# mprib/caliscope

Measured on AMD Instinct MI355X. Metric: observations/sec per LM iteration, higher is better.
Workload: dtype f64; 1 GPU; cfg4: 64 cams / 2000000 obs in total (200000 points / 2000000 obs on rank 0), extrinsics-only BA, linear loss; n_obs_total=2000000, params_per_camera=6, tolerances=ftol=xtol=gtol=1e-8 (reference defaults), sums=FP64 atomics (default)

## Files before the change

### caliscope_amd/csrc/cba_kernels.h

```cpp
#pragma once
#include <hip/hip_runtime.h>

#include "ba_math.h"
#include "trf_math.h"
#include "wg_binding.h"
#include "chol_schedule.h"

namespace cba {

constexpr int BLOCK = 256;
constexpr int CHUNK = 256;
constexpr int WAVE = 64;

struct VecLayout {
  int ncp;
  int ncp_pad;
  int P;
  int Ppad;
  __host__ __device__ long total() const { return (long)ncp_pad + 3L * Ppad; }
};

__device__ __forceinline__ double wave_sum(double v) {
#pragma unroll
  for (int o = WAVE / 2; o > 0; o >>= 1) v += __shfl_down(v, o, WAVE);
// ... 422 lines not shown
  double* sh_pt = sh_U + (DET ? DET_ROUND * DET_LD : n_cams * UP::STRIDE);
  double* sh_red = sh_pt + 9 * CHUNK;
  int* sh_perm = reinterpret_cast<int*>(sh_red + 8);
  int* sh_cs = sh_perm + CHUNK;
  constexpr int DROUNDS = (UP::STRIDE + DET_ROUND - 1) / DET_ROUND;
  constexpr int DM = DET ? DETM : 1;
  double dacc[DROUNDS][DM];
#pragma unroll
  for (int r = 0; r < DROUNDS; ++r)
#pragma unroll
    for (int m = 0; m < DM; ++m) dacc[r][m] = 0.0;
  if (!CAMG) stage_camtab(sh_tab, tab, n_cams);
  if (!DET)
    for (int i = threadIdx.x; i < n_cams * UP::STRIDE; i += BLOCK) sh_U[i] = 0.0;
  __syncthreads();
  const double* px = xvec + lay.ncp_pad;
  double* gp = gvec + lay.ncp_pad;
  double cost = 0.0;
  bool bad = false;
  const int last_obs = max(chunk_start[n_chunks] - 1, 0);
  int ch = blockIdx.x;
  int o0 = 0, o1 = 0;
  ObsRec cur = {0.0, 0.0, 0, 0};
  if (ch < n_chunks) {
    o0 = chunk_start[ch]; o1 = chunk_start[ch + 1];
    cur = load_obs(obs_u, obs_v, obs_cam, obs_pt, min(o0 + (int)threadIdx.x, last_obs));
  }
  while (ch < n_chunks) {
    const int nxt = ch + gridDim.x, nc = min(nxt, n_chunks - 1);
    const int no0 = chunk_start[nc], no1 = chunk_start[nc + 1];
    const ObsRec nx = load_obs(obs_u, obs_v, obs_cam, obs_pt, min(no0 + (int)threadIdx.x, last_obs));
    const int cp0 = chunk_pts[2 * ch], npts = chunk_pts[2 * ch + 1];
    const int pp = min(cp0 + (int)threadIdx.x, lay.P - 1);
    const int pa = pt_start[pp] - o0, pb = pt_start[pp + 1] - o0;
    const int i = o0 + threadIdx.x;
    double pv[9];
#pragma unroll
    for (int q = 0; q < 9; ++q) pv[q] = 0.0;
    double e[2] = {0.0, 0.0}, A[2][MAX_NC];
    int np_det = 0;
    if (DET) {
#pragma unroll
      for (int k = 0; k < MAX_NC; ++k) { A[0][k] = 0.0; A[1][k] = 0.0; }
      sh_perm[threadIdx.x] = det.perm[(long)ch * CHUNK + threadIdx.x];
      for (int q = threadIdx.x; q <= n_cams; q += BLOCK) sh_cs[q] = det.cstart[(long)ch * (n_cams + 1) + q];
    }
    if (i < o1) {
      const int cam = cur.cam, pt = cur.pt;
      double B[2][3];
      cost += obs_linearize<NC>(cam_of(cam), px[pt], px[lay.Ppad + pt], px[2 * lay.Ppad + pt], cur.u, cur.v, loss,
                                f_scale, e, A, B);
      if (!isfinite(e[0] + e[1])) bad = true;
      pv[0] = B[0][0] * B[0][0] + B[1][0] * B[1][0];
      pv[1] = B[0][0] * B[0][1] + B[1][0] * B[1][1];
      pv[2] = B[0][0] * B[0][2] + B[1][0] * B[1][2];
      pv[3] = B[0][1] * B[0][1] + B[1][1] * B[1][1];
      pv[4] = B[0][1] * B[0][2] + B[1][1] * B[1][2];
      pv[5] = B[0][2] * B[0][2] + B[1][2] * B[1][2];
      pv[6] = B[0][0] * e[0] + B[1][0] * e[1];
      pv[7] = B[0][1] * e[0] + B[1][1] * e[1];
      pv[8] = B[0][2] * e[0] + B[1][2] * e[1];
      const int np = (int)cam_of(cam).nparams;
      np_det = np;
      if (!DET) {
        double* Uc = sh_U + cam * UP::STRIDE;
#pragma unroll
        for (int r = 0; r < NC; ++r) {
          if (r < np) {
#pragma unroll
            for (int c = r; c < NC; ++c)
              if (c < np) lds_add(&Uc[UP::idx(r, c)], A[0][r] * A[0][c] + A[1][r] * A[1][c]);
            lds_add(&Uc[UP::TRI + r], A[0][r] * e[0] + A[1][r] * e[1]);
          }
        }
      }
    }
#pragma unroll
    for (int q = 0; q < 9; ++q) sh_pt[q * CHUNK + threadIdx.x] = pv[q];
    __syncthreads();
    auto reduce_point = [&](int p, int a, int b) {
      double acc[9];
#pragma unroll
      for (int q = 0; q < 9; ++q) acc[q] = 0.0;
      for (int j = a; j < b; ++j) {
#pragma unroll
        for (int q = 0; q < 9; ++q) acc[q] += sh_pt[q * CHUNK + j];
      }
#pragma unroll
      for (int q = 0; q < 6; ++q) Vblk[(long)q * lay.Ppad + p] = acc[q];
      gp[p] = acc[6];
      gp[lay.Ppad + p] = acc[7];
      gp[2 * lay.Ppad + p] = acc[8];
    };
    if (npts < 0 && threadIdx.x < 9) {
      double acc = 0.0;
      for (int j = 0; j < o1 - o0; ++j) acc += sh_pt[threadIdx.x * CHUNK + j];
      if (threadIdx.x < 6) unsafeAtomicAdd(&Vblk[(long)threadIdx.x * lay.Ppad + cp0], acc);
      else unsafeAtomicAdd(&gp[(long)(threadIdx.x - 6) * lay.Ppad + cp0], acc);
    }
    if ((int)threadIdx.x < npts && pb > pa) reduce_point(pp, pa, pb);
    for (int lp = threadIdx.x + BLOCK; lp < npts; lp += BLOCK) {
      const int p = cp0 + lp;
      const int a = pt_start[p] - o0, b = pt_start[p + 1] - o0;
      if (b > a) reduce_point(p, a, b);
    }
    __syncthreads();
    if (DET) {
#pragma unroll
      for (int rd = 0; rd < DROUNDS; ++rd) {
        double val[DET_ROUND];
#pragma unroll
        for (int q = 0; q < DET_ROUND; ++q) val[q] = cam_block_value<NC>(rd * DET_ROUND + q, A, e, np_det);
        det_round<DM>(val, sh_U, sh_perm, sh_cs, n_cams, dacc[rd]);
      }
    }
    cur = nx; o0 = no0; o1 = no1; ch = nxt;
  }
  double* dst = partialU + (long)blockIdx.x * n_cams * UP::STRIDE;
  if (DET) {
#pragma unroll
    for (int rd = 0; rd < DROUNDS; ++rd)
#pragma unroll
      for (int m = 0; m < DM; ++m) {
        const int task = (int)threadIdx.x + BLOCK * m;
        const int c = task / DET_ROUND, v = rd * DET_ROUND + task % DET_ROUND;
        if (task < n_cams * DET_ROUND && v < UP::STRIDE) dst[c * UP::STRIDE + v] = dacc[rd][m];
      }
  } else {
    for (int i = threadIdx.x; i < n_cams * UP::STRIDE; i += BLOCK) dst[i] = sh_U[i];
  }
  const double tot = block_sum(cost, sh_red);
  if (threadIdx.x == 0) partial_cost[blockIdx.x] = tot;
  if (bad) flags[0] = 1;
}

constexpr int CS_MAX_PTS = 512;
struct CsPlan {
  const double* u;
  const double* v;
  const int* cam;
  const int* ptl;
  const int* obs_start;
  const int* pt_first;
  const int* pt_count;
  int n_sc;
  int pmax;
};
struct TrialSrc {
  const double *x, *g, *sinv, *s;
  const double* ab;
  double* x_new;
  double* step_partial;
};
template <int NC, bool CAMG = false, bool UGLOB = false, bool TRIAL = false>
__global__ void __launch_bounds__(BLOCK)
k_build_cs(CsPlan cs, const double* __restrict__ xvec, VecLayout lay, const double* __restrict__ tab, int n_cams, int loss, double f_scale,
           double* __restrict__ Vblk, double* __restrict__ gvec, double* __restrict__ partialU, double* __restrict__ partial_cost,
           int* __restrict__ flags, const double* __restrict__ skip, TrialSrc trial = TrialSrc{}) {
  CBA_STAMP(ST_BUILD);
  using UP = UPack<NC>;
  static_assert(!UGLOB || CAMG, "a camera count beyond the LDS copy of the blocks is beyond the LDS copy of the table as well");
  if (skip && *skip != 0.0) return;
  extern __shared__ __attribute__((aligned(16))) double sh[];
  double* sh_tab = sh;
  double* sh_U = sh_tab + (CAMG ? 0 : n_cams * CAMTAB_LDS);
  const int PM = cs.pmax;
  double* sh_vg = sh_U + (UGLOB ? 0 : n_cams * UP::STRIDE);
  double* sh_x = sh_vg + 9 * PM;
  double* sh_red = sh_x + 3 * PM;
  if (!CAMG) stage_camtab(sh_tab, tab, n_cams);
  if (!UGLOB)
    for (int i = threadIdx.x; i < n_cams * UP::STRIDE; i += BLOCK) sh_U[i] = 0.0;
  const double* px = xvec + lay.ncp_pad;
  double* gp = gvec + lay.ncp_pad;
  double cost = 0.0, step_sq = 0.0;
  const double t_alpha = TRIAL ? trial.ab[0] : 0.0, t_beta = TRIAL ? trial.ab[1] : 0.0;
  bool bad = false;
  for (int s = blockIdx.x; s < cs.n_sc; s += gridDim.x) {
    const int o0 = cs.obs_start[s], o1 = cs.obs_start[s + 1], p0 = cs.pt_first[s], npts = cs.pt_count[s];
    __syncthreads();
    for (int i = threadIdx.x; i < 9 * PM; i += BLOCK) sh_vg[i] = 0.0;
    if (TRIAL) {
      for (int i = threadIdx.x; i < npts; i += BLOCK) {
#pragma unroll
        for (int k = 0; k < 3; ++k) {
          const long e = (long)lay.ncp_pad + (long)k * lay.Ppad + p0 + i;
          const double si = trial.sinv[e];
          const double st = t_alpha * trial.g[e] / (si * si) + t_beta * trial.s[e];
          const double xn = trial.x[e] + st;
          trial.x_new[e] = xn;
          sh_x[k * PM + i] = xn;
          step_sq = fma(st, st, step_sq);
        }
      }
    } else {
      for (int i = threadIdx.x; i < npts; i += BLOCK) {
        sh_x[i] = px[p0 + i]; sh_x[PM + i] = px[lay.Ppad + p0 + i]; sh_x[2 * PM + i] = px[2 * lay.Ppad + p0 + i];
      }
    }
    __syncthreads();
    const int R = (o1 - o0 + BLOCK - 1) / BLOCK;
    const int j0 = o0 + (int)threadIdx.x * R, j1 = min(j0 + R, o1);
    double acc[UP::STRIDE];
#pragma unroll
    for (int q = 0; q < UP::STRIDE; ++q) acc[q] = 0.0;
    int cur_cam = -1, cur_np = 0;
    auto flush = [&]() {
      if (cur_cam < 0) return;
      double* Uc = (UGLOB ? partialU : sh_U) + (long)cur_cam * UP::STRIDE;
#pragma unroll
      for (int r = 0; r < NC; ++r) {
        if (r < cur_np) {
#pragma unroll
          for (int c = r; c < NC; ++c)
            if (c < cur_np) { if (UGLOB) atomicAdd(&Uc[UP::idx(r, c)], acc[UP::idx(r, c)]); else lds_add(&Uc[UP::idx(r, c)], acc[UP::idx(r, c)]); }
          if (UGLOB) atomicAdd(&Uc[UP::TRI + r], acc[UP::TRI + r]); else lds_add(&Uc[UP::TRI + r], acc[UP::TRI + r]);
        }
      }
#pragma unroll
      for (int q = 0; q < UP::STRIDE; ++q) acc[q] = 0.0;
    };
    const int jl = max(o1 - 1, 0);
    int n_cam = cs.cam[min(j0, jl)], n_pl = cs.ptl[min(j0, jl)];
    double n_u = cs.u[min(j0, jl)], n_v = cs.v[min(j0, jl)];
    for (int j = j0; j < j1; ++j) {
      asm volatile("s_waitcnt vmcnt(0)" ::: "memory");
      asm volatile("" : "+v"(n_cam), "+v"(n_pl), "+v"(n_u), "+v"(n_v));
      const int cam = n_cam, pl = n_pl;
      const double u = n_u, v = n_v;
      n_cam = cs.cam[min(j + 1, jl)]; n_pl = cs.ptl[min(j + 1, jl)]; n_u = cs.u[min(j + 1, jl)]; n_v = cs.v[min(j + 1, jl)];
      __builtin_amdgcn_sched_barrier(0);
      if (cam != cur_cam) { flush(); cur_cam = cam; cur_np = (int)cam_of<CAMG>(sh_tab, tab, cam).nparams; }
      double e[2], A[2][MAX_NC], B[2][3];
      {
        double G[2][3], Yr[3], Aint[2][3];
        const CamTab& ctc = cam_of<CAMG>(sh_tab, tab, cam);
        cost += obs_factors(ctc, sh_x[pl], sh_x[PM + pl], sh_x[2 * PM + pl], u, v, loss, f_scale, e, G, Yr, Aint, B);
#pragma unroll
        for (int r = 0; r < 2; ++r) {
          const double p0 = Yr[1] * G[r][2] - Yr[2] * G[r][1], p1 = Yr[2] * G[r][0] - Yr[0] * G[r][2], p2 = Yr[0] * G[r][1] - Yr[1] * G[r][0];
          if constexpr (UGLOB) {
            A[r][0] = ctc.Jl[0] * p0 + ctc.Jl[3] * p1 + ctc.Jl[6] * p2;
            A[r][1] = ctc.Jl[1] * p0 + ctc.Jl[4] * p1 + ctc.Jl[7] * p2;
            A[r][2] = ctc.Jl[2] * p0 + ctc.Jl[5] * p1 + ctc.Jl[8] * p2;
          } else {
            A[r][0] = p0; A[r][1] = p1; A[r][2] = p2;
          }
          A[r][3] = G[r][0]; A[r][4] = G[r][1]; A[r][5] = G[r][2];
          A[r][6] = Aint[r][0]; A[r][7] = Aint[r][1]; A[r][8] = Aint[r][2];
        }
      }
      if (!isfinite(e[0] + e[1])) bad = true;
#pragma unroll
      for (int r = 0; r < NC; ++r) {
#pragma unroll
        for (int c = r; c < NC; ++c) acc[UP::idx(r, c)] = fma(A[1][r], A[1][c], fma(A[0][r], A[0][c], acc[UP::idx(r, c)]));
        acc[UP::TRI + r] = fma(A[1][r], e[1], fma(A[0][r], e[0], acc[UP::TRI + r]));
      }
      lds_add(&sh_vg[0 * PM + pl], B[0][0] * B[0][0] + B[1][0] * B[1][0]);
      lds_add(&sh_vg[1 * PM + pl], B[0][0] * B[0][1] + B[1][0] * B[1][1]);
      lds_add(&sh_vg[2 * PM + pl], B[0][0] * B[0][2] + B[1][0] * B[1][2]);
      lds_add(&sh_vg[3 * PM + pl], B[0][1] * B[0][1] + B[1][1] * B[1][1]);
      lds_add(&sh_vg[4 * PM + pl], B[0][1] * B[0][2] + B[1][1] * B[1][2]);
      lds_add(&sh_vg[5 * PM + pl], B[0][2] * B[0][2] + B[1][2] * B[1][2]);
      lds_add(&sh_vg[6 * PM + pl], B[0][0] * e[0] + B[1][0] * e[1]);
      lds_add(&sh_vg[7 * PM + pl], B[0][1] * e[0] + B[1][1] * e[1]);
      lds_add(&sh_vg[8 * PM + pl], B[0][2] * e[0] + B[1][2] * e[1]);
    }
    flush();
    __syncthreads();
    for (int i = threadIdx.x; i < npts; i += BLOCK) {
#pragma unroll
      for (int q = 0; q < 6; ++q) Vblk[(long)q * lay.Ppad + p0 + i] = sh_vg[q * PM + i];
      gp[p0 + i] = sh_vg[6 * PM + i];
      gp[lay.Ppad + p0 + i] = sh_vg[7 * PM + i];
      gp[2 * lay.Ppad + p0 + i] = sh_vg[8 * PM + i];
    }
  }
  __syncthreads();
  if (!UGLOB) {
    for (int c = threadIdx.x; c < n_cams; c += BLOCK) {
      const double* Jl = tab + (long)c * CAMTAB_DOUBLES + 12;
      double* Uc = sh_U + (long)c * UP::STRIDE;
      double M[3][3], T[3][3];
#pragma unroll
      for (int r = 0; r < 3; ++r)
#pragma unroll
        for (int q = 0; q < 3; ++q) M[r][q] = Uc[UP::idx(min(r, q), max(r, q))];
#pragma unroll
      for (int r = 0; r < 3; ++r)
#pragma unroll
        for (int q = 0; q < 3; ++q) T[r][q] = Jl[r] * M[0][q] + Jl[3 + r] * M[1][q] + Jl[6 + r] * M[2][q];
#pragma unroll
      for (int r = 0; r < 3; ++r)
#pragma unroll
        for (int q = r; q < 3; ++q) Uc[UP::idx(r, q)] = T[r][0] * Jl[q] + T[r][1] * Jl[3 + q] + T[r][2] * Jl[6 + q];
#pragma unroll
      for (int q = 3; q <= NC; ++q) {
        double* v0 = (q < NC) ? &Uc[UP::idx(0, q)] : &Uc[UP::TRI + 0];
        double* v1 = (q < NC) ? &Uc[UP::idx(1, q)] : &Uc[UP::TRI + 1];
        double* v2 = (q < NC) ? &Uc[UP::idx(2, q)] : &Uc[UP::TRI + 2];
        const double a0 = *v0, a1 = *v1, a2 = *v2;
        *v0 = Jl[0] * a0 + Jl[3] * a1 + Jl[6] * a2;
        *v1 = Jl[1] * a0 + Jl[4] * a1 + Jl[7] * a2;
        *v2 = Jl[2] * a0 + Jl[5] * a1 + Jl[8] * a2;
      }
    }
    __syncthreads();
    double* dst = partialU + (long)blockIdx.x * n_cams * UP::STRIDE;
    for (int i = threadIdx.x; i < n_cams * UP::STRIDE; i += BLOCK) dst[i] = sh_U[i];
  }
  const double tot = block_sum(cost, sh_red);
  if (threadIdx.x == 0) partial_cost[blockIdx.x] = tot;
  if (TRIAL) {
    const double st = block_sum(step_sq, sh_red);
    if (threadIdx.x == 0) trial.step_partial[blockIdx.x] = st;
  }
  if (bad) flags[0] = 1;
}

__global__ void __launch_bounds__(256)
k_gather_uv(const double* __restrict__ uv_raw, const int* __restrict__ order, long n, double* __restrict__ u, double* __restrict__ v) {
  for (long i = (long)blockIdx.x * 256 + threadIdx.x; i < n; i += (long)gridDim.x * 256) {
    const double2 w = reinterpret_cast<const double2*>(uv_raw)[order[i]];
    u[i] = w.x; v[i] = w.y;
  }
}
__global__ void __launch_bounds__(256)
k_cs_fill(const int* __restrict__ perm, const int* __restrict__ sc_obs, const int* __restrict__ sc_p0, const double* __restrict__ u,
          const double* __restrict__ v, const int* __restrict__ cam, const int* __restrict__ pt, double* __restrict__ cu, double* __restrict__ cv,
          int* __restrict__ ccam, int* __restrict__ cptl) {
  const int s = blockIdx.x, o0 = sc_obs[s], o1 = sc_obs[s + 1], p0 = sc_p0[s];
  for (int j = o0 + threadIdx.x; j < o1; j += 256) {
    const int i = perm[j];
    cu[j] = u[i]; cv[j] = v[i]; ccam[j] = cam[i]; cptl[j] = pt[i] - p0;
  }
}

template <int NC>
__global__ void k_unpack_camera_grad(const double* __restrict__ Upacked, const int* __restrict__ cam_off,
                                     const int* __restrict__ cam_np, int n_cams, double* __restrict__ gvec) {
  using UP = UPack<NC>;
  const int t = blockIdx.x * blockDim.x + threadIdx.x;
  const int c = t / NC, r = t % NC;
  if (c >= n_cams || r >= cam_np[c]) return;
  gvec[cam_off[c] + r] = Upacked[c * UP::STRIDE + UP::TRI + r];
}

template <int NC>
__global__ void k_scale_update(const double* __restrict__ Upacked, const double* __restrict__ Vblk,
                               const int* __restrict__ param_cam, const int* __restrict__ param_loc, VecLayout lay,
                               int first, double* __restrict__ sinv, const double* __restrict__ cdiag) {
  using UP = UPack<NC>;
  const long total = lay.total();
  for (long i = (long)blockIdx.x * blockDim.x + threadIdx.x; i < total; i += (long)gridDim.x * blockDim.x) {
    double v;
    if (i < lay.ncp_pad) {
      if (i >= lay.ncp) continue;
      const int r = param_loc[i];
      v = Upacked[param_cam[i] * UP::STRIDE + UP::idx(r, r)];
    } else {
      const long k = (i - lay.ncp_pad) / lay.Ppad, p = (i - lay.ncp_pad) % lay.Ppad;
      if (p >= lay.P) continue;
      const int q = (k == 0) ? 0 : (k == 1 ? 3 : 5);
      v = Vblk[(long)q * lay.Ppad + p];
      if (cdiag) v += cdiag[k * lay.Ppad + p];
    }
    v = sqrt(v);
    if (first) { if (v == 0.0) v = 1.0; }
    else v = fmax(v, sinv[i]);
    sinv[i] = v;
  }
}

__global__ void k_cam_rescale(const double* __restrict__ state, const double* __restrict__ mult, const double* __restrict__ diag_h,
                              int ncp, double* __restrict__ sinv, double* __restrict__ cam_diag) {
  const int i = blockIdx.x * blockDim.x + threadIdx.x;
  if (i >= ncp) return;
  const double si = state[i] * mult[i];
  sinv[i] = si;
  cam_diag[i] = diag_h[i] * si * si;
}

__global__ void __launch_bounds__(BLOCK)
k_lin_scalars(const double* __restrict__ x, const double* __restrict__ g, const double* __restrict__ sinv,
              long total, int cam_end, int count_cams, int max_from, double* __restrict__ v1, double* __restrict__ partial,
              double* __restrict__ partial_max) {
  __shared__ double sh_red[BLOCK / WAVE];
  double s0 = 0, s1 = 0, s2 = 0, m = 0;
  for (long i = (long)blockIdx.x * BLOCK + threadIdx.x; i < total; i += (long)gridDim.x * BLOCK) {
    const double gi = g[i], si = sinv[i], xi = x[i];
    const double gh = gi / si;
    v1[i] = gh / si;
    if (i >= max_from) m = fmax(m, fabs(gi));
    if (i < cam_end && !count_cams) continue;
    s0 += gh * gh;
    s1 += (xi * si) * (xi * si);
    s2 += xi * xi;
  }
  double r;
  r = block_sum(s0, sh_red); if (threadIdx.x == 0) partial[blockIdx.x * 4 + 0] = r;
  r = block_sum(s1, sh_red); if (threadIdx.x == 0) partial[blockIdx.x * 4 + 1] = r;
  r = block_sum(s2, sh_red); if (threadIdx.x == 0) partial[blockIdx.x * 4 + 2] = r;
  if (threadIdx.x == 0) partial[blockIdx.x * 4 + 3] = 0.0;
  r = block_max(m, sh_red); if (threadIdx.x == 0) partial_max[blockIdx.x] = r;
}

__global__ void k_combine(const double* __restrict__ g, const double* __restrict__ sinv, const double* __restrict__ s,
                          double a, double b, long total, const double* __restrict__ over, int n_over, double* __restrict__ out) {
  for (long i = (long)blockIdx.x * blockDim.x + threadIdx.x; i < total; i += (long)gridDim.x * blockDim.x) {
    const double si = sinv[i];
    out[i] = (i < n_over) ? over[i] : a * g[i] / (si * si) + b * s[i];
  }
}

constexpr int MAIL_GNORM = 60, MAIL_GNORM_SEQ = 61;
struct SpecSkip {
  const int* word;
  const double* max_rows;
  int n_rows;
  double* mail; unsigned long long seq;
};
__device__ __forceinline__ void publish_gnorm(const SpecSkip& sk) {
  __shared__ double sh_gn[BLOCK / WAVE];
  double m = 0.0;
  for (int b = threadIdx.x; b < sk.n_rows; b += BLOCK) m = fmax(m, sk.max_rows[b]);
  m = block_max(m, sh_gn);
  if (threadIdx.x == 0) {
    sk.mail[MAIL_GNORM] = m;
    __threadfence_system();
    reinterpret_cast<volatile unsigned long long*>(sk.mail)[MAIL_GNORM_SEQ] = sk.seq;
  }
}
__global__ void __launch_bounds__(BLOCK) k_gnorm_pub(SpecSkip sk) { publish_gnorm(sk); }

// ... 2021 lines not shown
    for (int k = 0; k < NP; ++k) rec[k] = mine[k];
    asm volatile("s_waitcnt lgkmcnt(0)" ::: "memory");
#pragma unroll
    for (int k = 0; k < NP; ++k) asm volatile("" : "+v"(rec[k].x), "+v"(rec[k].y));
    const bool more = ch + stride < n_chunks;
    if (more) issue(nx.o0);
    const int ncam = obs_cam[min(nx.o0 + tid, last_obs)];
    const Ent nn = load_ent(min(ch + 2 * stride, last_chunk));
    const PtIn pcur = load_point(cur.cp0, cur.npts);
    __builtin_amdgcn_sched_barrier(0);
    double t0, t1, t2;
    {
      const double* cs = sh_step + cam * CSS;
      const double w0 = cs[0], w1 = cs[1], w2 = cs[2];
      const double Y0 = rec[0].x, Y1 = rec[0].y, Y2 = rec[1].x;
      const double m0 = fma(w1, Y2, fma(-w2, Y1, cs[3]));
      const double m1 = fma(w2, Y0, fma(-w0, Y2, cs[4]));
      const double m2 = fma(w0, Y1, fma(-w1, Y0, cs[5]));
      t0 = fma(rec[4].y, m2, fma(rec[3].x, m1, rec[1].y * m0));
      t1 = fma(rec[5].x, m2, fma(rec[3].y, m1, rec[2].x * m0));
      t2 = fma(rec[5].y, m2, fma(rec[4].x, m1, rec[2].y * m0));
      if constexpr (NC == 9) {
        const double i0 = cs[6], i1 = cs[7], i2 = cs[8];
        t0 = fma(rec[9].x, i2, fma(rec[7].y, i1, fma(rec[6].x, i0, t0)));
        t1 = fma(rec[9].y, i2, fma(rec[8].x, i1, fma(rec[6].y, i0, t1)));
        t2 = fma(rec[10].x, i2, fma(rec[8].y, i1, fma(rec[7].x, i0, t2)));
      }
      if (cur.o0 + tid >= cur.o1) { t0 = 0.0; t1 = 0.0; t2 = 0.0; }
    }
    double* pt = sh_pt + buf * BSR_PT;
    pt[tid] = t0; pt[CHUNK + tid] = t1; pt[2 * CHUNK + tid] = t2;
    point_phase(pprev, sh_pt + (buf ^ 1) * BSR_PT, eprev.cp0, eprev.npts, eprev.o0);
    __syncthreads();
    pprev = pcur; eprev = cur;
    buf ^= 1;
    if (!more) break;
    cam = ncam; cur = nx; nx = nn; ch += stride;
  }
  asm volatile("s_waitcnt vmcnt(0)" ::: "memory");
  point_phase(pprev, sh_pt + (buf ^ 1) * BSR_PT, eprev.cp0, eprev.npts, eprev.o0);
  if (SCAL) {
    __syncthreads();
    double r;
    r = block_sum(sc0, sh_pt); if (tid == 0) step_partial[blockIdx.x * 4 + 0] = r;
    r = block_sum(sc1, sh_pt); if (tid == 0) { step_partial[blockIdx.x * 4 + 1] = r; step_partial[blockIdx.x * 4 + 2] = 0.0; step_partial[blockIdx.x * 4 + 3] = 0.0; }
  }
}
template <int NC, bool SCAL = false>
__global__ void __launch_bounds__(BLOCK)
k_backsub_rec(const double* __restrict__ Trec, const int* __restrict__ obs_cam, const int* __restrict__ pt_start, const int* __restrict__ chunk_start,
              const int* __restrict__ chunk_pts, int n_chunks, VecLayout lay, const double* __restrict__ tab, const int* __restrict__ cam_off,
              const int* __restrict__ cam_np, int n_cams, double lam, const double* __restrict__ lam_dev, const double* __restrict__ Vblk,
              const double* __restrict__ gvec, const double* __restrict__ sinv, double* __restrict__ svec, double* __restrict__ step_partial) {
  CBA_STAMP(ST_BACKSUB);
  extern __shared__ __attribute__((aligned(16))) double sh[];
  if (lam_dev) lam = *lam_dev;
  backsub_rec_body<NC, SCAL>(Trec, obs_cam, pt_start, chunk_start, chunk_pts, n_chunks, lay, tab, cam_off, cam_np, n_cams, lam, Vblk,
                             gvec + lay.ncp_pad, sinv + lay.ncp_pad, svec, svec + lay.ncp_pad, step_partial, sh);
}

__global__ void __launch_bounds__(BLOCK)
k_step_scalars(const double* __restrict__ g, const double* __restrict__ sinv, const double* __restrict__ s, long total,
               long first, double* __restrict__ partial) {
  __shared__ double sh_red[BLOCK / WAVE];
  double s0 = 0, s1 = 0;
  for (long i = first + (long)blockIdx.x * BLOCK + threadIdx.x; i < total; i += (long)gridDim.x * BLOCK) {
    const double p = s[i] * sinv[i];
    s0 += p * p;
    s1 += g[i] * s[i];
  }
  double r;
  r = block_sum(s0, sh_red); if (threadIdx.x == 0) partial[blockIdx.x * 4 + 0] = r;
  r = block_sum(s1, sh_red); if (threadIdx.x == 0) partial[blockIdx.x * 4 + 1] = r;
  if (threadIdx.x == 0) { partial[blockIdx.x * 4 + 2] = 0.0; partial[blockIdx.x * 4 + 3] = 0.0; }
}
__global__ void __launch_bounds__(BLOCK)
k_w_scalar(const double* __restrict__ g, const double* __restrict__ sinv, const double* __restrict__ s, long total,
           long first, const double* __restrict__ scal_gdot, double gh_sq, const double* __restrict__ gh_sq_dev,
           double* __restrict__ partial) {
  __shared__ double sh_red[BLOCK / WAVE];
  if (gh_sq_dev) gh_sq = *gh_sq_dev;
  const double c = scal_gdot[0] / gh_sq;
  double s0 = 0;
  for (long i = first + (long)blockIdx.x * BLOCK + threadIdx.x; i < total; i += (long)gridDim.x * BLOCK) {
    const double w = s[i] * sinv[i] - c * g[i] / sinv[i];
    s0 += w * w;
  }
  const double r = block_sum(s0, sh_red);
  if (threadIdx.x == 0) partial[blockIdx.x] = r;
}

__global__ void __launch_bounds__(BLOCK)
k_trial_update(const double* __restrict__ x, const double* __restrict__ g, const double* __restrict__ sinv,
               const double* __restrict__ s, double alpha, double beta, long total, int cam_end, int count_cams,
               const double* __restrict__ cam_x_new, int n_over, const double* __restrict__ ab_dev, double* __restrict__ x_new,
               double* __restrict__ partial, double* __restrict__ tab_out = nullptr, const double* __restrict__ cam_const = nullptr,
               const int* __restrict__ cam_model = nullptr, const int* __restrict__ cam_np = nullptr, const int* __restrict__ cam_off = nullptr,
               int n_cams = 0) {
  __shared__ double sh_red[BLOCK / WAVE];
  if (ab_dev) { alpha = ab_dev[0]; beta = ab_dev[1]; }
  double s0 = 0;
  auto entry = [&](long i) {
    const double si = sinv[i];
    double st = alpha * g[i] / (si * si) + beta * s[i];
    double xn = x[i] + st;
    if (i < n_over) { xn = cam_x_new[i]; st = xn - x[i]; }
    x_new[i] = xn;
    if (i >= cam_end || count_cams) s0 += st * st;
  };
  if (tab_out) {
    if (blockIdx.x == 0)
      for (long i = threadIdx.x; i < cam_end; i += BLOCK) entry(i);
    for (long i = cam_end + (long)blockIdx.x * BLOCK + threadIdx.x; i < total; i += (long)gridDim.x * BLOCK) entry(i);
  } else {
    for (long i = (long)blockIdx.x * BLOCK + threadIdx.x; i < total; i += (long)gridDim.x * BLOCK) entry(i);
  }
  const double r = block_sum(s0, sh_red);
  if (threadIdx.x == 0) partial[blockIdx.x] = r;
  if (tab_out && blockIdx.x == 0) {
    __threadfence();
    __syncthreads();
    for (int c = threadIdx.x; c < n_cams; c += BLOCK) {
      double xc[MAX_NC];
      const int np = cam_np[c];
      for (int i = 0; i < MAX_NC; ++i) xc[i] = (i < np) ? __builtin_nontemporal_load(&x_new[cam_off[c] + i]) : 0.0;
      CamTab t;
      cam_prepare(xc, cam_const + c * CAM_CONST_STRIDE, cam_model[c], np, &t, cam_off[c]);
      const double* src = reinterpret_cast<const double*>(&t);
      for (int i = 0; i < CAMTAB_DOUBLES; ++i) tab_out[c * CAMTAB_DOUBLES + i] = src[i];
    }
  }
}

__device__ __forceinline__ void fused_lam(double* __restrict__ scal, double radius_in, double* __restrict__ fz);
struct SubspaceIn;
__device__ __forceinline__ void fused_subspace(double* __restrict__ scal, const int* __restrict__ flags, double* __restrict__ fz, const SubspaceIn* pre = nullptr);
__global__ void k_fused_lam(double* __restrict__ scal, double radius_in, double* __restrict__ fz) { fused_lam(scal, radius_in, fz); }
__global__ void k_fused_subspace(double* __restrict__ scal, const int* __restrict__ flags, double* __restrict__ fz) {
  fused_subspace(scal, flags, fz);
}

__device__ __forceinline__ void fused_lam(double* __restrict__ scal, double radius_in, double* __restrict__ fz) {
  const double gh_sq = scal[0], jg_sq = scal[12] + scal[3], xs = sqrt(scal[1]);
  const double radius = radius_in > 0.0 ? radius_in : (xs > 0.0 ? xs : 1.0);
  const double lam = trf::damping(jg_sq, gh_sq, radius);
  fz[0] = lam; fz[1] = radius;
  scal[40] = lam; scal[41] = radius;
}

struct SubspaceIn { double gh_sq, c_gg, jg, lam, radius; int f1, f2; };
__device__ __forceinline__ SubspaceIn subspace_inputs(const double* __restrict__ scal, const int* __restrict__ flags, const double* __restrict__ fz) {
  return SubspaceIn{scal[0], scal[3], scal[12], fz[0], fz[1], flags[1], flags[2]};
}
__device__ __forceinline__ void fused_subspace(double* __restrict__ scal, const int* __restrict__ flags, double* __restrict__ fz, const SubspaceIn* pre) {
  const SubspaceIn in = pre ? *pre : subspace_inputs(scal, flags, fz);
  const double gh_sq = in.gh_sq, jg_sq = in.jg + in.c_gg, p_sq = scal[16], ghp = scal[17];
  const double lam = in.lam, radius = in.radius, gh_norm = sqrt(gh_sq);
  const double c = ghp / gh_sq;
  const double w_sq = p_sq - ghp * ghp / gh_sq;
  scal[20] = w_sq;
  const bool two_d = true;
  double need_host = 0.0, pS[2] = {0.0, 0.0}, alpha = 0.0, beta = 0.0, predicted = 0.0;
  const bool ok = in.f1 == 0 && in.f2 == 0 && isfinite(p_sq) && isfinite(ghp) && gh_sq > 0.0;
  if (!ok || !(w_sq > 1e-3 * p_sq)) {
    need_host = 1.0;
  } else {
    double b00, b01 = 0.0, b11;
    const double w_norm = two_d ? sqrt(w_sq) : 1.0;
    if (two_d) trf::subspace_model(jg_sq, gh_sq, lam, ghp, p_sq, w_sq, &b00, &b01, &b11);
    else { b00 = jg_sq / gh_sq; b11 = 1.0; }
    trf::solve_subspace_2d(b00, b01, b11, gh_norm, 0.0, radius, pS);
    if (!two_d) pS[1] = 0.0;
    predicted = -(0.5 * (pS[0] * (b00 * pS[0] + b01 * pS[1]) + pS[1] * (b01 * pS[0] + b11 * pS[1])) + gh_norm * pS[0]);
    beta = two_d ? pS[1] / w_norm : 0.0;
    alpha = pS[0] / gh_norm - beta * c;
  }
  fz[2] = alpha; fz[3] = beta;
  scal[42] = need_host; scal[43] = pS[0]; scal[44] = pS[1]; scal[45] = predicted; scal[46] = alpha; scal[47] = beta;
}


struct BoundArgs {
  const double* lb;
  const double* ub;
  const double* state_in;
  double* state_out;
  double* cam_diag_out;
};
struct ScaleSums { double s0 = 0.0, s1 = 0.0, s2 = 0.0, m = 0.0; };
__device__ __forceinline__ bool scale_point_diag(long i, const VecLayout& lay, const double* __restrict__ Vblk, const double* __restrict__ cdiag, double* v) {
  const long k = (i - lay.ncp_pad) / lay.Ppad, p = (i - lay.ncp_pad) % lay.Ppad;
  if (p >= lay.P) return false;
  const int q = (k == 0) ? 0 : (k == 1 ? 3 : 5);
  *v = Vblk[(long)q * lay.Ppad + p];
  if (cdiag) *v += cdiag[k * lay.Ppad + p];
  return true;
}
__device__ __forceinline__ void scale_lin_entry(long i, bool live, double v, double si, int first, bool carry, double gi, double xi,
                                                double* __restrict__ sinv, double* __restrict__ v1, ScaleSums& a) {
  if (live) {
    v = sqrt(v);
    if (first) { if (v == 0.0) v = 1.0; } else v = fmax(v, si);
    si = v;
    sinv[i] = si;
  } else if (carry) {
    sinv[i] = si;
  }
  const double gh = gi / si;
  v1[i] = gh / si;
  a.m = fmax(a.m, fabs(gi));
  a.s0 += gh * gh;
  a.s1 += (xi * si) * (xi * si);
  a.s2 += xi * xi;
}
template <int NC, bool BND = false>
__global__ void __launch_bounds__(BLOCK)
k_scale_lin(const double* __restrict__ Upacked, const double* __restrict__ Vblk, const int* __restrict__ param_cam,
            const int* __restrict__ param_loc, VecLayout lay, int first, double* __restrict__ sinv, const double* __restrict__ cdiag,
            const double* __restrict__ x, const double* __restrict__ g, double* __restrict__ v1, double* __restrict__ partial,
            double* __restrict__ partial_max, const double* __restrict__ sinv_in = nullptr, BoundArgs bnd = BoundArgs{}) {
  CBA_STAMP(ST_SCALE_LIN);
  using UP = UPack<NC>;
  __shared__ double sh_red[BLOCK / WAVE];
  const long total = lay.total();
  const double* sin = sinv_in ? sinv_in : sinv;
  ScaleSums a;
  double s3 = 0.0;
  for (long i = (long)blockIdx.x * BLOCK + threadIdx.x; i < total; i += (long)gridDim.x * BLOCK) {
    double si = sin[i];
    bool live = true;
    double v = 0.0;
    if (BND && i < lay.ncp) {
      const int r = param_loc[i];
      double sj = sqrt(Upacked[param_cam[i] * UP::STRIDE + UP::idx(r, r)]);
      if (first) { if (sj == 0.0) sj = 1.0; } else sj = fmax(sj, bnd.state_in[i]);
      bnd.state_out[i] = sj;
      const double gi = g[i], xi = x[i], lo = bnd.lb[i], hi = bnd.ub[i];
      double vv = 1.0, dv = 0.0;
      if (gi < 0.0 && isfinite(hi)) { vv = hi - xi; dv = -1.0; }
      else if (gi > 0.0 && isfinite(lo)) { vv = xi - lo; dv = 1.0; }
      a.m = fmax(a.m, fabs(gi * vv));
      if (dv != 0.0) vv *= sj;
      const double se = sj / sqrt(vv);
      const double dh = gi * dv / sj;
      sinv[i] = se;
      bnd.cam_diag_out[i] = dh * se * se;
      const double gh = gi / se;
      v1[i] = gh / se;
      a.s0 += gh * gh;
      a.s1 += (xi * se) * (xi * se);
      a.s2 += xi * xi;
      s3 += dh * gh * gh;
      continue;
    }
    if (i < lay.ncp_pad) {
      if (i >= lay.ncp) live = false;
      else { const int r = param_loc[i]; v = Upacked[param_cam[i] * UP::STRIDE + UP::idx(r, r)]; }
    } else {
      live = scale_point_diag(i, lay, Vblk, cdiag, &v);
    }
    scale_lin_entry(i, live, v, si, first, sinv_in != nullptr, g[i], x[i], sinv, v1, a);
  }
  double r;
  r = block_sum(a.s0, sh_red); if (threadIdx.x == 0) partial[blockIdx.x * 4 + 0] = r;
  r = block_sum(a.s1, sh_red); if (threadIdx.x == 0) partial[blockIdx.x * 4 + 1] = r;
  r = block_sum(a.s2, sh_red); if (threadIdx.x == 0) partial[blockIdx.x * 4 + 2] = r;
  r = block_sum(s3, sh_red); if (threadIdx.x == 0) partial[blockIdx.x * 4 + 3] = r;
  r = block_max(a.m, sh_red); if (threadIdx.x == 0) partial_max[blockIdx.x] = r;
  if (BND && blockIdx.x == 0)
    for (int i = lay.ncp + threadIdx.x; i < lay.ncp_pad; i += BLOCK) { bnd.state_out[i] = 1.0; bnd.cam_diag_out[i] = 0.0; }
}

template <int NC> struct ScaleFuse {
  static constexpr int CPW = 1;
  static constexpr int PT_UNROLL = 4;
  static constexpr int PT_ENTRIES = PT_UNROLL * 64 * REDUCE_RY;
  __host__ __device__ static int cam_wgs(int n_cams) { return (n_cams + CPW - 1) / CPW; }
  __host__ __device__ static long pt_wgs(const VecLayout& lay) { return (lay.total() - lay.ncp + PT_ENTRIES - 1) / PT_ENTRIES; }
};
struct ScaleArgs {
  const double* Vblk; VecLayout lay; int first;
  double* sinv; const double* sinv_in;
  const double* x; const double* g;
  double* v1; double* partial; double* partial_max;
};
template <int NC>
__global__ void __launch_bounds__(64 * REDUCE_RY)
k_reduce_scale_pub(const double* __restrict__ partial, int nrow, int n_cams, double* __restrict__ out, double* __restrict__ grad_out,
                   const int* __restrict__ cam_off, const int* __restrict__ cam_np, ScaleArgs sc, int with_pub, PubArgs pub) {
  CBA_STAMP(ST_REDUCE_PUB);
  using UP = UPack<NC>;
  using SF = ScaleFuse<NC>;
  int wg = (int)blockIdx.x;
  if (with_pub) {
    if (wg == 0) { publish_packet(pub); return; }
    --wg;
  }
  __shared__ double sh[REDUCE_RY][64];
  __shared__ double sh_col[64];
  __shared__ double sh_s[4][REDUCE_RY];
  const int tx = threadIdx.x, ty = threadIdx.y;
  const int n_cam_wgs = SF::cam_wgs(n_cams);
  const double* __restrict__ xv = sc.x;
  double* __restrict__ sout = sc.sinv;
  const double* sin = sc.sinv_in ? sc.sinv_in : sout;
  double* __restrict__ v1 = sc.v1;
  ScaleSums a;
  if (wg < n_cam_wgs) {
    const int c0 = wg * SF::CPW, ncol = min(SF::CPW, n_cams - c0) * UP::STRIDE;
    const int width = n_cams * UP::STRIDE, j = c0 * UP::STRIDE + tx;
    double acc[8] = {0.0, 0.0, 0.0, 0.0, 0.0, 0.0, 0.0, 0.0};
    if (tx < ncol) {
      int b = ty;
      for (; b + 31 * REDUCE_RY < nrow; b += 32 * REDUCE_RY) {
        double v[32];
#pragma unroll
        for (int q = 0; q < 32; ++q) v[q] = partial[(long)(b + q * REDUCE_RY) * width + j];
#pragma unroll
        for (int q = 0; q < 32; ++q) acc[q & 7] += v[q];
      }
      for (; b + 7 * REDUCE_RY < nrow; b += 8 * REDUCE_RY) {
#pragma unroll
        for (int q = 0; q < 8; ++q) acc[q] += partial[(long)(b + q * REDUCE_RY) * width + j];
      }
      for (; b < nrow; b += REDUCE_RY) acc[0] += partial[(long)b * width + j];
    }
    sh[ty][tx] = ((acc[0] + acc[1]) + (acc[2] + acc[3])) + ((acc[4] + acc[5]) + (acc[6] + acc[7]));
    __syncthreads();
    if (ty == 0) {
      double tot = 0.0;
#pragma unroll
      for (int y = 0; y < REDUCE_RY; ++y) tot += sh[y][tx];
      sh_col[tx] = tot;
      if (tx < ncol) {
        out[j] = tot;
        const int c = j / UP::STRIDE, r = j % UP::STRIDE - UP::TRI;
        if (r >= 0 && r < cam_np[c]) grad_out[cam_off[c] + r] = tot;
      }
    }
    __syncthreads();
    if (ty == 0 && tx < SF::CPW * NC) {
      const int cl = tx / NC, r = tx % NC, c = c0 + cl;
      if (c < n_cams && r < cam_np[c]) {
        const long i = cam_off[c] + r;
        scale_lin_entry(i, true, sh_col[cl * UP::STRIDE + UP::idx(r, r)], sin[i], sc.first, false, sh_col[cl * UP::STRIDE + UP::TRI + r], xv[i], sout, v1, a);
      }
    }
  } else {
    const double* __restrict__ gv = sc.g;
    const double* __restrict__ Vblk = sc.Vblk;
    const long total = sc.lay.total(), stride = ((long)gridDim.x - (with_pub ? 1 : 0) - n_cam_wgs) * (64 * REDUCE_RY);
    constexpr int UNR = SF::PT_UNROLL;
    const long i0 = sc.lay.ncp + (long)(wg - n_cam_wgs) * (64 * REDUCE_RY) + ty * 64 + tx;
    if (i0 < total) {
      double v[UNR], si[UNR], gi[UNR], xi[UNR];
      bool live[UNR];
#pragma unroll
      for (int u = 0; u < UNR; ++u) {
        const long i = (i0 + u * stride < total) ? i0 + u * stride : i0;
        v[u] = 0.0;
        live[u] = i >= sc.lay.ncp_pad && scale_point_diag(i, sc.lay, Vblk, nullptr, &v[u]);
        si[u] = sin[i]; gi[u] = gv[i]; xi[u] = xv[i];
      }
#pragma unroll
      for (int u = 0; u < UNR; ++u)
        if (i0 + u * stride < total) scale_lin_entry(i0 + u * stride, live[u], v[u], si[u], sc.first, sc.sinv_in != nullptr, gi[u], xi[u], sout, v1, a);
    }
  }
  const double r0 = wave_sum(a.s0), r1 = wave_sum(a.s1), r2 = wave_sum(a.s2), rm = wave_max(a.m);
  if (tx == 0) { sh_s[0][ty] = r0; sh_s[1][ty] = r1; sh_s[2][ty] = r2; sh_s[3][ty] = rm; }
  __syncthreads();
  if (ty == 0 && tx < 4) {
    double r = 0.0;
    for (int y = 0; y < REDUCE_RY; ++y) r = (tx == 3) ? fmax(r, sh_s[3][y]) : r + sh_s[tx][y];
    if (tx == 3) { sc.partial_max[wg] = r; sc.partial[wg * 4 + 3] = 0.0; } else sc.partial[wg * 4 + tx] = r;
  }
}

__device__ __forceinline__ double column_sum(const double* __restrict__ partial, int nrow, int width, int col, double* sh) {
  double s = 0.0;
  for (int b = threadIdx.x; b < nrow; b += BLOCK) s += partial[(long)b * width + col];
  return block_sum(s, sh);
}

__global__ void __launch_bounds__(BLOCK)
k_lin_finish(const double* __restrict__ partial_lin, const double* __restrict__ partial_max, int rows_lin,
             const double* __restrict__ partial_jv, int rows_jv, double radius, double* __restrict__ scal, double* __restrict__ fz) {
  __shared__ double sh_red[10][BLOCK / WAVE];
  double v[10];
#pragma unroll
  for (int q = 0; q < 10; ++q) v[q] = 0.0;
  for (int b = threadIdx.x; b < rows_lin; b += BLOCK) {
#pragma unroll
    for (int j = 0; j < 4; ++j) v[j] += partial_lin[(long)b * 4 + j];
    v[4] = fmax(v[4], partial_max[b]);
  }
  for (int b = threadIdx.x; b < rows_jv; b += BLOCK) {
#pragma unroll
    for (int j = 0; j < 4; ++j) v[5 + j] += partial_jv[(long)b * 4 + j];
  }
  const int lane = threadIdx.x & (WAVE - 1), w = threadIdx.x / WAVE;
#pragma unroll
  for (int q = 0; q < 9; ++q) {
    const double r = (q == 4) ? wave_max(v[q]) : wave_sum(v[q]);
    if (lane == 0) sh_red[q][w] = r;
  }
  __syncthreads();
  if (threadIdx.x == 0) {
#pragma unroll
    for (int q = 0; q < 9; ++q) {
      double r = 0.0;
      for (int i = 0; i < BLOCK / WAVE; ++i) r = (q == 4) ? fmax(r, sh_red[q][i]) : r + sh_red[q][i];
      scal[q < 5 ? q : 12 + (q - 5)] = r;
    }
    fused_lam(scal, radius, fz);
  }
}

__global__ void __launch_bounds__(BLOCK)
k_step_finish(const double* __restrict__ partial, int rows, double* __restrict__ scal, const int* __restrict__ flags, double* __restrict__ fz) {
  __shared__ double sh_red[4][BLOCK / WAVE];
  double v[4] = {0.0, 0.0, 0.0, 0.0};
  for (int b = threadIdx.x; b < rows; b += BLOCK) {
#pragma unroll
    for (int j = 0; j < 4; ++j) v[j] += partial[(long)b * 4 + j];
  }
  const int lane = threadIdx.x & (WAVE - 1), w = threadIdx.x / WAVE;
#pragma unroll
  for (int j = 0; j < 4; ++j) {
    const double r = wave_sum(v[j]);
    if (lane == 0) sh_red[j][w] = r;
  }
  __syncthreads();
  if (threadIdx.x == 0) {
#pragma unroll
    for (int j = 0; j < 4; ++j) {
      double r = 0.0;
      for (int i = 0; i < BLOCK / WAVE; ++i) r += sh_red[j][i];
      scal[16 + j] = r;
    }
    fused_subspace(scal, flags, fz);
  }
}

constexpr int STEP_SMALL_THREADS = 1024;
constexpr long STEP_SMALL_MAX = 32768;
__global__ void __launch_bounds__(STEP_SMALL_THREADS)
k_step_small(const double* __restrict__ g, const double* __restrict__ sinv, const double* __restrict__ s, long total, double* __restrict__ scal,
             const int* __restrict__ flags, double* __restrict__ fz) {
  __shared__ double sh_red[2][STEP_SMALL_THREADS / WAVE];
  double s0 = 0.0, s1 = 0.0;
  for (long i = threadIdx.x; i < total; i += STEP_SMALL_THREADS) {
    const double p = s[i] * sinv[i];
    s0 += p * p;
    s1 += g[i] * s[i];
  }
  const int lane = threadIdx.x & (WAVE - 1), w = threadIdx.x / WAVE;
  const double r0 = wave_sum(s0), r1 = wave_sum(s1);
  if (lane == 0) { sh_red[0][w] = r0; sh_red[1][w] = r1; }
  __syncthreads();
  if (threadIdx.x == 0) {
    double a = 0.0, b = 0.0;
    for (int i = 0; i < STEP_SMALL_THREADS / WAVE; ++i) { a += sh_red[0][i]; b += sh_red[1][i]; }
    scal[16] = a; scal[17] = b; scal[18] = 0.0; scal[19] = 0.0;
    fused_subspace(scal, flags, fz);
  }
}

__global__ void __launch_bounds__(BLOCK)
k_step_cam(const double* __restrict__ partial, int rows, const double* __restrict__ x, const double* __restrict__ g, const double* __restrict__ sinv,
           const double* __restrict__ s, int ncp_pad, double* __restrict__ scal, const int* __restrict__ flags, double* __restrict__ fz,
           double* __restrict__ x_new, double* __restrict__ step_cam, double* __restrict__ tab_out, const double* __restrict__ cam_const,
           const int* __restrict__ cam_model, const int* __restrict__ cam_np, const int* __restrict__ cam_off, int n_cams,
           const double* __restrict__ lb = nullptr, const double* __restrict__ ub = nullptr, int ncp = 0) {
  CBA_STAMP(ST_STEP_CAM);
  extern __shared__ __attribute__((aligned(16))) double sh_xc[];
  __shared__ double sh_red[4][BLOCK / WAVE];
  __shared__ double sh_ab[3];
  __shared__ int sh_outside;
  if (threadIdx.x == 0) sh_outside = 0;
  SubspaceIn pre{};
  if (threadIdx.x == 0) pre = subspace_inputs(scal, flags, fz);
  constexpr int KEEP = 2;
  double kx[KEEP], kg[KEEP], ksi[KEEP], ks[KEEP];
#pragma unroll
  for (int q = 0; q < KEEP; ++q) {
    const int i = threadIdx.x + q * BLOCK;
    const bool in = i < ncp_pad;
    kx[q] = in ? x[i] : 0.0; kg[q] = in ? g[i] : 0.0; ksi[q] = in ? sinv[i] : 1.0; ks[q] = in ? s[i] : 0.0;
  }
  const int my_cam = threadIdx.x < n_cams ? threadIdx.x : -1;
  int my_np = 0, my_off = 0, my_model = 0;
  double my_const[CAM_CONST_STRIDE];
  if (my_cam >= 0) {
    my_np = cam_np[my_cam]; my_off = cam_off[my_cam]; my_model = cam_model[my_cam];
#pragma unroll
    for (int i = 0; i < CAM_CONST_STRIDE; ++i) my_const[i] = cam_const[my_cam * CAM_CONST_STRIDE + i];
  }
  double v[2] = {0.0, 0.0};
  for (int b = threadIdx.x; b < rows; b += BLOCK) { v[0] += partial[(long)b * 4 + 0]; v[1] += partial[(long)b * 4 + 1]; }
#pragma unroll
  for (int q = 0; q < KEEP; ++q) {
    const double ps = ks[q] * ksi[q];
    v[0] = fma(ps, ps, v[0]);
    v[1] = fma(kg[q], ks[q], v[1]);
  }
  for (int i = threadIdx.x + KEEP * BLOCK; i < ncp_pad; i += BLOCK) {
    const double si = s[i], ps = si * sinv[i];
    v[0] = fma(ps, ps, v[0]);
    v[1] = fma(g[i], si, v[1]);
  }
  const int lane = threadIdx.x & (WAVE - 1), w = threadIdx.x / WAVE;
#pragma unroll
  for (int j = 0; j < 2; ++j) {
    const double r = wave_sum(v[j]);
    if (lane == 0) sh_red[j][w] = r;
  }
  __syncthreads();
  if (threadIdx.x == 0) {
#pragma unroll
    for (int j = 0; j < 2; ++j) {
      double r = 0.0;
      for (int i = 0; i < BLOCK / WAVE; ++i) r += sh_red[j][i];
      scal[16 + j] = r;
    }
    scal[18] = 0.0; scal[19] = 0.0;
    fused_subspace(scal, flags, fz, &pre);
    sh_ab[0] = fz[2]; sh_ab[1] = fz[3]; sh_ab[2] = scal[42];
  }
  __syncthreads();
  if (sh_ab[2] != 0.0) return;
  const double alpha = sh_ab[0], beta = sh_ab[1];
  double s0 = 0.0;
  auto entry = [&](int i, double xi, double gi, double si, double stp) {
    const double st = alpha * gi / (si * si) + beta * stp;
    const double xn = xi + st;
    x_new[i] = xn;
    sh_xc[i] = xn;
    s0 = fma(st, st, s0);
    if (lb && i < ncp && !(xn > lb[i] && xn < ub[i])) sh_outside = 1;
  };
#pragma unroll
  for (int q = 0; q < KEEP; ++q)
    if (threadIdx.x + q * BLOCK < ncp_pad) entry(threadIdx.x + q * BLOCK, kx[q], kg[q], ksi[q], ks[q]);
  for (int i = threadIdx.x + KEEP * BLOCK; i < ncp_pad; i += BLOCK) entry(i, x[i], g[i], sinv[i], s[i]);
  {
    const double r = wave_sum(s0);
    if (lane == 0) sh_red[2][w] = r;
  }
  __syncthreads();
  if (sh_outside) {
    if (threadIdx.x == 0) { scal[42] = 2.0; step_cam[0] = 0.0; }
    return;
  }
  if (threadIdx.x == 0) {
    double r = 0.0;
    for (int i = 0; i < BLOCK / WAVE; ++i) r += sh_red[2][i];
    step_cam[0] = r;
  }
  for (int c = threadIdx.x; c < n_cams; c += BLOCK) {
    double xc[MAX_NC];
    const bool mine = c == my_cam;
    const int np = mine ? my_np : cam_np[c], off = mine ? my_off : cam_off[c];
    for (int i = 0; i < MAX_NC; ++i) xc[i] = (i < np) ? sh_xc[off + i] : 0.0;
    CamTab t;
    if (mine) cam_prepare(xc, my_const, my_model, np, &t, off);
    else cam_prepare(xc, cam_const + c * CAM_CONST_STRIDE, cam_model[c], np, &t, off);
    const double* src = reinterpret_cast<const double*>(&t);
    for (int i = 0; i < CAMTAB_DOUBLES; ++i) tab_out[c * CAMTAB_DOUBLES + i] = src[i];
  }
}

__global__ void __launch_bounds__(BLOCK)
k_publish(double* __restrict__ scal, int n_scal, int* __restrict__ flags, double* __restrict__ host_scal,
          int* __restrict__ host_flags, unsigned long long seq, const double* __restrict__ part_a, int rows_a, int slot_a,
          const double* __restrict__ part_b, int rows_b, int slot_b) {
  __shared__ double sh_red[BLOCK / WAVE];
  const int t = threadIdx.x;
  if (part_a) { const double r = column_sum(part_a, rows_a, 1, 0, sh_red); if (t == 0) scal[slot_a] = r; }
  if (part_b) { const double r = column_sum(part_b, rows_b, 1, 0, sh_red); if (t == 0) scal[slot_b] = r; }
  __syncthreads();
  if (t < n_scal) host_scal[t] = scal[t];
  if (t < 4) { host_flags[t] = flags[t]; flags[t] = 0; }
  __threadfence_system();
  __syncthreads();
  if (t == 0) reinterpret_cast<volatile unsigned long long*>(host_scal)[63] = seq;
}

__global__ void k_publish_cam(const double* __restrict__ a, const double* __restrict__ b, const double* __restrict__ c, int ncp,
                              double* __restrict__ host, unsigned long long* __restrict__ host_seq, unsigned long long seq) {
  for (int i = threadIdx.x; i < ncp; i += blockDim.x) {
    host[i] = a[i];
    if (b) host[ncp + i] = b[i];
    if (c) host[2 * ncp + i] = c[i];
  }
  __threadfence_system();
  __syncthreads();
  if (threadIdx.x == 0) *reinterpret_cast<volatile unsigned long long*>(host_seq) = seq;
}

__global__ void k_fill(double* __restrict__ p, double v, long n) {
  for (long i = (long)blockIdx.x * blockDim.x + threadIdx.x; i < n; i += (long)gridDim.x * blockDim.x) p[i] = v;
}


__global__ void __launch_bounds__(BLOCK)
k_triangulate(long n_points, const long* __restrict__ pt_start, const int* __restrict__ obs_cam, const double* __restrict__ obs_xy,
              const int* __restrict__ cam_model, const double* __restrict__ cam_intr, const double* __restrict__ cam_P, int f32,
              double* __restrict__ xyz, double* __restrict__ undist) {
  const long q = (long)blockIdx.x * BLOCK + threadIdx.x;
  if (q >= n_points) return;
  const long a = pt_start[q], b = pt_start[q + 1];
  const double nan = __longlong_as_double(0x7ff8000000000000LL);
  double M[4][4];
#pragma unroll
  for (int r = 0; r < 4; ++r)
#pragma unroll
    for (int c = 0; c < 4; ++c) M[r][c] = 0.0;
  for (long i = a; i < b; ++i) {
    const int cam = obs_cam[i];
    double x = obs_xy[2 * i], y = obs_xy[2 * i + 1];
    if (cam_intr) undistort_one(cam_model[cam], cam_intr + 9 * cam, x, y, f32, &x, &y);
    if (undist) { undist[2 * i] = x; undist[2 * i + 1] = y; }
    const double* P = cam_P + 12 * cam;
    double r0[4], r1[4];
#pragma unroll
    for (int c = 0; c < 4; ++c) { r0[c] = x * P[8 + c] - P[c]; r1[c] = y * P[8 + c] - P[4 + c]; }
#pragma unroll
    for (int r = 0; r < 4; ++r)
#pragma unroll
      for (int c = r; c < 4; ++c) M[r][c] += r0[r] * r0[c] + r1[r] * r1[c];
  }
  if (b - a < 2) { xyz[3 * q] = xyz[3 * q + 1] = xyz[3 * q + 2] = nan; return; }
#pragma unroll
  for (int r = 1; r < 4; ++r)
#pragma unroll
    for (int c = 0; c < r; ++c) M[r][c] = M[c][r];
  double w[4];
  sym4_null_vector(M, w);
  xyz[3 * q] = w[0] / w[3];
  xyz[3 * q + 1] = w[1] / w[3];
  xyz[3 * q + 2] = w[2] / w[3];
}


constexpr int HEAVY_OBS = 40;

__global__ void k_zero_heavy(const int* __restrict__ heavy_pts, int n_heavy, VecLayout lay, double* __restrict__ a, int rows_a,
                             double* __restrict__ b, int rows_b) {
  const int t = blockIdx.x * blockDim.x + threadIdx.x;
  if (t >= n_heavy) return;
  const int p = heavy_pts[t];
  for (int k = 0; k < rows_a; ++k) a[(long)k * lay.Ppad + p] = 0.0;
  for (int k = 0; k < rows_b; ++k) b[(long)k * lay.Ppad + p] = 0.0;
}

__global__ void k_heavy_finish(const int* __restrict__ heavy_pts, const int* __restrict__ heavy_frag, int n_heavy, VecLayout lay, double lam,
                               const double* __restrict__ Vblk, const double* __restrict__ gvec, const double* __restrict__ sinv,
                               double* __restrict__ svec) {
  const int t = blockIdx.x * blockDim.x + threadIdx.x;
  if (t >= n_heavy || !heavy_frag[t]) return;
  const int p = heavy_pts[t];
  const double* gp = gvec + lay.ncp_pad;
  const double* dp = sinv + lay.ncp_pad;
  double* sp = svec + lay.ncp_pad;
  double Vd[6], L[6], q[3], y[3], x[3] = {0.0, 0.0, 0.0};
#pragma unroll
  for (int k = 0; k < 6; ++k) Vd[k] = Vblk[(long)k * lay.Ppad + p];
  const double d0 = dp[p], d1 = dp[lay.Ppad + p], d2 = dp[2 * lay.Ppad + p];
  Vd[0] += lam * d0 * d0; Vd[3] += lam * d1 * d1; Vd[5] += lam * d2 * d2;
#pragma unroll
  for (int k = 0; k < 3; ++k) q[k] = gp[(long)k * lay.Ppad + p] + sp[(long)k * lay.Ppad + p];
  if (chol3(Vd, L)) { chol3_fwd(L, q, y); chol3_bwd(L, y, x); }
#pragma unroll
  for (int k = 0; k < 3; ++k) sp[(long)k * lay.Ppad + p] = -x[k];
}

template <int NC>
__global__ void __launch_bounds__(BLOCK)
k_heavy_schur(const int* __restrict__ heavy_pts, const int* __restrict__ pt_start, const int* __restrict__ obs_cam,
              const int* __restrict__ cam_off, const int* __restrict__ cam_np, int ncp,
              const double* __restrict__ Trec, const double* __restrict__ tab, double* __restrict__ heavy_W, double* __restrict__ Sacc) {
  constexpr int REC = SchurRec<NC>::HREC;
  extern __shared__ __attribute__((aligned(16))) double sh[];
  double* W = sh;
  int* seen = reinterpret_cast<int*>(W + (size_t)ncp * 3);
  const int h = blockIdx.x, p = heavy_pts[h];
  for (int e = threadIdx.x; e < ncp * 3; e += BLOCK) W[e] = 0.0;
  for (int e = threadIdx.x; e < ncp; e += BLOCK) seen[e] = 0;
  __syncthreads();
  const int o0 = pt_start[p], o1 = pt_start[p + 1];
  for (int i = o0 + threadIdx.x; i < o1; i += BLOCK) {
    const int cam = obs_cam[i], off = cam_off[cam], np = cam_np[cam];
    double T[3 * NC];
    expand_record<NC>(Trec + (long)i * REC, tab + (long)cam * CAMTAB_DOUBLES + 12, T);
#pragma unroll
    for (int r = 0; r < NC; ++r) {
      if (r < np) {
        lds_add(&W[(off + r) * 3 + 0], T[3 * r]); lds_add(&W[(off + r) * 3 + 1], T[3 * r + 1]); lds_add(&W[(off + r) * 3 + 2], T[3 * r + 2]);
        seen[off + r] = 1;
      }
    }
  }
  __syncthreads();
  double* Wg = heavy_W + (long)h * ncp * 3;
  for (int e = threadIdx.x; e < ncp * 3; e += BLOCK) Wg[e] = W[e];
  for (long e = threadIdx.x; e < (long)ncp * ncp; e += BLOCK) {
    const int r = (int)(e / ncp), c = (int)(e % ncp);
    if (c < r || !seen[r] || !seen[c]) continue;
    const double acc = W[r * 3] * W[c * 3] + W[r * 3 + 1] * W[c * 3 + 1] + W[r * 3 + 2] * W[c * 3 + 2];
    unsafeAtomicAdd(&Sacc[(long)r * ncp + c], acc);
  }
}

struct ConPlan {
  int n_con, n_comp;
  const int* pt;
  const int* lp;
  const double* dist;
  const double* weight;
  const int* order;
  const int* comp_con;
  const int* comp_pt;
// ... 561 lines not shown
```

### caliscope_amd/csrc/cba_lib.hip

```cpp
#include <hip/hip_runtime.h>

#include <algorithm>
#include <atomic>
#include <chrono>
#include <cmath>
#include <condition_variable>
#include <cstdarg>
#include <cstdio>
#include <cstdlib>
#include <cstring>
#include <map>
#include <mutex>
#include <shared_mutex>
#include <memory>
#include <string>
#include <type_traits>
#include <thread>
#include <utility>
#include <vector>

#include <rccl/rccl.h>
#include <rocprofiler-sdk-roctx/roctx.h>

#include "../../include/caliscope_ba.h"
#include "cba_kernels.h"
#include "chol_factor.h"
#include "schur_plan.h"
#include "host_plan.h"
#include "wg_binding.h"

using namespace cba;

#ifndef CBA_SOURCE_DIGEST
#define CBA_SOURCE_DIGEST "unknown"
#endif
extern "C" __attribute__((used, visibility("hidden"))) const char cba_source_digest_marker[] = "CBA_SOURCE_DIGEST=" CBA_SOURCE_DIGEST;

static thread_local std::string g_last_error;

static int fail(int code, const char* fmt, ...) {
  char buf[1024];
  va_list ap;
  va_start(ap, fmt);
  vsnprintf(buf, sizeof(buf), fmt, ap);
  va_end(ap);
  g_last_error = buf;
  return code;
}

#define HIPCHK(expr)                                                                                   \
  do {                                                                                                 \
    hipError_t _e = (expr);                                                                            \
    if (_e != hipSuccess)                                                                              \
      return fail(CBA_ERR_HIP, "%s failed: %s (%s:%d)", #expr, hipGetErrorString(_e), __FILE__, __LINE__); \
  } while (0)

enum TimerId {
  T_CAM_PREP = 0, T_COST, T_BUILD, T_BUILD_REDUCE, T_SCALE_SCALARS, T_JV, T_SCHUR, T_SCHUR_REDUCE, T_CHOLESKY,
  T_BACKSUB, T_VECTOR, T_SCHUR_PAIRS, T_EXCHANGE, T_COUNT
};
static const char* kTimerNames[T_COUNT] = {
    "cam_prep", "cost", "build", "build_reduce", "scale_scalars", "jv", "schur", "schur_reduce_finalize",
    "cholesky_solve", "backsub", "vector_ops", "schur_pairs", "exchange"};

struct EventPair { hipEvent_t a, b; };
struct cba_group;

constexpr int JV_ROWS = 2048, CON_ROWS = 1024, PARTIAL4_ROWS = JV_ROWS + CON_ROWS;

struct cba_problem {
  int device = 0;
  hipStream_t stream = nullptr;
  int C = 0, P = 0, ncp = 0, nct = 6;
  long N = 0;
  VecLayout lay{};
  int n_chunks = 0, grid = 0, max_obs_per_point = 0;
  int G = 1, gsz = 1, n_tiles = 1, n_tile_chunks = 0, tile_grid = 0;
  int cus = 256;
  double plan_lane_util = 0.0;
  long tile_stream_len = 0, n_pairs = 0;
  TilePlan tp{};
  int* tile_wg_begin = nullptr;
  int loss = 0;
  double f_scale = 1.0;
  long device_bytes = 0;
  double *obs_u = nullptr, *obs_v = nullptr;
  int *obs_cam = nullptr, *obs_pt = nullptr, *pt_start = nullptr, *chunk_start = nullptr, *order = nullptr;
  int* chunk_pts = nullptr;
  double* cam_const = nullptr;
  int *cam_model = nullptr, *cam_np = nullptr, *cam_off = nullptr, *param_cam = nullptr, *param_loc = nullptr;
  double *tab = nullptr, *tab_new = nullptr;
  double *x0 = nullptr, *x = nullptr, *x_new = nullptr, *g = nullptr, *s = nullptr, *sinv = nullptr, *v1 = nullptr, *v2 = nullptr;
  double *V = nullptr, *Upacked = nullptr;
  double *partial = nullptr, *partial4 = nullptr, *partial1 = nullptr;
  double* partial_gmax = nullptr;
  int scale_rows = 0;
  bool scale_fused = true;
  long partial_width = 0;
  bool want_chol_trace = false;
  long long* chol_trace = nullptr;
  int ldw = 0;
  double *Sacc = nullptr, *S = nullptr, *Lbuf = nullptr, *rhs = nullptr, *red = nullptr, *Trec = nullptr, *partial_b = nullptr;
  CsPlan cs{};
  bool tab_global = false;
  int det_m = 0;
  DetPlan det{nullptr, nullptr};
  double* tri = nullptr;
  double* Xinv = nullptr;
  double* Tinv = nullptr;
  bool chol_ends = true;
  bool linear_pass = true;
  bool chol_pair = true;
  bool chol_early = true;
  bool fuse_reg_finalize = true;
  double* scal = nullptr;
  double* xbuf = nullptr;
  double *sinv_state_c = nullptr, *cam_diag = nullptr, *cam_over1 = nullptr, *cam_over2 = nullptr;
  bool cam_scaled = false, cam_state_saved = false;
  double *fz = nullptr, *V2 = nullptr, *g2 = nullptr, *U2 = nullptr, *partial4b = nullptr;
  bool eval_only = false;
  bool peer_needs_primitives = false;
  bool have_build = false;
  bool trial_built = false;
  bool cost_pending = false;
  double cost_x = 0.0;
  double trial_cost = 0.0;
  int grid_backsub = 1;
  int jv_grid = 0;
  bool has_fragments = false;
  bool backsub_rec = false;
  int n_heavy = 0; int* heavy_pts = nullptr; int* heavy_frag = nullptr; double* heavy_W = nullptr;
  std::vector<int> h_heavy_pts;
  ConPlan con{};
  int con_grid = 0;
  int n_con_orphan = 0; int* con_orphan = nullptr;
  int* flags = nullptr;
  double* h_scal = nullptr;
  int* h_flags = nullptr;
  double* d_hscal = nullptr;
  double *h_cam = nullptr, *d_hcam = nullptr;
  double *h_bcam = nullptr, *d_hbcam = nullptr;
  double *lb_dev = nullptr, *ub_dev = nullptr, *sinv_state_c2 = nullptr, *cam_diag2 = nullptr;
  bool bounds_on = false;
  unsigned long long publish_seq = 0;
  bool spin_wait = true;
  int* d_hflags = nullptr;
  bool first_scale = true;
  double* sinv2 = nullptr;
  bool spec_enqueued = false, spec_valid = false;
  int spec_rows_jv = 0;
  bool spec_skip = true, tol_set = false, last_trial_hint = false;
  double ftol = 0.0, xtol = 0.0;
  int* spec_word = nullptr;
  bool spec_jv_enqueued = false;
  bool spec_jv_dropped = false;
  bool spec_scale_ready = false;
  long spec_jv_skipped = 0;
  unsigned long long gnorm_seq = 0;
  bool gnorm_mailed = false;
  bool lf_pending = false;
  LinFin lf{};
  bool have_x0 = false;
  std::vector<int> h_tile_wg_begin;
  struct PlanTask* plan_task = nullptr;
  int reg_reduce_y = 4;
  int plan_max_blocks = 0;
  size_t partial_capacity = 0;
  bool plan_is_cheap = false;
  int plan_error = 0;
  bool schur_clock = false;
  long long* stamps = nullptr;
  bool begun = false, linearized = false, stepped = false, have_trial = false;
  double gh_sq = 0.0;
  std::vector<int> h_cam_off, h_cam_np;
  double* h_vec = nullptr;
  size_t h_vec_doubles = 0;
  hipEvent_t h_vec_sent = nullptr;
  bool h_vec_in_flight = false;
  bool timers_on = false;
  std::vector<EventPair> pending[T_COUNT];
  std::vector<EventPair> free_events;
  double t_ms[T_COUNT] = {0};
  long t_calls[T_COUNT] = {0};
  std::vector<void*> allocs;
  std::vector<size_t> alloc_bytes;
  size_t mail_doubles = 0;
  char* arena_cur = nullptr; size_t arena_left = 0, arena_next = (size_t)4 << 20;
  char* up_stage = nullptr; size_t up_cap = 0, up_used = 0;
  std::atomic<ncclComm_t> comm{nullptr};
  std::atomic<bool> comm_aborted{false};
  cba_group* group = nullptr;
  int rank = 0, world = 1;
  unsigned long long group_generation = 0;
  bool sharded() const { return comm.load() != nullptr || group != nullptr || comm_aborted.load(); }
  bool small_solve_on = true;
  bool one_workgroup_solve() const { return ncp <= SMALL_N && small_solve_on && !sharded() && !chol_trace; }
};

constexpr size_t kPoolChunk = (size_t)4 << 20;
constexpr size_t kPoolKeep = 4;
constexpr size_t kPoolStagingMax = (size_t)8 << 20;
struct DevicePool {
  std::vector<void*> chunks;
  std::vector<hipStream_t> streams;
  std::vector<std::pair<double*, size_t>> mail;
  std::vector<std::pair<double*, size_t>> staging;
  std::vector<char*> upstage;
};
constexpr size_t kUpStage = (size_t)256 << 10, kUpStageMax = (size_t)64 << 10;
static std::mutex g_pool_mu;
static std::map<int, DevicePool> g_pool;

template <typename T>
static int dev_alloc(cba_problem* p, T** out, size_t count) {
  const size_t bytes = (std::max<size_t>(count, 1) * sizeof(T) + 255) & ~(size_t)255;
  if (bytes > p->arena_left) {
    const size_t chunk = std::max(bytes, p->arena_next);
    void* ptr = nullptr;
    if (chunk == kPoolChunk) {
      std::lock_guard<std::mutex> lock(g_pool_mu);
      DevicePool& pool = g_pool[p->device];
      if (!pool.chunks.empty()) { ptr = pool.chunks.back(); pool.chunks.pop_back(); }
    }
    if (!ptr) HIPCHK(hipMalloc(&ptr, chunk));
    p->allocs.push_back(ptr);
    p->alloc_bytes.push_back(chunk);
    if (bytes >= p->arena_next) {
      p->device_bytes += (long)bytes;
      *out = static_cast<T*>(ptr);
      return CBA_OK;
    }
    p->arena_cur = static_cast<char*>(ptr);
    p->arena_left = chunk;
    p->arena_next = std::min<size_t>(p->arena_next * 2, (size_t)256 << 20);
  }
  *out = reinterpret_cast<T*>(p->arena_cur);
  p->arena_cur += bytes;
  p->arena_left -= bytes;
  p->device_bytes += (long)bytes;
  return CBA_OK;
}
template <typename T>
static int dev_upload(cba_problem* p, T** out, const T* h, size_t count) {
  int rc = dev_alloc(p, out, count);
  if (rc) return rc;
  const size_t bytes = count * sizeof(T);
  if (bytes && p->up_stage && p->stream && bytes <= kUpStageMax && p->up_used + bytes <= p->up_cap) {
    std::memcpy(p->up_stage + p->up_used, h, bytes);
    HIPCHK(hipMemcpyAsync(*out, p->up_stage + p->up_used, bytes, hipMemcpyHostToDevice, p->stream));
    p->up_used += (bytes + 63) & ~(size_t)63;
  } else if (bytes) {
    HIPCHK(hipMemcpy(*out, h, bytes, hipMemcpyHostToDevice));
  }
  return CBA_OK;
}
template <typename T, typename V>
static int dev_upload(cba_problem* p, T** out, const V& h) {
  static_assert(std::is_same<typename std::remove_cv<typename std::remove_pointer<decltype(h.data())>::type>::type, T>::value, "element type");
  return dev_upload(p, out, h.data(), h.size());
}
template <typename T>
static int dev_zeros(cba_problem* p, T** out, size_t count) {
  int rc = dev_alloc(p, out, count);
  if (rc) return rc;
  HIPCHK(hipMemsetAsync(*out, 0, count * sizeof(T), p->stream));
  return CBA_OK;
// ... 541 lines not shown
  }
  {
    int t = 0;
    for (int a = 0; a < G; ++a)
      for (int b = a; b < G; ++b, ++t) { ta[t] = a; tb[t] = b; }
  }
  int rc;
  int *dob = nullptr, *dcs = nullptr, *dcode = nullptr, *dwf = nullptr, *dwt = nullptr, *dwe = nullptr, *dws = nullptr, *dta = nullptr, *dtb = nullptr,
      *dgc = nullptr, *dgp = nullptr;
  unsigned *dcodes = nullptr, *dnit = nullptr;
#define TRYP(e) do { rc = (e); if (rc) return rc; } while (0)
  TRYP(upload(&dob, plan.obs)); TRYP(upload(&dcs, plan.chunk_start)); TRYP(upload(&dcode, plan.code_start));
  TRYP(upload(&dcodes, plan.codes)); TRYP(upload(&dnit, plan.nit));
  TRYP(upload(&dwf, bind.wfirst)); TRYP(upload(&dwt, bind.wt)); TRYP(upload(&dwe, bind.wend)); TRYP(upload(&dws, bind.wstride));
  TRYP(upload(&dta, ta)); TRYP(upload(&dtb, tb)); TRYP(upload(&dgc, gcam)); TRYP(upload(&dgp, gpar));
  TRYP(upload(&out.tile_wg_begin, bind.wgb));
#undef TRYP
  out.h_wgb = bind.wgb;
  {
    int rows = 0;
    for (int t = 0; t < nT; ++t) rows = std::max(rows, (bind.wgb[t + 1] - bind.wgb[t]) * std::max(prm.rep, 1));
    out.reg_reduce_y = rows > 96 ? REG_REDUCE_Y_MAX : 4;
  }
  lap("upload");
  TilePlan tp{};
  tp.chunk_start = dcs; tp.wg_first = dwf; tp.wg_end = dwe; tp.wg_tile = dwt; tp.wg_stride = dws; tp.tile_a = dta; tp.tile_b = dtb;
  tp.group_cam_begin = dgc; tp.group_par_begin = dgp; tp.g = g;
  tp.tile_elems = CT * p->nct * p->nct; tp.obs = dob; tp.rep = prm.rep;
  tp.codes = dcodes; tp.code_start = dcode; tp.nit = dnit;
  tp.prio_shift = (NC == 6) ? 0 : -1;
  if (const char* e = std::getenv("CBA_PAIR_PRIO")) tp.prio_shift = std::atoi(e);
  out.tp = tp;
  return CBA_OK;
}

static void apply_install(cba_problem* p, PlanInstall& in) {
  p->tp = in.tp;
  p->tile_grid = in.tile_grid; p->n_tile_chunks = in.n_tile_chunks; p->reg_reduce_y = in.reg_reduce_y;
  p->tile_stream_len = in.tile_stream_len; p->n_pairs = in.n_pairs; p->plan_lane_util = in.lane_util;
  p->tile_wg_begin = in.tile_wg_begin;
  p->h_tile_wg_begin = std::move(in.h_wgb);
  for (auto& o : in.owned) { p->allocs.push_back(o.first); p->alloc_bytes.push_back(o.second); p->device_bytes += (long)o.second; }
  in.owned.clear();
}

static int prepare_install_background(const cba_problem* p, Reg2Plan& plan, const Reg2Params& prm, PlanInstall& in) {
  if (hipSetDevice(p->device) != hipSuccess) return CBA_ERR_HIP;
  auto upload = [&](auto** out, const auto& h) -> int {
    using T = typename std::remove_pointer<typename std::remove_pointer<decltype(out)>::type>::type;
    const size_t bytes = std::max<size_t>(h.size(), 1) * sizeof(T);
    void* ptr = nullptr;
    if (hipMalloc(&ptr, bytes) != hipSuccess) return CBA_ERR_HIP;
    in.owned.emplace_back(ptr, bytes);
    if (!h.empty() && hipMemcpy(ptr, h.data(), h.size() * sizeof(T), hipMemcpyHostToDevice) != hipSuccess) return CBA_ERR_HIP;
    *out = static_cast<T*>(ptr);
    return CBA_OK;
  };
  return (p->nct == 9) ? prepare_install<9, Reg3Cfg<9>>(p, plan, prm, p->plan_max_blocks, upload, in)
                       : prepare_install<6, Reg3Cfg<6>>(p, plan, prm, p->plan_max_blocks, upload, in);
}

struct PlanTask {
  Reg2Params prm;
  Reg2Plan cheap, plan;
  PlanInstall install;
  const cba_problem* handle = nullptr;
  int rc_cheap = 0, rc = 0;
  double seconds_cheap = 0.0, seconds = 0.0;
  bool two_stage = false;
  std::atomic<int> stage{0};
  std::atomic<bool> cancel{false};
  std::mutex mu;
  std::condition_variable cv;
  std::thread th;
  HostVec<int> hcam_keep;
  std::vector<int> hps_keep;
  void start(const Reg2Params& params, const int* hcam, const int* hps, bool two, const cba_problem* h) {
    prm = params;
    handle = h;
    prm.cancel = &cancel;
    two_stage = two;
    th = std::thread([this, hcam, hps] {
      auto publish = [this](int s) { { std::lock_guard<std::mutex> lock(mu); stage.store(s, std::memory_order_release); } cv.notify_all(); };
      if (two_stage) {
        const auto t0 = std::chrono::steady_clock::now();
        Reg2Params c = prm;
        c.cheap = true;
        rc_cheap = build_reg2_plan(c, hcam, hps, cheap);
        seconds_cheap = std::chrono::duration<double>(std::chrono::steady_clock::now() - t0).count();
        publish(1);
      }
      const auto t0 = std::chrono::steady_clock::now();
      if (two_stage && prm.threads == 0) prm.threads = (int)std::max(1u, std::min(32u, usable_cpus() / 2));
      rc = (two_stage && rc_cheap) ? rc_cheap : build_reg2_plan(prm, hcam, hps, plan);
      if (two_stage && !rc && !cancel.load()) {
        rc = prepare_install_background(handle, plan, prm, install);
        if (rc) for (auto& o : install.owned) (void)hipFree(o.first);
        if (rc) install.owned.clear();
      }
      seconds = std::chrono::duration<double>(std::chrono::steady_clock::now() - t0).count();
      publish(2);
    });
  }
  void wait_stage(int s) {
    std::unique_lock<std::mutex> lock(mu);
    cv.wait(lock, [&] { return stage.load(std::memory_order_acquire) >= s; });
  }
  ~PlanTask() {
    cancel.store(true);
    if (th.joinable()) th.join();
    for (auto& o : install.owned) (void)hipFree(o.first);
  }
};

static void drop_plan_task(cba_problem* p) {
  delete p->plan_task;
  p->plan_task = nullptr;
}

static int install_reg2_plan(cba_problem* p, Reg2Plan& plan, const Reg2Params& prm) {
  PlanInstall in;
  auto upload = [&](auto** out, const auto& h) { return dev_upload(p, out, h); };
  const int rc = (p->nct == 9) ? prepare_install<9, Reg3Cfg<9>>(p, plan, prm, p->plan_max_blocks, upload, in)
                               : prepare_install<6, Reg3Cfg<6>>(p, plan, prm, p->plan_max_blocks, upload, in);
  if (rc) return rc;
  apply_install(p, in);
  return CBA_OK;
}

static void choose_schur_groups(cba_problem* p) {
  const int gmax = std::min(p->C, kSchurRegMaxGroup);
  p->G = (p->C + gmax - 1) / gmax;
  p->gsz = (p->C + p->G - 1) / p->G;
  p->n_tiles = p->G * (p->G + 1) / 2;
}

template <int NC>
static int configure_kernels(cba_problem* p) {
  int rc;
  {
    p->tab_global = false;
    const size_t worst = std::max(std::max(lds_jv(p, 2), lds_backsub(p)), lds_tprep<NC>(p));
    p->tab_global = !p->det_m && worst > 150 * 1024;
    if (const char* e = std::getenv("CBA_CAMTAB_GLOBAL")) p->tab_global = std::atoi(e) != 0 && !p->det_m;
  }
  if ((rc = allow_lds(k_cost<false>, lds_cost(p)))) return rc;
  if ((rc = allow_lds(k_cost<true>, lds_cost(p)))) return rc;
  if ((rc = allow_lds(k_cost<false, true>, lds_cost(p)))) return rc;
  if ((rc = allow_lds(k_cost<true, true>, lds_cost(p)))) return rc;
  const bool use_cs = p->cs.n_sc && !p->det_m && !p->n_heavy;
  if (use_cs) {
    if (build_cs_uglob<NC>(p)) { rc = allow_lds(k_build_cs<NC, true, true>, lds_build_cs<NC>(p, true, true)); if (!rc) rc = allow_lds(k_build_cs<NC, true, true, true>, lds_build_cs<NC>(p, true, true)); }
    else if (build_cs_camg<NC>(p)) { rc = allow_lds(k_build_cs<NC, true>, lds_build_cs<NC>(p, true)); if (!rc) rc = allow_lds(k_build_cs<NC, true, false, true>, lds_build_cs<NC>(p, true)); }
    else { rc = allow_lds(k_build_cs<NC, false>, lds_build_cs<NC>(p, false)); if (!rc) rc = allow_lds(k_build_cs<NC, false, false, true>, lds_build_cs<NC>(p, false)); }
    if (rc) return rc;
  }
  if (!use_cs || !build_cs_uglob<NC>(p)) {
    if ((rc = allow_lds(k_build<NC>, lds_build<NC>(p)))) return rc;
    if ((rc = allow_lds(k_build<NC, 0, true>, lds_build<NC>(p)))) return rc;
  } else if (p->eval_only) {
  }
  if (p->det_m) {
    if ((rc = allow_lds(k_build<NC, 3>, lds_build<NC>(p)))) return rc;
    if ((rc = allow_lds(k_build<NC, 5>, lds_build<NC>(p)))) return rc;
    if ((rc = allow_lds(k_build<NC, 8>, lds_build<NC>(p)))) return rc;
    if ((rc = allow_lds(k_tprep<NC, 3>, lds_tprep<NC>(p)))) return rc;
    if ((rc = allow_lds(k_tprep<NC, 5>, lds_tprep<NC>(p)))) return rc;
    if ((rc = allow_lds(k_tprep<NC, 8>, lds_tprep<NC>(p)))) return rc;
    if ((rc = allow_lds(k_tprep<NC, 3, false, false, LIN_FORM<NC>>, lds_tprep<NC>(p)))) return rc;
    if ((rc = allow_lds(k_tprep<NC, 5, false, false, LIN_FORM<NC>>, lds_tprep<NC>(p)))) return rc;
    if ((rc = allow_lds(k_tprep<NC, 8, false, false, LIN_FORM<NC>>, lds_tprep<NC>(p)))) return rc;
    if constexpr (NC == 6) {
      if ((rc = allow_lds(k_build<NC, 16>, lds_build<NC>(p)))) return rc;
      if ((rc = allow_lds(k_tprep<NC, 16>, lds_tprep<NC>(p)))) return rc;
      if ((rc = allow_lds(k_tprep<NC, 16, false, false, LIN_FORM<NC>>, lds_tprep<NC>(p)))) return rc;
    }
  }
  if ((rc = allow_lds(k_jv<NC, 1>, lds_jv(p, 1)))) return rc;
  if ((rc = allow_lds(k_jv<NC, 2>, lds_jv(p, 2)))) return rc;
  if ((rc = allow_lds(k_jv<NC, 1, true>, lds_jv(p, 1)))) return rc;
  if ((rc = allow_lds(k_jv<NC, 2, true>, lds_jv(p, 2)))) return rc;
  if ((rc = allow_lds(k_jv<NC, 1, false, LIN_FORM<NC>>, lds_jv(p, 1)))) return rc;
  if ((rc = allow_lds(k_jv<NC, 2, false, LIN_FORM<NC>>, lds_jv(p, 2)))) return rc;
  if ((rc = allow_lds(k_jv<NC, 1, true, LIN_FORM<NC>>, lds_jv(p, 1)))) return rc;
  if ((rc = allow_lds(k_jv<NC, 2, true, LIN_FORM<NC>>, lds_jv(p, 2)))) return rc;
  if ((rc = allow_lds(k_schur_reg3<NC, RegCfg<NC>::SPLIT, RegCfg<NC>::MINW>, Reg3Cfg<NC>::LDS_BYTES))) return rc;
  if ((rc = allow_lds(k_tprep<NC>, lds_tprep<NC>(p)))) return rc;
  if ((rc = allow_lds(k_tprep<NC, 0, true>, lds_tprep<NC>(p)))) return rc;
  if ((rc = allow_lds(k_tprep<NC, 0, false, true>, lds_tprep<NC>(p)))) return rc;
  if ((rc = allow_lds(k_tprep<NC, 0, true, true>, lds_tprep<NC>(p)))) return rc;
  if ((rc = allow_lds(k_tprep<NC, 0, false, false, LIN_FORM<NC>>, lds_tprep<NC>(p)))) return rc;
  if ((rc = allow_lds(k_tprep<NC, 0, true, false, LIN_FORM<NC>>, lds_tprep<NC>(p)))) return rc;
  if ((rc = allow_lds(k_tprep<NC, 0, false, true, LIN_FORM<NC>>, lds_tprep<NC>(p)))) return rc;
  if ((rc = allow_lds(k_tprep<NC, 0, true, true, LIN_FORM<NC>>, lds_tprep<NC>(p)))) return rc;
  if ((rc = allow_lds(k_backsub<NC>, lds_backsub(p)))) return rc;
  if ((rc = allow_lds(k_backsub<NC, true>, lds_backsub(p)))) return rc;
  if ((rc = allow_lds(k_backsub<NC, false, true>, lds_backsub(p)))) return rc;
  if ((rc = allow_lds(k_backsub<NC, true, true>, lds_backsub(p)))) return rc;
  {
    const char* e = std::getenv("CBA_BACKSUB_REC");
    p->backsub_rec = (NC == 6 || (e && e[0] == '1')) && !p->eval_only && !p->has_fragments && lds_backsub_rec<NC>(p) <= 150 * 1024 && !(e && e[0] == '0');
    if (p->backsub_rec) {
      if ((rc = allow_lds(k_backsub_rec<NC, false>, lds_backsub_rec<NC>(p)))) return rc;
      if ((rc = allow_lds(k_backsub_rec<NC, true>, lds_backsub_rec<NC>(p)))) return rc;
      if (!std::getenv("CBA_BACKSUB_WGS"))
        p->grid_backsub = std::max(1, std::min(p->n_chunks, p->cus * resident_per_cu(k_backsub_rec<NC, true>, lds_backsub_rec<NC>(p), 2)));
    }
  }
  {
    int per_cu = p->tab_global ? resident_per_cu(k_jv<NC, 1, true>, lds_jv(p, 1), 2) : resident_per_cu(k_jv<NC, 1>, lds_jv(p, 1), 2);
    if (const char* e = std::getenv("CBA_JV_WGS")) per_cu = std::max(1, std::min(std::atoi(e), 8));
    p->jv_grid = (int)std::max<long>(1, std::min<long>((p->N + BLOCK - 1) / BLOCK, (long)p->cus * per_cu));
    p->jv_grid = std::min(p->jv_grid, JV_ROWS);
  }
  if (p->n_heavy && (rc = allow_lds(k_heavy_schur<NC>, (size_t)p->ncp * 3 * sizeof(double) + (size_t)p->ncp * sizeof(int)))) return rc;
  if ((rc = allow_lds(k_chol_apply, (size_t)p->ncp * 8))) return rc;
  if ((rc = allow_lds(k_step_cam, (size_t)p->lay.ncp_pad * 8))) return rc;
  if (p->one_workgroup_solve() && (rc = allow_lds(k_small_solve<NC>, kSmallSolveLds))) return rc;
  return CBA_OK;
}


static void start_plan_task(cba_problem* p, const cba_options* opt, int n_cus, const int* hcam, const int* hps) {
  constexpr long kTwoStageObs = 500000;
  const char* plan_env = std::getenv("CBA_PLAN");
  bool plan_two_stage = p->N >= kTwoStageObs;
  if (plan_env && std::strcmp(plan_env, "swap") == 0) plan_two_stage = true;
  if (plan_env && (std::strcmp(plan_env, "full") == 0 || std::strcmp(plan_env, "cheap") == 0)) plan_two_stage = false;
  if ((opt && opt->deterministic) || p->schur_clock) plan_two_stage = false;
  Reg2Params prm = (p->nct == 9) ? reg2_params<9, Reg3Cfg<9>>(p) : reg2_params<6, Reg3Cfg<6>>(p);
  if (plan_env) prm.cheap = std::strcmp(plan_env, "cheap") == 0;
  p->plan_task = new PlanTask();
  {
    const int cus0 = n_cus > 0 ? n_cus : 256;
    const size_t tile_lds = (p->nct == 9) ? Reg3Cfg<9>::LDS_BYTES : Reg3Cfg<6>::LDS_BYTES;
    const int per_cu = std::min(std::max<int>(1, (int)((160 * 1024) / tile_lds)), (p->nct == 9) ? RegCfg<9>::PER_CU : RegCfg<6>::PER_CU);
    const int mb0 = (opt && opt->max_blocks > 0) ? opt->max_blocks : 2 * cus0;
    p->plan_max_blocks = std::min(cus0 * per_cu, std::max(mb0, cus0));
  }
  p->plan_task->start(prm, hcam, hps, plan_two_stage, p);
}

static int open_stream_and_mailbox(cba_problem* p, const MailLayout& mail) {
  {
    std::lock_guard<std::mutex> lock(g_pool_mu);
    DevicePool& pool = g_pool[p->device];
    if (!pool.streams.empty()) { p->stream = pool.streams.back(); pool.streams.pop_back(); }
    for (size_t i = 0; i < pool.mail.size(); ++i)
      if (pool.mail[i].second >= mail.total) {
        p->h_scal = pool.mail[i].first; p->mail_doubles = pool.mail[i].second;
        pool.mail.erase(pool.mail.begin() + (long)i);
        break;
      }
  }
  if (!p->stream) HIPCHK(hipStreamCreateWithFlags(&p->stream, hipStreamNonBlocking));
  if (!p->h_scal) {
    p->mail_doubles = std::max<size_t>(mail.total, MailLayout(96).total);
    HIPCHK(hipHostMalloc((void**)&p->h_scal, p->mail_doubles * sizeof(double), hipHostMallocMapped));
  }
  HIPCHK(hipHostGetDevicePointer((void**)&p->d_hscal, p->h_scal, 0));
  p->h_cam = p->h_scal + mail.cam; p->d_hcam = p->d_hscal + mail.cam;
  p->h_flags = reinterpret_cast<int*>(p->h_scal + mail.flags); p->d_hflags = reinterpret_cast<int*>(p->d_hscal + mail.flags);
  p->h_bcam = p->h_scal + mail.bcam; p->d_hbcam = p->d_hscal + mail.bcam;
  std::memset(p->h_scal, 0, mail.total * sizeof(double));
  return CBA_OK;
}

#define TRYS(e) do { const int rc_ = (e); if (rc_) return rc_; } while (0)

static int upload_observations(cba_problem* p, const double* obs_uv, const SortedObs& obs, const PointTables& tabs) {
  TRYS(dev_upload(p, &p->obs_cam, obs.cam)); TRYS(dev_upload(p, &p->obs_pt, obs.pt));
  TRYS(dev_upload(p, &p->order, obs.order)); TRYS(dev_upload(p, &p->pt_start, tabs.pt_start)); TRYS(dev_upload(p, &p->chunk_start, tabs.chunk_start));
  double* uv_raw = nullptr;
  TRYS(dev_upload(p, &uv_raw, obs_uv, (size_t)2 * p->N)); TRYS(dev_alloc(p, &p->obs_u, (size_t)p->N)); TRYS(dev_alloc(p, &p->obs_v, (size_t)p->N));
  hipLaunchKernelGGL(k_gather_uv, dim3((int)std::min<long>((p->N + 255) / 256, 2048)), dim3(256), 0, p->stream, (const double*)uv_raw, (const int*)p->order, p->N, p->obs_u, p->obs_v);
  return CBA_OK;
}

static int upload_det_plan(cba_problem* p, const HostDetPlan& plan) {
  unsigned char* dperm = nullptr; unsigned short* dcst = nullptr;
  TRYS(dev_upload(p, &dperm, plan.perm)); TRYS(dev_upload(p, &dcst, plan.cst));
  p->det_m = plan.det_m;
  p->det = DetPlan{dperm, dcst};
  return CBA_OK;
}

static int upload_cs_plan(cba_problem* p, const HostCsPlan& plan) {
  double *dcu = nullptr, *dcv = nullptr;
  int *dcc = nullptr, *dcp = nullptr, *dso = nullptr, *dp0 = nullptr, *dnp = nullptr, *dperm = nullptr;
  TRYS(dev_upload(p, &dperm, plan.cperm));
  TRYS(dev_alloc(p, &dcu, (size_t)p->N)); TRYS(dev_alloc(p, &dcv, (size_t)p->N)); TRYS(dev_alloc(p, &dcc, (size_t)p->N)); TRYS(dev_alloc(p, &dcp, (size_t)p->N));
  TRYS(dev_upload(p, &dso, plan.sc_obs)); TRYS(dev_upload(p, &dp0, plan.sc_p0)); TRYS(dev_upload(p, &dnp, plan.sc_np));
  hipLaunchKernelGGL(k_cs_fill, dim3(plan.n_sc), dim3(256), 0, p->stream, (const int*)dperm, (const int*)dso, (const int*)dp0, (const double*)p->obs_u, (const double*)p->obs_v,
                     (const int*)p->obs_cam, (const int*)p->obs_pt, dcu, dcv, dcc, dcp);
  p->cs = CsPlan{dcu, dcv, dcc, dcp, dso, dp0, dnp, plan.n_sc, plan.pmax};
  return CBA_OK;
}

static int upload_cameras(cba_problem* p, const double* cam_const, const CameraLayout& cams, const PointTables& tabs) {
  if (p->n_heavy) {
    TRYS(dev_upload(p, &p->heavy_pts, tabs.heavy)); TRYS(dev_upload(p, &p->heavy_frag, tabs.heavy_frag));
    TRYS(dev_alloc(p, &p->heavy_W, (size_t)p->n_heavy * p->ncp * 3));
  }
  TRYS(dev_upload(p, &p->cam_const, cam_const, (size_t)p->C * 12));
  TRYS(dev_upload(p, &p->cam_model, cams.model)); TRYS(dev_upload(p, &p->cam_np, cams.np)); TRYS(dev_upload(p, &p->cam_off, cams.off));
  TRYS(dev_upload(p, &p->param_cam, cams.param_cam)); TRYS(dev_upload(p, &p->param_loc, cams.param_loc));
  return CBA_OK;
}

static int alloc_vectors(cba_problem* p) {
  TRYS(dev_alloc(p, &p->tab, (size_t)p->C * CAMTAB_DOUBLES)); TRYS(dev_alloc(p, &p->tab_new, (size_t)p->C * CAMTAB_DOUBLES));
  for (double** v : {&p->x0, &p->x, &p->x_new, &p->g, &p->s, &p->sinv, &p->v1, &p->v2, &p->sinv2}) TRYS(dev_zeros(p, v, (size_t)p->lay.total()));
  for (double** v : {&p->sinv_state_c, &p->cam_diag, &p->cam_over1, &p->cam_over2, &p->lb_dev, &p->ub_dev, &p->sinv_state_c2, &p->cam_diag2})
    TRYS(dev_zeros(p, v, (size_t)p->lay.ncp_pad));
  TRYS(dev_zeros(p, &p->V, (size_t)6 * p->lay.Ppad));
  const int ustride = (p->nct == 9) ? UPack<9>::STRIDE : UPack<6>::STRIDE;
  TRYS(dev_alloc(p, &p->Upacked, (size_t)p->C * ustride + 128));
  return CBA_OK;
}

static int install_first_plan(cba_problem* p, bool plan_timing) {
  PlanTask& task = *p->plan_task;
  const auto t_wait = std::chrono::steady_clock::now();
  task.wait_stage(task.two_stage ? 1 : 2);
  if (plan_timing) {
    fprintf(stderr, "  plan: %s took %.3f s on its own threads, started before the uploads; waited %.3f s for it\n", task.two_stage ? "the cheap plan" : "dealt streams and codes",
            task.two_stage ? task.seconds_cheap : task.seconds, std::chrono::duration<double>(std::chrono::steady_clock::now() - t_wait).count());
    const Reg2Plan& made = task.two_stage ? task.cheap : task.plan;
    fprintf(stderr, "  plan: its phases: point runs %.4f s, jobs %.4f s, concatenation %.4f s (%.0f MB)\n", made.seconds_runs, made.seconds_jobs, made.seconds_concat,
            (made.obs.size() + made.codes.size()) * 4e-6);
  }
  if (task.two_stage ? task.rc_cheap : task.rc)
    return fail(CBA_ERR_UNSUPPORTED, "a world point has more observations inside one camera-group tile than a chunk of the pair plan holds (%d records)",
                (p->nct == 9) ? Reg3Cfg<9>::SCHUNK : Reg3Cfg<6>::SCHUNK);
  const int rc = install_reg2_plan(p, task.two_stage ? task.cheap : task.plan, task.prm);
  p->plan_is_cheap = task.two_stage || task.prm.cheap;
  return rc;
}

static int alloc_solver_buffers(cba_problem* p) {
  const int ncp = p->ncp, nct = p->nct;
  const long tot = p->lay.total();
  const int ustride = (nct == 9) ? UPack<9>::STRIDE : UPack<6>::STRIDE;
  const long w_build = (long)p->C * ustride;
  p->partial_width = w_build;
  p->partial_capacity = (size_t)std::max<long>((long)p->grid * w_build, (long)(p->tile_grid + p->tile_grid / 8 + 1) * std::max(p->tp.rep, 1) * p->tp.tile_elems);
  TRYS(dev_alloc(p, &p->partial, p->partial_capacity));
  TRYS(dev_alloc(p, &p->partial4, (size_t)PARTIAL4_ROWS * 4)); TRYS(dev_alloc(p, &p->partial1, (size_t)2048)); TRYS(dev_alloc(p, &p->partial_gmax, (size_t)2048)); TRYS(dev_alloc(p, &p->partial4b, (size_t)2048 * 4));
  TRYS(dev_zeros(p, &p->Sacc, (size_t)ncp * ncp + (size_t)B_SLICES * p->lay.ncp_pad));
  TRYS(dev_alloc(p, &p->tri, (size_t)ncp * (ncp + 1) / 2 + p->lay.ncp_pad));
  if (!p->eval_only) {
    TRYS(dev_alloc(p, &p->red, (size_t)p->G * p->tp.tile_elems));
    TRYS(dev_alloc(p, &p->Trec, (size_t)std::max<long>(p->N, 1) * ((nct == 9) ? SchurRec<9>::HREC : SchurRec<6>::HREC)));
    TRYS(dev_alloc(p, &p->partial_b, (size_t)p->grid * p->lay.ncp_pad));
  }
  TRYS(dev_alloc(p, &p->S, (size_t)ncp * ncp)); p->ldw = (ncp + 3) & ~3;
  if (p->want_chol_trace) TRYS(dev_alloc(p, &p->chol_trace, (size_t)((ncp + NB - 1) / NB + 2) * 8));
  TRYS(dev_alloc(p, &p->Lbuf, (size_t)(ncp + 1) * p->ldw));
  TRYS(dev_alloc(p, &p->Xinv, (size_t)chol_xinv_blocks((ncp + NB - 1) / NB) * NB * NB));
  TRYS(dev_zeros(p, &p->Tinv, (size_t)ncp * p->ldw));
  TRYS(dev_alloc(p, &p->rhs, (size_t)p->lay.ncp_pad));
  TRYS(dev_zeros(p, &p->scal, 64)); TRYS(dev_zeros(p, &p->flags, 8)); TRYS(dev_alloc(p, &p->xbuf, 128));
  p->spec_word = p->flags + 4;
  TRYS(dev_alloc(p, &p->fz, 8)); TRYS(dev_zeros(p, &p->V2, (size_t)6 * p->lay.Ppad)); TRYS(dev_zeros(p, &p->g2, (size_t)tot));
  TRYS(dev_alloc(p, &p->U2, (size_t)p->C * ustride + 128));
  return CBA_OK;
}

static int open_staging(cba_problem* p) {
  const size_t tot = (size_t)p->lay.total();
  {
    std::lock_guard<std::mutex> lock(g_pool_mu);
    DevicePool& pool = g_pool[p->device];
    for (size_t i = 0; i < pool.staging.size(); ++i)
      if (pool.staging[i].second >= tot && pool.staging[i].second <= 4 * tot + 4096) {
        p->h_vec = pool.staging[i].first; p->h_vec_doubles = pool.staging[i].second;
        pool.staging.erase(pool.staging.begin() + (long)i);
        break;
      }
  }
  HIPCHK(hipEventCreateWithFlags(&p->h_vec_sent, hipEventDisableTiming));
  if (!p->h_vec) {
    p->h_vec_doubles = tot;
    HIPCHK(hipHostMalloc((void**)&p->h_vec, p->h_vec_doubles * sizeof(double), hipHostMallocDefault));
  }
  return CBA_OK;
}
static int device_synchronize() { HIPCHK(hipDeviceSynchronize()); return CBA_OK; }
#undef TRYS

extern "C" {

int cba_create(const cba_problem_desc* d, const cba_options* opt, cba_problem** out) {
  if (!d || !out) return fail(CBA_ERR_INVALID, "cba_create: null argument");
  *out = nullptr;
  if (const int rc = validate_problem_desc(fail, d)) return rc;
  const double t_enter = std::chrono::duration<double>(std::chrono::steady_clock::now().time_since_epoch()).count();
  int ndev = 0;
  if (hipGetDeviceCount(&ndev) != hipSuccess || ndev <= 0)
    return fail(CBA_ERR_NO_DEVICE, "no HIP device available: the MI355X engine has no CPU fallback");
  int dev = (opt && opt->device_id >= 0) ? opt->device_id : 0;
  if (!(opt && opt->device_id >= 0)) (void)hipGetDevice(&dev);
  if (dev >= ndev) return fail(CBA_ERR_INVALID, "device %d requested, %d available", dev, ndev);
  HIPCHK(hipSetDevice(dev));
  int n_cus = 0;
  if (hipDeviceGetAttribute(&n_cus, hipDeviceAttributeMultiprocessorCount, dev) != hipSuccess) n_cus = 0;

  cba_problem* p = new cba_problem();
  p->device = dev;
  p->C = d->n_cams; p->P = d->n_points; p->N = d->n_obs;
  p->loss = d->loss; p->f_scale = d->f_scale;
  if (const char* e = std::getenv("CBA_REG_FINALIZE")) p->fuse_reg_finalize = e[0] != '0';
  if (const char* e = std::getenv("CBA_CHOL_EARLY")) p->chol_early = e[0] != '0';
  if (const char* e = std::getenv("CBA_CHOL_ENDS")) p->chol_ends = e[0] != '0';
  if (const char* e = std::getenv("CBA_CHOL_PAIR")) p->chol_pair = e[0] != '0';
  if (const char* e = std::getenv("CBA_LINEAR_PASS")) p->linear_pass = e[0] != '0';
  if (const char* e = std::getenv("CBA_SPEC_SKIP")) p->spec_skip = e[0] != '0';
  if (const char* e = std::getenv("CBA_SCALE_FUSED")) p->scale_fused = e[0] != '0';
  if (const char* e = std::getenv("CBA_SMALL_SOLVE")) p->small_solve_on = e[0] != '0';
#ifdef CBA_PROFILING
  p->schur_clock = std::getenv("CBA_SCHUR_CLOCK") != nullptr;
  p->want_chol_trace = std::getenv("CBA_CHOL_TRACE") != nullptr;
  if (std::getenv("CBA_STAMPS")) {
    const size_t n = (size_t)STAMP_SLOTS * STAMP_BLOCKS * STAMP_ROW;
    if (hipMalloc((void**)&p->stamps, n * sizeof(long long)) == hipSuccess) {
      (void)hipMemset(p->stamps, 0, n * sizeof(long long));
      (void)hipMemcpyToSymbol(HIP_SYMBOL(g_cba_stamps), &p->stamps, sizeof(p->stamps));
    }
  }
#endif
  int rc = CBA_OK;
#define TRY(e) do { rc = (e); if (rc) { cba_destroy(p); return rc; } } while (0)
  const bool deterministic = opt && opt->deterministic;

  CameraLayout cams;
  TRY(camera_layout(fail, d, cams));
  const int ncp = cams.ncp, nct = cams.nct;
  p->ncp = ncp; p->nct = nct;
  p->h_cam_off = cams.off; p->h_cam_np = cams.np;
  p->lay.ncp = ncp; p->lay.ncp_pad = cams.ncp_pad;
  p->lay.P = p->P; p->lay.Ppad = (p->P + 31) / 32 * 32;

  const bool plan_timing = plan_timing_on();
  auto t_now = []() { return std::chrono::duration<double>(std::chrono::steady_clock::now().time_since_epoch()).count(); };
  double t_mark = t_now();
  auto lap = [&](const char* what) { if (plan_timing) { const double t = t_now(); fprintf(stderr, "cba_create: %-28s %.6f s\n", what, t - t_mark); t_mark = t; } };
  SortedObs obs;
  PointTables tabs;
  {
    HostVec<int64_t> order(p->N), pstart((size_t)p->P + 1), cstart((size_t)p->N + 2);
    const int64_t nch = cba_host_plan(p->P, p->N, d->obs_pt, d->obs_cam, p->C, CHUNK, order.data(), pstart.data(), cstart.data());
    if (nch < 0) TRY((int)nch);
    p->n_chunks = (int)nch;
    lap("sort by point, chunk table");
    gather_sorted(p->N, d->obs_cam, d->obs_pt, order.data(), obs);
    TRY(point_tables(fail, p->P, pstart.data(), nch, cstart.data(), obs.pt.data(), CHUNK, HEAVY_OBS, tabs));
  }
  p->max_obs_per_point = tabs.max_obs_per_point;
  p->n_heavy = (int)tabs.heavy.size();
  p->h_heavy_pts = tabs.heavy;
  p->has_fragments = tabs.has_fragments;
  p->eval_only = opt && opt->evaluation_only != 0;
  choose_schur_groups(p);
  if (!p->eval_only) start_plan_task(p, opt, n_cus, obs.cam.data(), tabs.pt_start.data());

  TRY(open_stream_and_mailbox(p, MailLayout(ncp)));
  const int cus = n_cus > 0 ? n_cus : 256;
  p->cus = cus;
  const int max_blocks = (opt && opt->max_blocks > 0) ? opt->max_blocks : 2 * cus;
  p->grid = std::max(1, std::min(p->n_chunks, max_blocks));
  p->grid_backsub = std::max(1, std::min(p->n_chunks, 2 * cus));
  if (const char* e = std::getenv("CBA_BACKSUB_WGS")) p->grid_backsub = std::max(1, std::min(p->n_chunks, std::min(std::max(std::atoi(e), 1), 8) * cus));

  lap("reorder on host");
  upload_stage_acquire(p);
  TRY(upload_observations(p, d->obs_uv, obs, tabs));
  if (deterministic) {
    HostDetPlan det;
    TRY(det_plan(fail, p->C, nct, p->n_chunks, tabs.chunk_start.data(), obs.cam.data(), CHUNK, DET_ROUND, BLOCK, det));
    TRY(upload_det_plan(p, det));
  }
  TRY(dev_upload(p, &p->chunk_pts, tabs.chunk_pts));
  {
    const char* cs_env = std::getenv("CBA_BUILD_CS");
    HostCsPlan cs;
    cs_plan(!(cs_env && cs_env[0] == '0'), deterministic, p->C, p->N, p->n_chunks, tabs.chunk_start.data(), tabs.chunk_pts.data(), obs.cam.data(), p->grid,
            (nct == 9) ? 4096 : 2048, CHUNK, CS_MAX_PTS, cs);
    if (cs.n_sc) TRY(upload_cs_plan(p, cs));
  }
  TRY(upload_cameras(p, d->cam_const, cams, tabs));
  lap("upload observations");
  TRY(alloc_vectors(p));
  lap("allocate vectors");
  if (nct == 9) TRY(configure_kernels<9>(p)); else TRY(configure_kernels<6>(p));
  lap("reorder, upload, allocate");
  if (!p->eval_only) TRY(install_first_plan(p, plan_timing));
  lap("Schur plan (streams, pairs, upload)");
  TRY(alloc_solver_buffers(p));
  TRY(open_staging(p));
  lap("solver buffers");
  TRY(device_synchronize());
#undef TRY
  upload_stage_release(p);
  lap("device synchronize");
  if (p->plan_task) {
    if (p->plan_task->two_stage) {
      p->plan_task->hcam_keep = std::move(obs.cam);
      p->plan_task->hps_keep = std::move(tabs.pt_start);
    } else {
      drop_plan_task(p);
    }
  }
  if (plan_timing) fprintf(stderr, "cba_create: %.3f s in total\n", t_now() - t_enter);
  *out = p;
  return CBA_OK;
}

static int maybe_swap_plan(cba_problem* p, bool wait);

int cba_plan_wait(cba_problem* p) {
  if (!p) return fail(CBA_ERR_INVALID, "cba_plan_wait: null problem");
  HIPCHK(hipSetDevice(p->device));
  return maybe_swap_plan(p, true);
}

int cba_set_loss(cba_problem* p, int32_t loss, double f_scale) {
  if (!p) return fail(CBA_ERR_INVALID, "cba_set_loss: null problem");
  if (loss < CBA_LOSS_LINEAR || loss > CBA_LOSS_ARCTAN) return fail(CBA_ERR_INVALID, "cba_set_loss: unknown loss %d", loss);
  if (loss != CBA_LOSS_LINEAR && !(f_scale > 0.0)) return fail(CBA_ERR_INVALID, "cba_set_loss: f_scale must be positive");
  p->loss = loss; p->f_scale = f_scale;
  p->have_build = false;
  p->spec_valid = false; p->spec_enqueued = false; p->spec_scale_ready = false;
  return CBA_OK;
}

int cba_get_info(cba_problem* p, cba_info* o) {
  if (!p || !o) return fail(CBA_ERR_INVALID, "null argument");
  o->n_cams = p->C; o->n_points = p->P; o->n_cam_params = p->ncp; o->n_params = p->ncp + 3 * p->P; o->n_obs = p->N;
  o->n_chunks = p->n_chunks; o->grid_blocks = p->grid;
  o->plan_state = !p->plan_is_cheap ? 0 : (p->plan_task ? 1 : 2); o->plan_error = p->plan_error;
  o->schur_groups = p->G; o->schur_tiles = p->n_tiles; o->schur_grid = p->tile_grid; o->schur_stream_len = p->tile_stream_len; o->schur_pairs = p->n_pairs;
  o->max_obs_per_point = p->max_obs_per_point; o->device_bytes = p->device_bytes; o->n_heavy_points = p->n_heavy;
  {
    const bool cs = p->cs.n_sc && !p->det_m && !p->n_heavy;
    const bool camg = cs ? (p->nct == 6 ? build_cs_camg<6>(p) : build_cs_camg<9>(p)) : (p->nct == 6 ? build_camg<6>(p) : build_camg<9>(p));
    const bool uglob = cs && (p->nct == 6 ? build_cs_uglob<6>(p) : build_cs_uglob<9>(p));
    o->build_camg = (camg ? 1 : 0) | (p->tab_global ? 2 : 0) | (cs ? 4 : 0) | (uglob ? 8 : 0) | (p->backsub_rec ? 16 : 0) |
                    (p->con.n_con && p->con.small ? 32 : 0) | (p->one_workgroup_solve() ? 64 : 0);
  }
  o->spec_jv_skipped = p->spec_jv_skipped;
  return CBA_OK;
}

int cba_enable_timers(cba_problem* p, int32_t on) { if (!p) return fail(CBA_ERR_INVALID, "null"); p->timers_on = on != 0; return CBA_OK; }
int cba_reset_timers(cba_problem* p) {
  if (!p) return fail(CBA_ERR_INVALID, "null");
  (void)hipSetDevice(p->device);
  drain_timers(p);
  for (int t = 0; t < T_COUNT; ++t) { p->t_ms[t] = 0; p->t_calls[t] = 0; }
  return CBA_OK;
}
int cba_get_timers(cba_problem* p, double* ms, int64_t* calls) {
  if (!p) return fail(CBA_ERR_INVALID, "null");
  (void)hipSetDevice(p->device);
  drain_timers(p);
  for (int t = 0; t < T_COUNT; ++t) { if (ms) ms[t] = p->t_ms[t]; if (calls) calls[t] = p->t_calls[t]; }
  return CBA_OK;
}

}

static void pack_host(const cba_problem* p, const double* x_ref, double* v, double pad_value) {
  const VecLayout& L = p->lay;
  std::fill(v, v + L.total(), pad_value);
  for (int i = 0; i < L.ncp; ++i) v[i] = x_ref[i];
  const double* pts = x_ref + L.ncp;
  double* vx = v + L.ncp_pad;
  for (int q = 0; q < L.P; ++q) {
    vx[q] = pts[3 * q]; vx[L.Ppad + q] = pts[3 * q + 1]; vx[2 * L.Ppad + q] = pts[3 * q + 2];
  }
}
static void unpack_host(const cba_problem* p, const double* v, double* x_ref) {
  const VecLayout& L = p->lay;
  for (int i = 0; i < L.ncp; ++i) x_ref[i] = v[i];
  double* pts = x_ref + L.ncp;
  const double* vx = v + L.ncp_pad;
  for (int q = 0; q < L.P; ++q) {
    pts[3 * q] = vx[q]; pts[3 * q + 1] = vx[L.Ppad + q]; pts[3 * q + 2] = vx[2 * L.Ppad + q];
  }
}

static int launch_cam_prep(cba_problem* p, const double* xvec, double* tab) {
  ScopedTimer t(p, T_CAM_PREP);
  hipLaunchKernelGGL(k_cam_prep, dim3((p->C + 63) / 64), dim3(64), 0, p->stream, xvec, p->cam_const, p->cam_model,
                     p->cam_np, p->cam_off, p->C, tab);
  return CBA_OK;
}

static int launch_cost(cba_problem* p, const double* xvec, const double* tab, int slot, double* r_out, int* rows_out = nullptr) {
  const int grid = (int)std::min<long>((p->N + BLOCK - 1) / BLOCK, 1024);
  {
    ScopedTimer t(p, T_COST);
    auto launch = [&](auto kernel, double* r, const int* ord) {
      hipLaunchKernelGGL(kernel, dim3(grid), dim3(BLOCK), lds_cost(p), p->stream, p->obs_u, p->obs_v, p->obs_cam,
                         p->obs_pt, p->N, xvec, p->lay, tab, p->C, p->loss, p->f_scale, p->partial1, p->flags, r, ord);
    };
    if (r_out) { if (p->tab_global) launch(k_cost<true, true>, r_out, (const int*)p->order); else launch(k_cost<true>, r_out, (const int*)p->order); }
    else { if (p->tab_global) launch(k_cost<false, true>, (double*)nullptr, (const int*)nullptr); else launch(k_cost<false>, (double*)nullptr, (const int*)nullptr); }
  }
  ScopedTimer t(p, T_VECTOR);
  int rows = grid;
  if (p->con.n_con) {
    hipLaunchKernelGGL(k_con_eval<false>, dim3(p->con_grid), dim3(BLOCK), 0, p->stream, p->con, xvec, p->lay, p->loss, p->f_scale,
                       (double*)nullptr, p->partial1 + grid, p->flags, r_out ? r_out + 2 * p->N : (double*)nullptr);
    rows += p->con_grid;
  }
  if (rows_out) { *rows_out = rows; return CBA_OK; }
  hipLaunchKernelGGL(k_reduce_narrow<false>, dim3(1), dim3(BLOCK), 0, p->stream, p->partial1, rows, 1, p->scal + slot);
  return CBA_OK;
}

static bool fused_trial(const cba_problem* p, bool compact) { return compact && p->cs.n_sc && !p->det_m && !p->n_heavy && !p->con.n_con; }
template <int NC>
static bool scale_fusable(const cba_problem* p, bool compact) {
  return p->scale_fused && fused_trial(p, compact) && !p->bounds_on && !p->cam_scaled && ScaleFuse<NC>::cam_wgs(p->C) + ScaleFuse<NC>::pt_wgs(p->lay) <= 2048;
}

template <int NC>
static int run_build_into(cba_problem* p, const double* xvec, const double* tab, double* V, double* g, double* Upacked, int cost_slot,
                          const double* skip = nullptr, bool defer_exchange = false, bool compact = false, int flag_slot = 0,
                          const TrialSrc* trial = nullptr, const PubArgs* pub = nullptr, const ScaleArgs* scale = nullptr) {
  RoctxRange range("cba:build");
  {
    ScopedTimer t(p, T_BUILD);
    if (p->n_heavy)
      hipLaunchKernelGGL(k_zero_heavy, dim3((p->n_heavy + 63) / 64), dim3(64), 0, p->stream, p->heavy_pts, p->n_heavy, p->lay, V, 6,
                         g + p->lay.ncp_pad, 3);
    auto launch_build = [&](auto kernel) {
      hipLaunchKernelGGL(kernel, dim3(p->grid), dim3(BLOCK), lds_build<NC>(p), p->stream, p->obs_u, p->obs_v, p->obs_cam,
                         p->obs_pt, p->pt_start, p->chunk_start, p->chunk_pts, p->n_chunks, xvec, p->lay, tab, p->C, p->loss, p->f_scale,
                         V, g, p->partial, p->partial1, p->flags + flag_slot, skip, p->det);
    };
    if (p->cs.n_sc && !p->det_m && !p->n_heavy) {
      const TrialSrc tsrc = trial ? *trial : TrialSrc{};
      auto launch_cs = [&](auto kernel, size_t lds) {
        hipLaunchKernelGGL(kernel, dim3(p->grid), dim3(BLOCK), lds, p->stream, p->cs, xvec, p->lay, tab, p->C, p->loss, p->f_scale,
                           V, g, p->partial, p->partial1, p->flags + flag_slot, skip, tsrc);
      };
      if (build_cs_uglob<NC>(p)) {
        (void)hipMemsetAsync(p->partial, 0, (size_t)p->C * UPack<NC>::STRIDE * sizeof(double), p->stream);
        if (trial) launch_cs(k_build_cs<NC, true, true, true>, lds_build_cs<NC>(p, true, true));
        else launch_cs(k_build_cs<NC, true, true>, lds_build_cs<NC>(p, true, true));
      } else if (build_cs_camg<NC>(p)) {
        if (trial) launch_cs(k_build_cs<NC, true, false, true>, lds_build_cs<NC>(p, true));
        else launch_cs(k_build_cs<NC, true>, lds_build_cs<NC>(p, true));
      } else {
        if (trial) launch_cs(k_build_cs<NC, false, false, true>, lds_build_cs<NC>(p, false));
        else launch_cs(k_build_cs<NC, false>, lds_build_cs<NC>(p, false));
      }
    } else
    switch (p->det_m) {
      case 3: launch_build(k_build<NC, 3>); break;
      case 5: launch_build(k_build<NC, 5>); break;
      case 8: launch_build(k_build<NC, 8>); break;
      case 16: { if constexpr (NC == 6) launch_build(k_build<NC, 16>); } break;
      default:
        if (build_camg<NC>(p)) launch_build(k_build<NC, 0, true>); else launch_build(k_build<NC, 0>);
        break;
    }
  }
  {
    ScopedTimer t(p, T_BUILD_REDUCE);
    const int w = p->C * UPack<NC>::STRIDE;
    const int u_rows = (p->cs.n_sc && !p->det_m && !p->n_heavy && build_cs_uglob<NC>(p)) ? 1 : p->grid;
    if (scale) {
      using SF = ScaleFuse<NC>;
      const int rows = SF::cam_wgs(p->C) + (int)SF::pt_wgs(p->lay);
      hipLaunchKernelGGL((k_reduce_scale_pub<NC>), dim3(rows + (pub ? 1 : 0)), dim3(64, REDUCE_RY), 0, p->stream, (const double*)p->partial, u_rows, p->C, Upacked, g,
                         (const int*)p->cam_off, (const int*)p->cam_np, *scale, pub ? 1 : 0, pub ? *pub : PubArgs{});
      p->scale_rows = rows;
      if (!compact)
        hipLaunchKernelGGL(k_reduce_narrow<false>, dim3(1), dim3(BLOCK), 0, p->stream, p->partial1, p->grid, 1, p->scal + cost_slot);
      return CBA_OK;
    }
    if (compact) {
      if (pub)
        hipLaunchKernelGGL(k_reduce_rows_pub, dim3((w + 63) / 64 + 1), dim3(64, REDUCE_RY), 0, p->stream, (const double*)p->partial, u_rows, w, Upacked, g,
                           (const int*)p->cam_off, (const int*)p->cam_np, (int)UPack<NC>::STRIDE, (int)UPack<NC>::TRI, *pub);
      else
        hipLaunchKernelGGL(k_reduce_rows, dim3((w + 63) / 64), dim3(64, REDUCE_RY), 0, p->stream, p->partial, u_rows, w, Upacked, g,
                           (const int*)p->cam_off, (const int*)p->cam_np, (int)UPack<NC>::STRIDE, (int)UPack<NC>::TRI);
      return CBA_OK;
    }
    hipLaunchKernelGGL(k_reduce_rows, dim3((w + 63) / 64), dim3(64, REDUCE_RY), 0, p->stream, p->partial, u_rows, w, Upacked,
                       (double*)nullptr, (const int*)nullptr, (const int*)nullptr, 1, 0);
    int rho_rows = p->grid;
    if (p->con.n_con) {
      HIPCHK(hipMemsetAsync(p->con.cdiag, 0, (size_t)3 * p->lay.Ppad * sizeof(double), p->stream));
      if (p->n_con_orphan)
        hipLaunchKernelGGL(k_zero_heavy, dim3((p->n_con_orphan + 63) / 64), dim3(64), 0, p->stream, (const int*)p->con_orphan, p->n_con_orphan, p->lay,
                           g + p->lay.ncp_pad, 3, (double*)nullptr, 0);
      hipLaunchKernelGGL(k_con_eval<true>, dim3(p->con_grid), dim3(BLOCK), 0, p->stream, p->con, xvec, p->lay, p->loss, p->f_scale, g,
                         p->partial1 + p->grid, p->flags, (double*)nullptr);
      rho_rows += p->con_grid;
    }
    hipLaunchKernelGGL(k_reduce_narrow<false>, dim3(1), dim3(BLOCK), 0, p->stream, p->partial1, rho_rows, 1, p->scal + cost_slot);
    if (defer_exchange) return CBA_OK;
    int rc = allreduce_sum(p, Upacked, (size_t)w);
    if (rc) return rc;
    hipLaunchKernelGGL((k_unpack_camera_grad<NC>), dim3((p->C * NC + 255) / 256), dim3(256), 0, p->stream, Upacked,
                       p->cam_off, p->cam_np, p->C, g);
  }
  return CBA_OK;
}

template <int NC>
static int run_build(cba_problem* p, const ScaleArgs* scale = nullptr) {
  return run_build_into<NC>(p, p->x, p->tab, p->V, p->g, p->Upacked, 8, nullptr, false, false, 3, nullptr, nullptr, scale);
}

template <int NC>
static int run_jv(cba_problem* p, int nv, int* rows_out = nullptr, const double* xvec = nullptr, const double* tab = nullptr, const SpecSkip& skip = SpecSkip{}) {
  ScopedTimer t(p, T_JV);
  if (!xvec) { xvec = p->x; tab = p->tab; }
  const int grid = nv == 1 ? p->jv_grid : (int)std::min<long>((p->N + BLOCK - 1) / BLOCK, 1024);
  const int con_rows = p->con.n_con ? p->con_grid : 0;
  if (grid + con_rows > PARTIAL4_ROWS)
    return fail(CBA_ERR_UNSUPPORTED, "run_jv: %d rows of k_jv and %d of k_con_jv exceed the %d rows of partial4", grid, con_rows, PARTIAL4_ROWS);
  auto launch_jv = [&](auto kernel) {
    hipLaunchKernelGGL(kernel, dim3(grid), dim3(BLOCK), lds_jv(p, nv), p->stream, p->obs_u, p->obs_v, p->obs_cam, p->obs_pt,
                       p->N, xvec, p->lay, tab, p->cam_off, p->C, p->loss, p->f_scale, p->v1, p->v2, p->partial4, skip);
  };
  if (linear_pass_now<NC>(p)) {
    if (nv == 1) { if (p->tab_global) launch_jv(k_jv<NC, 1, true, LIN_FORM<NC>>); else launch_jv(k_jv<NC, 1, false, LIN_FORM<NC>>); }
    else { if (p->tab_global) launch_jv(k_jv<NC, 2, true, LIN_FORM<NC>>); else launch_jv(k_jv<NC, 2, false, LIN_FORM<NC>>); }
  } else if (nv == 1) { if (p->tab_global) launch_jv(k_jv<NC, 1, true>); else launch_jv(k_jv<NC, 1>); }
  else { if (p->tab_global) launch_jv(k_jv<NC, 2, true>); else launch_jv(k_jv<NC, 2>); }
  int rows = grid;
  if (con_rows) {
    if (nv == 1) hipLaunchKernelGGL(k_con_jv<1>, dim3(p->con_grid), dim3(BLOCK), 0, p->stream, p->con, p->lay, p->v1, p->v2, p->partial4 + 4 * grid);
    else hipLaunchKernelGGL(k_con_jv<2>, dim3(p->con_grid), dim3(BLOCK), 0, p->stream, p->con, p->lay, p->v1, p->v2, p->partial4 + 4 * grid);
    rows += con_rows;
  }
  if (rows_out) { *rows_out = rows; return CBA_OK; }
  hipLaunchKernelGGL(k_reduce_narrow<false>, dim3(1), dim3(BLOCK), 0, p->stream, p->partial4, rows, 4, p->scal + 12);
  return CBA_OK;
}

template <int NC>
static int run_lin_chain(cba_problem* p, bool scalars = true, bool compact = false, double radius = 0.0, bool defer_finish = false) {
  RoctxRange range("cba:linearize");
  p->spec_scale_ready = false; p->gnorm_mailed = false;
  bool scaled = false;
  if (!p->have_build) {
    const ScaleArgs sa{p->V, p->lay, p->first_scale ? 1 : 0, p->sinv, nullptr, p->x, p->g, p->v1, p->partial4b, p->partial_gmax};
    scaled = scale_fusable<NC>(p, compact);
    int rcb = run_build<NC>(p, scaled ? &sa : nullptr);
    if (rcb) return rcb;
    p->cost_pending = true;
    p->have_build = true;
    p->spec_valid = false;
  }
  if (compact && p->spec_valid) {
    p->spec_valid = false;
    if (defer_finish) {
      p->lf = LinFin{p->partial4b, p->partial_gmax, p->partial4, p->scale_rows, p->spec_rows_jv, radius, p->scal, p->fz};
      p->lf_pending = true;
      return CBA_OK;
    }
    ScopedTimer t(p, T_SCALE_SCALARS);
    hipLaunchKernelGGL(k_lin_finish, dim3(1), dim3(BLOCK), 0, p->stream, p->partial4b, p->partial_gmax, p->scale_rows, p->partial4, p->spec_rows_jv, radius,
                       p->scal, p->fz);
    return CBA_OK;
  }
  p->spec_valid = false;
  const long tot = p->lay.total();
  const int vg = vec_grid(tot);
  const bool bnd = defer_finish && p->bounds_on;
  if (bnd && !p->first_scale && !p->cam_scaled)
    HIPCHK(hipMemcpyAsync(p->sinv_state_c, p->sinv, (size_t)p->lay.ncp_pad * sizeof(double), hipMemcpyDeviceToDevice, p->stream));
  if (p->cam_scaled && !bnd)
    HIPCHK(hipMemcpyAsync(p->sinv, p->sinv_state_c, (size_t)p->lay.ncp_pad * sizeof(double), hipMemcpyDeviceToDevice, p->stream));
  p->cam_state_saved = false;
  {
    ScopedTimer t(p, T_SCALE_SCALARS);
    if (compact) {
      const BoundArgs ba = bnd ? BoundArgs{p->lb_dev, p->ub_dev, p->sinv_state_c, p->sinv_state_c, p->cam_diag} : BoundArgs{};
      if (bnd) p->cam_scaled = true;
      auto launch_sl = [&](auto kernel) {
        hipLaunchKernelGGL(kernel, dim3(vg), dim3(BLOCK), 0, p->stream, p->Upacked, p->V, p->param_cam, p->param_loc, p->lay,
                           p->first_scale ? 1 : 0, p->sinv, p->con.n_con ? (const double*)p->con.cdiag : (const double*)nullptr, p->x, p->g, p->v1,
                           p->partial4b, p->partial_gmax, (const double*)nullptr, ba);
      };
      if (!scaled) {
        if (bnd) launch_sl(k_scale_lin<NC, true>); else launch_sl(k_scale_lin<NC, false>);
        p->scale_rows = vg;
      }
      p->first_scale = false;
      int rows_jv = 0;
      int rcj = run_jv<NC>(p, 1, &rows_jv);
      if (rcj) return rcj;
      if (defer_finish) {
        p->lf = LinFin{p->partial4b, p->partial_gmax, p->partial4, p->scale_rows, rows_jv, radius, p->scal, p->fz};
        p->lf_pending = true;
        return CBA_OK;
      }
      hipLaunchKernelGGL(k_lin_finish, dim3(1), dim3(BLOCK), 0, p->stream, p->partial4b, p->partial_gmax, p->scale_rows, p->partial4, rows_jv, radius,
                         p->scal, p->fz);
      return CBA_OK;
    }
    hipLaunchKernelGGL((k_scale_update<NC>), dim3(vg), dim3(BLOCK), 0, p->stream, p->Upacked, p->V, p->param_cam, p->param_loc,
// ... 176 lines not shown
      fprintf(stderr, "%s phases, mean clocks per wave (%zu waves, %.1f trips, %.1f pair iterations each):", who, waves, sum[4] / wv, sum[5] / wv);
      for (int k = 0; k < 4; ++k) fprintf(stderr, "  %s %.0f", names[k], sum[k] / wv);
      fprintf(stderr, "  | in-loop total %.0f, wave lifetime mean %.0f max %.0f\n", (sum[0] + sum[1] + sum[2] + sum[3]) / wv, sum[6] / wv, tmax);
    };
    report("k_schur_reg3", [](size_t) { return true; });
    return CBA_OK;
  }
}
#endif

template <int NC>
static int run_newton_chain(cba_problem* p, double lam, const double* lam_dev, bool compact = false) {
  const int ncp = p->ncp;
  if (p->plan_task) {
    const int rcs = maybe_swap_plan(p, false);
    if (rcs) return rcs;
  }
  RoctxRange range("cba:damped_step");
  {
    RoctxRange r2("cba:schur");
    ScopedTimer t(p, T_SCHUR);
    {
      const bool linf = p->lf_pending;
      p->lf_pending = false;
      auto launch_tprep = [&](auto kernel) {
        hipLaunchKernelGGL(kernel, dim3(p->grid), dim3(BLOCK), lds_tprep<NC>(p), p->stream, p->obs_u, p->obs_v, p->obs_cam, p->obs_pt,
                           p->chunk_start, p->n_chunks, p->x, p->lay, p->tab, p->cam_off, p->C, p->loss, p->f_scale, lam, lam_dev, p->V, p->g,
                           p->sinv, p->Trec, p->partial_b, p->flags, p->det, linf ? p->lf : LinFin{});
      };
      if (linear_pass_now<NC>(p)) switch (p->det_m) {
        case 3: launch_tprep(k_tprep<NC, 3, false, false, LIN_FORM<NC>>); break;
        case 5: launch_tprep(k_tprep<NC, 5, false, false, LIN_FORM<NC>>); break;
        case 8: launch_tprep(k_tprep<NC, 8, false, false, LIN_FORM<NC>>); break;
        case 16: { if constexpr (NC == 6) launch_tprep(k_tprep<NC, 16, false, false, LIN_FORM<NC>>); } break;
        default:
          if (linf) { if (p->tab_global) launch_tprep(k_tprep<NC, 0, true, true, LIN_FORM<NC>>); else launch_tprep(k_tprep<NC, 0, false, true, LIN_FORM<NC>>); }
          else if (p->tab_global) launch_tprep(k_tprep<NC, 0, true, false, LIN_FORM<NC>>); else launch_tprep(k_tprep<NC, 0, false, false, LIN_FORM<NC>>);
          break;
      } else switch (p->det_m) {
        case 3: launch_tprep(k_tprep<NC, 3>); break;
        case 5: launch_tprep(k_tprep<NC, 5>); break;
        case 8: launch_tprep(k_tprep<NC, 8>); break;
        case 16: { if constexpr (NC == 6) launch_tprep(k_tprep<NC, 16>); } break;
        default:
          if (linf) { if (p->tab_global) launch_tprep(k_tprep<NC, 0, true, true>); else launch_tprep(k_tprep<NC, 0, false, true>); }
          else if (p->tab_global) launch_tprep(k_tprep<NC, 0, true>); else launch_tprep(k_tprep<NC, 0>);
          break;
      }
      ScopedTimer tpairs(p, T_SCHUR_PAIRS);
      constexpr int SP = RegCfg<NC>::SPLIT, MW = RegCfg<NC>::MINW;
#ifdef CBA_PROFILING
      if (p->schur_clock) {
        int rcc = run_pairs_clocked<NC>(p);
        if (rcc) return rcc;
      } else
#endif
      hipLaunchKernelGGL((k_schur_reg3<NC, SP, MW>), dim3(p->tile_grid), dim3(Reg3Cfg<NC>::LAUNCH_THREADS), Reg3Cfg<NC>::LDS_BYTES, p->stream, p->tp, p->Trec, p->partial, (const double*)p->tab);
    }
  }
  bool small_solve = false;
  const bool fold_in_finalize = !p->n_heavy && !p->con.n_con && !p->sharded();
  {
    ScopedTimer t(p, T_SCHUR_REDUCE);
    const bool fused_finalize = fold_in_finalize && !p->one_workgroup_solve() && p->fuse_reg_finalize;
    if (fused_finalize) {
      const int per = REG_REDUCE_Y_MAX / p->reg_reduce_y;
      const int tile_x = (p->gsz * p->gsz * NC * NC + 64 * per - 1) / (64 * per), fold_x = (p->gsz * NC * NC + 63) / 64, rhs_x = (p->lay.ncp_pad + 63) / 64;
      hipLaunchKernelGGL((k_reg_finalize<NC>), dim3(p->G * fold_x + rhs_x + p->n_tiles * tile_x), dim3(64, REG_REDUCE_Y_MAX), 0, p->stream, p->tp, p->tile_wg_begin, p->partial,
                         p->cam_off, p->cam_np, ncp, p->n_tiles, p->G, p->reg_reduce_y, fold_x, rhs_x, tile_x, (const double*)p->partial_b, p->grid, p->lay.ncp_pad, p->Upacked, p->g,
                         p->sinv, lam, lam_dev, p->cam_diag, p->S, p->rhs, p->Lbuf, p->ldw, chol_side_block(p, chol_side_d0((ncp + NB - 1) / NB)), chol_side_block(p, 0));
    } else {
      hipLaunchKernelGGL(k_reg_reduce, dim3(std::max((p->tp.tile_elems + 63) / 64, (p->lay.ncp_pad + 63) / 64), p->n_tiles + B_SLICES), dim3(64, p->reg_reduce_y), 0,
                         p->stream, p->tp, p->tile_wg_begin, p->partial, p->cam_off, p->cam_np, NC, ncp, p->Sacc, p->red, p->n_tiles,
                         (const double*)p->partial_b, p->grid, p->lay.ncp_pad, p->Sacc + (size_t)ncp * ncp);
      if (!fold_in_finalize)
        hipLaunchKernelGGL(k_reg_fold, dim3((p->gsz * NC * NC + 63) / 64, p->G), dim3(64), 0, p->stream, p->tp, p->red,
                           p->cam_off, p->cam_np, NC, ncp, p->Sacc);
      if (p->n_heavy)
        hipLaunchKernelGGL((k_heavy_schur<NC>), dim3(p->n_heavy), dim3(BLOCK), (size_t)ncp * 3 * sizeof(double) + (size_t)ncp * sizeof(int), p->stream,
                           p->heavy_pts, p->pt_start, p->obs_cam, p->cam_off, p->cam_np, ncp, p->Trec, p->tab, p->heavy_W, p->Sacc);
      if (p->con.n_con) {
        if (p->con.small)
          hipLaunchKernelGGL((k_con_schur_small<NC>), dim3(p->con.n_comp), dim3(BLOCK), (size_t)p->con.small_lds, p->stream, p->con, p->lay, lam, p->V, p->g,
                             p->sinv, p->Trec, p->tab, p->pt_start, p->obs_cam, p->cam_off, p->cam_np, ncp, p->Sacc, p->Sacc + (size_t)ncp * ncp, p->flags);
        else
          hipLaunchKernelGGL((k_con_schur<NC>), dim3(p->con.n_comp), dim3(BLOCK), 0, p->stream, p->con, p->lay, lam, p->V, p->g, p->sinv,
                             p->Trec, p->tab, p->pt_start, p->obs_cam, p->cam_off, p->cam_np, ncp, p->Sacc, p->Sacc + (size_t)ncp * ncp, p->flags);
      }
    }
    if (p->sharded()) {
      const size_t ntri = (size_t)ncp * (ncp + 1) / 2 + ncp;
      const int tg = (int)std::min<size_t>(((size_t)ncp * ncp + ncp + 255) / 256, 1024);
      hipLaunchKernelGGL(k_tri_pack, dim3(tg), dim3(256), 0, p->stream, p->Sacc, p->tri, ncp, 0, p->lay.ncp_pad);
      int rcs = allreduce_sum(p, p->tri, ntri);
      if (rcs) return rcs;
      hipLaunchKernelGGL(k_tri_pack, dim3(tg), dim3(256), 0, p->stream, p->Sacc, p->tri, ncp, 1, p->lay.ncp_pad);
    }
    const long nn = (long)ncp * ncp;
    small_solve = p->one_workgroup_solve();
    if (!small_solve && !fused_finalize) {
      hipLaunchKernelGGL((k_schur_finalize<NC>), dim3((int)((nn + 255) / 256)), dim3(256), 0, p->stream, p->Sacc,
                         p->Sacc + (size_t)ncp * ncp, p->Upacked, p->g, p->sinv, p->param_cam, p->param_loc, ncp, lam, lam_dev, p->cam_diag, p->S, p->rhs, p->Lbuf, p->ldw,
                         fold_in_finalize ? (const double*)p->red : (const double*)nullptr, p->tp.g, (long)p->tp.tile_elems, (const int*)p->tp.group_cam_begin,
                         p->lay.ncp_pad, chol_side_block(p, chol_side_d0((ncp + NB - 1) / NB)), chol_side_block(p, 0));
    }
  }
  int rc = CBA_OK;
  if (small_solve) {
    RoctxRange r2("cba:cholesky");
    ScopedTimer t(p, T_CHOLESKY);
    hipLaunchKernelGGL((k_small_solve<NC>), dim3(1), dim3(SMALL_THREADS), kSmallSolveLds, p->stream, p->Sacc, p->Sacc + (size_t)ncp * ncp, p->Upacked, p->g, p->sinv,
                       p->param_cam, p->param_loc, ncp, lam, lam_dev, p->cam_diag, p->S, p->rhs, fold_in_finalize ? (const double*)p->red : (const double*)nullptr,
                       p->tp.g, (long)p->tp.tile_elems, (const int*)p->tp.group_cam_begin, p->flags, p->s, p->lay.ncp_pad);
  } else {
    RoctxRange r2("cba:cholesky");
    rc = run_cholesky(p);
  }
  if (rc) return rc;
  {
    RoctxRange r2("cba:backsub");
    ScopedTimer t(p, T_BACKSUB);
    if (p->n_heavy)
      hipLaunchKernelGGL(k_zero_heavy, dim3((p->n_heavy + 63) / 64), dim3(64), 0, p->stream, p->heavy_pts, p->n_heavy, p->lay,
                         p->s + p->lay.ncp_pad, 3, p->s + p->lay.ncp_pad, 0);
    auto launch_backsub = [&](auto kernel) {
      hipLaunchKernelGGL(kernel, dim3(p->grid_backsub), dim3(BLOCK), lds_backsub(p), p->stream, p->obs_u, p->obs_v, p->obs_cam,
                         p->obs_pt, p->pt_start, p->chunk_start, p->chunk_pts, p->n_chunks, p->x, p->lay, p->tab, p->cam_off, p->C, p->loss,
                         p->f_scale, lam, lam_dev, p->V, p->g, p->sinv, p->s, p->partial4);
    };
    auto launch_backsub_rec = [&](auto kernel) {
      hipLaunchKernelGGL(kernel, dim3(p->grid_backsub), dim3(BLOCK), lds_backsub_rec<NC>(p), p->stream, (const double*)p->Trec, (const int*)p->obs_cam,
                         (const int*)p->pt_start, (const int*)p->chunk_start, (const int*)p->chunk_pts, p->n_chunks, p->lay, (const double*)p->tab,
                         (const int*)p->cam_off, (const int*)p->cam_np, p->C, lam, lam_dev, (const double*)p->V, (const double*)p->g,
                         (const double*)p->sinv, p->s, p->partial4);
    };
    if (p->backsub_rec) { if (fused_trial(p, compact)) launch_backsub_rec(k_backsub_rec<NC, true>); else launch_backsub_rec(k_backsub_rec<NC, false>); }
    else if (fused_trial(p, compact)) { if (p->tab_global) launch_backsub(k_backsub<NC, true, true>); else launch_backsub(k_backsub<NC, false, true>); }
    else if (p->tab_global) launch_backsub(k_backsub<NC, true>); else launch_backsub(k_backsub<NC>);
    if (p->n_heavy)
      hipLaunchKernelGGL(k_heavy_finish, dim3((p->n_heavy + 63) / 64), dim3(64), 0, p->stream, p->heavy_pts, p->heavy_frag, p->n_heavy, p->lay, lam,
                         p->V, p->g, p->sinv, p->s);
    if (p->con.n_con) {
      if (p->n_con_orphan)
        hipLaunchKernelGGL(k_con_orphan_start, dim3((p->n_con_orphan + 63) / 64), dim3(64), 0, p->stream, (const int*)p->con_orphan, p->n_con_orphan, p->lay,
                           lam, (const double*)p->V, (const double*)p->g, (const double*)p->sinv, p->s);
      if (p->con.small)
        hipLaunchKernelGGL(k_con_backsub_small, dim3(p->con.n_comp), dim3(BLOCK), (size_t)(9 * p->con.max_np + 2 * p->con.max_m) * sizeof(double), p->stream,
                           p->con, p->lay, lam, p->V, p->sinv, p->s);
      else
        hipLaunchKernelGGL(k_con_backsub, dim3(p->con.n_comp), dim3(BLOCK), 0, p->stream, p->con, p->lay, lam, p->V, p->sinv, p->s);
    }
  }
  if (fused_trial(p, compact)) {
    ScopedTimer t(p, T_VECTOR);
    hipLaunchKernelGGL(k_step_cam, dim3(1), dim3(BLOCK), (size_t)p->lay.ncp_pad * sizeof(double), p->stream, (const double*)p->partial4, p->grid_backsub,
                       (const double*)p->x, (const double*)p->g, (const double*)p->sinv, (const double*)p->s, p->lay.ncp_pad, p->scal, (const int*)p->flags, p->fz,
                       p->x_new, p->partial4 + p->grid, p->tab_new, (const double*)p->cam_const, (const int*)p->cam_model, (const int*)p->cam_np,
                       (const int*)p->cam_off, p->C, p->bounds_on ? (const double*)p->lb_dev : (const double*)nullptr,
                       p->bounds_on ? (const double*)p->ub_dev : (const double*)nullptr, p->ncp);
    return CBA_OK;
  }
  return run_step_scalars(p, lam_dev != nullptr, compact);
}

static void read_newton(cba_problem* p, cba_newton_info* out) {
  out->ok = (p->h_flags[1] == 0 && p->h_flags[2] == 0) ? 1 : 0;
  out->p_sq = p->h_scal[16];
  out->gh_dot_p = p->h_scal[17];
  out->w_sq = p->h_scal[20];
  if (out->ok && !(std::isfinite(out->p_sq) && std::isfinite(out->gh_dot_p) && std::isfinite(out->w_sq))) out->ok = 0;
}

template <int NC>
static int run_newton(cba_problem* p, double lam, cba_newton_info* out) {
  int rc = run_newton_chain<NC>(p, lam, nullptr);
  if (rc) return rc;
  rc = sync_scalars(p, 24);
  if (rc) return rc;
  read_newton(p, out);
  return CBA_OK;
}

template <int NC>
static int step_enqueue(cba_problem* p, double radius, bool compact, unsigned long long* seq_out) {
  int rc = run_lin_chain<NC>(p, true, compact, radius, compact && !p->det_m);
  if (rc) return rc;
  if (!compact) hipLaunchKernelGGL(k_fused_lam, dim3(1), dim3(1), 0, p->stream, p->scal, radius, p->fz);
  rc = run_newton_chain<NC>(p, 0.0, p->fz, compact);
  if (rc) return rc;
  if (!compact) hipLaunchKernelGGL(k_fused_subspace, dim3(1), dim3(1), 0, p->stream, p->scal, p->flags, p->fz);
  const long tot = p->lay.total();
  const int vg = vec_grid(tot);
  const bool ft = fused_trial(p, compact);
  if (!ft) {
    ScopedTimer t(p, T_VECTOR);
    hipLaunchKernelGGL(k_trial_update, dim3(vg), dim3(BLOCK), 0, p->stream, p->x, p->g, p->sinv, p->s, 0.0, 0.0, tot, p->lay.ncp_pad,
                       p->rank == 0 ? 1 : 0, (const double*)nullptr, 0, (const double*)(p->fz + 2), p->x_new, p->partial4, p->tab_new,
                       (const double*)p->cam_const, (const int*)p->cam_model, (const int*)p->cam_np, (const int*)p->cam_off, p->C);
    if (!compact) hipLaunchKernelGGL(k_reduce_narrow<false>, dim3(1), dim3(BLOCK), 0, p->stream, p->partial4, vg, 1, p->scal + 28);
  }
  const TrialSrc tsrc{p->x, p->g, p->sinv, p->s, p->fz + 2, p->x_new, p->partial4};
  const unsigned long long seq = compact ? ++p->publish_seq : 0;
  const bool bnd = compact && p->bounds_on;
  const bool last_trial = p->last_trial_hint;
  p->last_trial_hint = false;
  const bool spec_test = compact && p->spec_skip && p->tol_set && !p->bounds_on && !last_trial;
  const PubArgs pub{p->scal, 49, p->flags, p->d_hscal, p->d_hflags, seq, p->partial1, p->grid, 24, p->partial4, ft ? p->grid + 1 : vg, 28,
                    {p->x, p->g, p->sinv_state_c, p->s}, bnd ? p->d_hbcam : (double*)nullptr, p->ncp,
                    spec_test ? p->spec_word : (int*)nullptr, p->ftol, p->xtol, p->cost_pending ? NAN : p->cost_x};
  const bool sf = scale_fusable<NC>(p, compact);
  const ScaleArgs sa{p->V2, p->lay, 0, p->sinv2, p->sinv, p->x_new, p->g2, p->v1, p->partial4b, p->partial_gmax};
  rc = run_build_into<NC>(p, p->x_new, p->tab_new, p->V2, p->g2, p->U2, 24, p->scal + 42, true, compact, 0, ft ? &tsrc : nullptr,
                          compact ? &pub : nullptr, sf ? &sa : nullptr);
  if (rc) return rc;
  if (!compact) return CBA_OK;
  *seq_out = seq;
  p->spec_enqueued = false; p->spec_jv_enqueued = false;
  {
    if (!sf) {
      ScopedTimer t(p, T_SCALE_SCALARS);
      const BoundArgs ba2 = bnd ? BoundArgs{p->lb_dev, p->ub_dev, p->sinv_state_c, p->sinv_state_c2, p->cam_diag2} : BoundArgs{};
      auto launch_sl2 = [&](auto kernel) {
        hipLaunchKernelGGL(kernel, dim3(vg), dim3(BLOCK), 0, p->stream, p->U2, p->V2, p->param_cam, p->param_loc, p->lay, 0, p->sinv2,
                           (const double*)nullptr, p->x_new, p->g2, p->v1, p->partial4b, p->partial_gmax, (const double*)p->sinv, ba2);
      };
      if (bnd) launch_sl2(k_scale_lin<NC, true>); else launch_sl2(k_scale_lin<NC, false>);
      p->scale_rows = vg;
    }
    const SpecSkip skip{spec_test ? p->spec_word : (const int*)nullptr, p->partial_gmax, p->scale_rows, p->d_hscal, seq};
    p->gnorm_seq = seq;
    if (!(p->spec_skip && last_trial)) {
      int rows_jv = 0;
      rc = run_jv<NC>(p, 1, &rows_jv, p->x_new, p->tab_new, skip);
      p->spec_rows_jv = rows_jv;
      p->spec_jv_enqueued = true;
    } else {
      ScopedTimer t(p, T_SCALE_SCALARS);
      hipLaunchKernelGGL(k_gnorm_pub, dim3(1), dim3(BLOCK), 0, p->stream, skip);
    }
    if (rc) return rc;
    p->spec_enqueued = true;
  }
  return CBA_OK;
}

template <int NC>
static int run_step(cba_problem* p, double radius, cba_step_info* out) {
  RoctxRange range("cba:step");
  const bool compact = !p->sharded();
  int rc;
  if (compact) {
    unsigned long long seq = 0;
    rc = step_enqueue<NC>(p, radius, true, &seq);
    if (rc) return rc;
    rc = publish_wait(p, seq, !p->spec_enqueued);
  } else {
    unsigned long long seq = 0;
    rc = step_enqueue<NC>(p, radius, false, &seq);
    if (rc) return rc;
    rc = exchange_at(p, SLOT(24) | SLOT(28), false, p->U2, (size_t)p->C * UPack<NC>::STRIDE);
    if (rc) return rc;
    hipLaunchKernelGGL((k_unpack_camera_grad<NC>), dim3((p->C * NC + 255) / 256), dim3(256), 0, p->stream, p->U2, p->cam_off, p->cam_np, p->C, p->g2);
    rc = sync_scalars(p, 48);
  }
  if (rc) return rc;
  p->spec_jv_dropped = compact && p->h_scal[48] != 0.0;
  if (p->spec_jv_dropped) ++p->spec_jv_skipped;
  const int bad_residual = p->h_flags[0];
  read_linearization(p, &out->lin);
  read_newton(p, &out->newton);
  out->lam = p->h_scal[40]; out->radius = p->h_scal[41];
  out->need_host = (int)p->h_scal[42];
  out->p_s[0] = p->h_scal[43]; out->p_s[1] = p->h_scal[44]; out->predicted = p->h_scal[45];
  out->alpha = p->h_scal[46]; out->beta = p->h_scal[47];
  if (const char* e = std::getenv("CBA_TEST_FAIL_FUSED_STEP")) {
    static std::atomic<long> n_fused{0};
    if (++n_fused == std::atol(e)) {
      out->newton.ok = 0; out->need_host = 1;
      if (p->bounds_on) for (int i = 0; i < p->ncp; ++i) p->h_bcam[(size_t)3 * p->ncp + i] = NAN;
    }
  }
  const double c = 0.5 * p->h_scal[24];
  out->trial.finite = (bad_residual == 0 && std::isfinite(c)) ? 1 : 0;
  out->trial.cost = out->trial.finite ? c : NAN;
  out->trial.step_norm = std::sqrt(p->h_scal[28]);
  out->trial.reserved = 0;
  p->trial_cost = c;
  return CBA_OK;
}

template <int NC>
static int run_gradient_norm(cba_problem* p, double* out) {
  if (!p->spec_skip || p->sharded() || p->bounds_on || p->cam_scaled || p->eval_only) {
    cba_linearization lin;
    const int rc = run_linearize<NC>(p, &lin);
    if (rc) return rc;
    p->linearized = true; p->stepped = false;
    *out = lin.g_norm_inf;
    return CBA_OK;
  }
  if (p->spec_scale_ready && p->gnorm_mailed) {
    volatile unsigned long long* word = reinterpret_cast<volatile unsigned long long*>(p->h_scal) + MAIL_GNORM_SEQ;
    const auto t0 = std::chrono::steady_clock::now();
    for (unsigned spins = 0; *word != p->gnorm_seq; ++spins) {
      if ((spins & 0xfff) == 0xfff && std::chrono::steady_clock::now() - t0 > std::chrono::seconds(2)) {
        HIPCHK(hipStreamSynchronize(p->stream));
        if (*word != p->gnorm_seq) return fail(CBA_ERR_HIP, "the gradient norm of the accepted trial did not arrive");
        break;
      }
    }
    std::atomic_thread_fence(std::memory_order_acquire);
    *out = p->h_scal[MAIL_GNORM];
    return CBA_OK;
  }
  const int vg = vec_grid(p->lay.total());
  if (!p->spec_scale_ready) {
    if (!p->have_build) {
      const int rcb = run_build<NC>(p);
      if (rcb) return rcb;
      p->cost_pending = true; p->have_build = true;
    }
    p->spec_valid = false;
    ScopedTimer t(p, T_SCALE_SCALARS);
    hipLaunchKernelGGL((k_scale_lin<NC, false>), dim3(vg), dim3(BLOCK), 0, p->stream, p->Upacked, p->V, p->param_cam, p->param_loc, p->lay, p->first_scale ? 1 : 0,
                       p->sinv, p->con.n_con ? (const double*)p->con.cdiag : (const double*)nullptr, p->x, p->g, p->v1, p->partial4b, p->partial_gmax,
                       (const double*)nullptr, BoundArgs{});
    p->scale_rows = vg;
    p->first_scale = false;
    p->spec_scale_ready = true;
  }
  {
    ScopedTimer t(p, T_SCALE_SCALARS);
    hipLaunchKernelGGL(k_reduce_narrow<true>, dim3(1), dim3(BLOCK), 0, p->stream, p->partial_gmax, p->scale_rows, 1, p->scal + 4);
  }
  const int rc = sync_scalars(p, 16);
  if (rc) return rc;
  *out = p->h_scal[4];
  return CBA_OK;
}

#define DISPATCH_NC(p, call6, call9) ((p)->nct == 9 ? (call9) : (call6))

extern "C" {

static int begin_common(cba_problem* p, double* cost_out, bool evaluate = true);

int cba_set_constraints(cba_problem* p, int32_t n_con, const int32_t* groups_a, const int32_t* groups_b, const double* distances,
                        const double* weights) {
  if (!p) return fail(CBA_ERR_INVALID, "cba_set_constraints: null problem");
  if (p->begun) return fail(CBA_ERR_INVALID, "cba_set_constraints: call it before cba_begin");
  if (p->con.n_con) return fail(CBA_ERR_INVALID, "cba_set_constraints: constraints are already set");
  if (n_con <= 0) return CBA_OK;
  if (!groups_a || !groups_b || !distances || !weights) return fail(CBA_ERR_INVALID, "cba_set_constraints: null array");
  HIPCHK(hipSetDevice(p->device));
  const auto t_enter = std::chrono::steady_clock::now();
  auto lap_ms = [&](std::chrono::steady_clock::time_point since) { return std::chrono::duration<double, std::milli>(std::chrono::steady_clock::now() - since).count(); };
  HostConPlan plan;
  int rc = constraint_plan(fail, p->P, p->ncp, n_con, groups_a, groups_b, distances, weights, CON_LDS_POINTS, plan);
  if (rc) return rc;
  const int K = plan.n_comp, max_pts = plan.max_pts;
  const long max_m = plan.max_m;
  std::vector<int> orphan;
  {
    std::vector<int> hps((size_t)p->P + 1);
    HIPCHK(hipStreamSynchronize(p->stream));
    HIPCHK(hipMemcpy(hps.data(), p->pt_start, hps.size() * sizeof(int), hipMemcpyDeviceToHost));
// ... 39 lines not shown
  HIPCHK(hipStreamSynchronize(p->stream));
  upload_stage_release(p);
  if (plan_timing_on())
    fprintf(stderr, "  cba_set_constraints: %d rows, %d components: graph %.3f ms, uploads + allocations %.3f, kernel attributes %.3f, memset + sync %.3f\n", n_con, K,
            ms_graph, ms_upload, ms_attr, lap_ms(t_sync));
  p->con = cp;
  p->con_orphan = dorphan; p->n_con_orphan = (int)orphan.size();
  p->con_grid = std::max(1, std::min((n_con + BLOCK - 1) / BLOCK, CON_ROWS));
  return CBA_OK;
}

int cba_begin(cba_problem* p, const double* x0, double* cost_out) {
  if (!p || !x0 || !cost_out) return fail(CBA_ERR_INVALID, "cba_begin: null argument");
  HIPCHK(hipSetDevice(p->device));
  { const int rcw = stage_wait(p); if (rcw) return rcw; }
  pack_host(p, x0, p->h_vec, 0.0);
  HIPCHK(hipMemcpyAsync(p->x0, p->h_vec, p->lay.total() * sizeof(double), hipMemcpyHostToDevice, p->stream));
  { const int rcs = stage_sent(p); if (rcs) return rcs; }
  p->have_x0 = true;
  return begin_common(p, cost_out);
}

int cba_restart(cba_problem* p, double* cost_out) {
  if (!p || !cost_out) return fail(CBA_ERR_INVALID, "cba_restart: null argument");
  if (!p->have_x0) return fail(CBA_ERR_INVALID, "cba_restart: call cba_begin first");
  HIPCHK(hipSetDevice(p->device));
  return begin_common(p, cost_out);
}

int cba_begin_deferred(cba_problem* p, const double* x0) {
  if (!p) return fail(CBA_ERR_INVALID, "cba_begin_deferred: null argument");
  if (!x0 && !p->have_x0) return fail(CBA_ERR_INVALID, "cba_begin_deferred: no x0 on the device yet");
  HIPCHK(hipSetDevice(p->device));
  if (x0) {
    { const int rcw = stage_wait(p); if (rcw) return rcw; }
    pack_host(p, x0, p->h_vec, 0.0);
    HIPCHK(hipMemcpyAsync(p->x0, p->h_vec, p->lay.total() * sizeof(double), hipMemcpyHostToDevice, p->stream));
    { const int rcs = stage_sent(p); if (rcs) return rcs; }
    p->have_x0 = true;
  }
  return begin_common(p, nullptr, false);
}

static int begin_common(cba_problem* p, double* cost_out, bool evaluate) {
  p->cam_scaled = false; p->cam_state_saved = false;
  p->have_build = false; p->trial_built = false; p->cost_pending = false; p->lf_pending = false;
  p->spec_scale_ready = false; p->gnorm_mailed = false; p->tol_set = false; p->last_trial_hint = false;
  {
    ScopedTimer t(p, T_CAM_PREP);
    double* trial_buf = (!p->eval_only && fused_trial(p, true)) ? p->x_new : nullptr;
    hipLaunchKernelGGL(k_begin, dim3(std::max(vec_grid(p->lay.total()), (p->C + BLOCK - 1) / BLOCK)), dim3(BLOCK), 0, p->stream, (const double*)p->x0, p->x, trial_buf,
                       p->sinv, p->cam_diag, p->flags, p->lay.total(), p->lay.ncp_pad, (const double*)p->cam_const, (const int*)p->cam_model, (const int*)p->cam_np,
                       (const int*)p->cam_off, p->C, p->tab);
  }
  p->first_scale = true;
  p->begun = true; p->linearized = false; p->stepped = false; p->have_trial = false;
  if (!evaluate) {
    p->cost_x = NAN;
    return CBA_OK;
  }
  int rc = launch_cost(p, p->x, p->tab, 24, nullptr);
  if (rc) return rc;
  rc = exchange(p, SLOT(24), false);
  if (rc) return rc;
  rc = sync_scalars(p, 32);
  if (rc) return rc;
  HIPCHK(hipGetLastError());
  *cost_out = p->h_flags[0] ? NAN : 0.5 * p->h_scal[24];
  p->cost_x = *cost_out;
  return CBA_OK;
}

int cba_linearize(cba_problem* p, cba_linearization* out) {
  if (!p || !out) return fail(CBA_ERR_INVALID, "cba_linearize: null argument");
  if (p->eval_only) return fail(CBA_ERR_INVALID, "cba_linearize: the problem was created with evaluation_only");
  if (!p->begun) return fail(CBA_ERR_INVALID, "cba_linearize: call cba_begin first");
  HIPCHK(hipSetDevice(p->device));
  int rc = DISPATCH_NC(p, run_linearize<6>(p, out), run_linearize<9>(p, out));
  if (rc) return rc;
  HIPCHK(hipGetLastError());
  p->linearized = true; p->stepped = false;
  return CBA_OK;
}

int cba_linearize_build(cba_problem* p) {
  if (!p) return fail(CBA_ERR_INVALID, "cba_linearize_build: null argument");
  if (!p->begun) return fail(CBA_ERR_INVALID, "cba_linearize_build: call cba_begin first");
  if (p->eval_only) return fail(CBA_ERR_INVALID, "cba_linearize_build: the problem was created with evaluation_only");
  HIPCHK(hipSetDevice(p->device));
  int rc = DISPATCH_NC(p, run_lin_chain<6>(p, false), run_lin_chain<9>(p, false));
  if (rc) return rc;
  HIPCHK(hipGetLastError());
  p->linearized = true; p->stepped = false;
  return CBA_OK;
}

int cba_newton_step(cba_problem* p, double lam, cba_newton_info* out) {
  if (!p || !out) return fail(CBA_ERR_INVALID, "cba_newton_step: null argument");
  if (!p->linearized) return fail(CBA_ERR_INVALID, "cba_newton_step: call cba_linearize first");
  if (!(lam >= 0.0) || !std::isfinite(lam)) return fail(CBA_ERR_INVALID, "cba_newton_step: lam must be finite and >= 0");
  HIPCHK(hipSetDevice(p->device));
  int rc = DISPATCH_NC(p, run_newton<6>(p, lam, out), run_newton<9>(p, lam, out));
  if (rc) return rc;
  HIPCHK(hipGetLastError());
  p->stepped = true;
  return CBA_OK;
}

int cba_step(cba_problem* p, double radius, cba_step_info* out) {
  if (!p || !out) return fail(CBA_ERR_INVALID, "cba_step: null argument");
  if (!p->begun) return fail(CBA_ERR_INVALID, "cba_step: call cba_begin first");
  if (!cba_step_supported(p)) return fail(CBA_ERR_UNSUPPORTED, "cba_step: not available for this problem (constraint rows, heavy points, or bound scaling without cba_set_bounds): use the primitives");
  HIPCHK(hipSetDevice(p->device));
  int rc = DISPATCH_NC(p, run_step<6>(p, radius, out), run_step<9>(p, radius, out));
  if (rc) return rc;
  HIPCHK(hipGetLastError());
  p->linearized = true; p->stepped = true;
  p->have_trial = out->need_host == 0;
  p->trial_built = p->have_trial;
  return CBA_OK;
}

int cba_set_bounds(cba_problem* p, const double* lb, const double* ub) {
  if (!p) return fail(CBA_ERR_INVALID, "cba_set_bounds: null argument");
  if (!lb || !ub) { p->bounds_on = false; return 0; }
  if (p->eval_only || p->sharded() || !fused_trial(p, true)) { p->bounds_on = false; return 0; }
  HIPCHK(hipSetDevice(p->device));
  HIPCHK(hipMemcpyAsync(p->lb_dev, lb, (size_t)p->ncp * sizeof(double), hipMemcpyHostToDevice, p->stream));
  HIPCHK(hipMemcpyAsync(p->ub_dev, ub, (size_t)p->ncp * sizeof(double), hipMemcpyHostToDevice, p->stream));
  HIPCHK(hipStreamSynchronize(p->stream));
  p->bounds_on = true;
  return 1;
}

int cba_step_camera_state(cba_problem* p, double* x_c, double* g_c, double* scale_inv_c, double* step_c) {
  if (!p || !x_c || !g_c || !scale_inv_c || !step_c) return fail(CBA_ERR_INVALID, "cba_step_camera_state: null argument");
  if (!p->bounds_on || !p->stepped) return fail(CBA_ERR_INVALID, "cba_step_camera_state: no bounded cba_step to report on");
  const size_t n = (size_t)p->ncp;
  std::memcpy(x_c, p->h_bcam, n * sizeof(double)); std::memcpy(g_c, p->h_bcam + n, n * sizeof(double));
  std::memcpy(scale_inv_c, p->h_bcam + 2 * n, n * sizeof(double)); std::memcpy(step_c, p->h_bcam + 3 * n, n * sizeof(double));
  return CBA_OK;
}

int cba_refresh_step_scalars(cba_problem* p, cba_newton_info* out) {
  if (!p || !out) return fail(CBA_ERR_INVALID, "cba_refresh_step_scalars: null argument");
  if (!p->stepped) return fail(CBA_ERR_INVALID, "cba_refresh_step_scalars: no damped step to measure");
  HIPCHK(hipSetDevice(p->device));
  const int f1 = p->h_flags[1], f2 = p->h_flags[2];
  int rc = run_step_scalars(p, false);
  if (!rc) rc = sync_scalars(p, 24);
  if (rc) return rc;
  p->h_flags[1] = f1; p->h_flags[2] = f2;
  read_newton(p, out);
  return CBA_OK;
}

int cba_step_supported(cba_problem* p) {
  return (p && !p->eval_only && !p->con.n_con && !p->n_heavy && (!p->cam_scaled || (p->bounds_on && !p->sharded())) && !p->peer_needs_primitives) ? 1 : 0;
}

static int upload_cam(cba_problem* p, const double* host, double* dev) {
  HIPCHK(hipMemcpyAsync(dev, host, (size_t)p->ncp * sizeof(double), hipMemcpyHostToDevice, p->stream));
  return CBA_OK;
}

int cba_subspace_gram_ex(cba_problem* p, double a1, double b1, const double* cam1, double a2, double b2, const double* cam2,
                         double* gram_out) {
  if (!p || !gram_out) return fail(CBA_ERR_INVALID, "cba_subspace_gram: null argument");
  if (!p->stepped) return fail(CBA_ERR_INVALID, "cba_subspace_gram: call cba_newton_step first");
  HIPCHK(hipSetDevice(p->device));
  const long tot = p->lay.total();
  if (cam1) { int rc = upload_cam(p, cam1, p->cam_over1); if (rc) return rc; }
  if (cam2) { int rc = upload_cam(p, cam2, p->cam_over2); if (rc) return rc; }
  {
    ScopedTimer t(p, T_VECTOR);
    hipLaunchKernelGGL(k_combine, dim3(vec_grid(tot)), dim3(BLOCK), 0, p->stream, p->g, p->sinv, p->s, a1, b1, tot,
                       (const double*)p->cam_over1, cam1 ? p->lay.ncp_pad : 0, p->v1);
    hipLaunchKernelGGL(k_combine, dim3(vec_grid(tot)), dim3(BLOCK), 0, p->stream, p->g, p->sinv, p->s, a2, b2, tot,
                       (const double*)p->cam_over2, cam2 ? p->lay.ncp_pad : 0, p->v2);
  }
  DISPATCH_NC(p, run_jv<6>(p, 2), run_jv<9>(p, 2));
  int rc = exchange(p, SLOT(12) | SLOT(13) | SLOT(14) | SLOT(15), false);
  if (!rc) rc = sync_scalars(p, 16);
  if (rc) return rc;
  HIPCHK(hipGetLastError());
  gram_out[0] = p->h_scal[12]; gram_out[1] = p->h_scal[13]; gram_out[2] = p->h_scal[14];
  return CBA_OK;
}

int cba_subspace_gram(cba_problem* p, double a1, double b1, double a2, double b2, double* gram_out) {
  return cba_subspace_gram_ex(p, a1, b1, nullptr, a2, b2, nullptr, gram_out);
}

int cba_set_camera_scaling(cba_problem* p, const double* mult, const double* diag_h, cba_linearization* out) {
  if (!p || !mult || !diag_h || !out) return fail(CBA_ERR_INVALID, "cba_set_camera_scaling: null argument");
  if (!p->linearized) return fail(CBA_ERR_INVALID, "cba_set_camera_scaling: call cba_linearize first");
  for (int i = 0; i < p->ncp; ++i)
    if (!(mult[i] > 0.0) || !std::isfinite(mult[i]) || !(diag_h[i] >= 0.0) || !std::isfinite(diag_h[i]))
      return fail(CBA_ERR_INVALID, "cba_set_camera_scaling: entry %d: mult must be positive and diag_h non-negative (finite)", i);
  HIPCHK(hipSetDevice(p->device));
  const int npad = p->lay.ncp_pad;
  if (!p->cam_state_saved) {
    HIPCHK(hipMemcpyAsync(p->sinv_state_c, p->sinv, (size_t)npad * sizeof(double), hipMemcpyDeviceToDevice, p->stream));
    p->cam_state_saved = true;
  }
  int rc = upload_cam(p, mult, p->cam_over1);
  if (!rc) rc = upload_cam(p, diag_h, p->cam_over2);
  if (rc) return rc;
  const long tot = p->lay.total();
  const int vg = vec_grid(tot);
  {
    ScopedTimer t(p, T_SCALE_SCALARS);
    hipLaunchKernelGGL(k_cam_rescale, dim3((p->ncp + 255) / 256), dim3(256), 0, p->stream, p->sinv_state_c, p->cam_over1, p->cam_over2, p->ncp,
                       p->sinv, p->cam_diag);
    hipLaunchKernelGGL(k_lin_scalars, dim3(vg), dim3(BLOCK), 0, p->stream, p->x, p->g, p->sinv, tot, npad, p->rank == 0 ? 1 : 0, npad,
                       p->v1, p->partial4, p->partial1);
    hipLaunchKernelGGL(k_reduce_narrow<false>, dim3(1), dim3(BLOCK), 0, p->stream, p->partial4, vg, 4, p->scal + 0);
    hipLaunchKernelGGL(k_reduce_narrow<true>, dim3(1), dim3(BLOCK), 0, p->stream, p->partial1, vg, 1, p->scal + 4);
  }
  rc = DISPATCH_NC(p, run_jv<6>(p, 1), run_jv<9>(p, 1));
  if (rc) return rc;
  rc = exchange(p, SLOT(0) | SLOT(1) | SLOT(2) | SLOT(3) | SLOT(12) | SLOT(13) | SLOT(14) | SLOT(15), true);
  if (!rc) rc = sync_scalars(p, 16);
  if (rc) return rc;
  HIPCHK(hipGetLastError());
  p->cam_scaled = true; p->stepped = false;
  read_linearization(p, out);
  return CBA_OK;
}

int cba_trial(cba_problem* p, double alpha, double beta, cba_trial_info* out) { return cba_trial_ex(p, alpha, beta, nullptr, out); }

int cba_trial_ex(cba_problem* p, double alpha, double beta, const double* cam_x_new, cba_trial_info* out) {
  if (!p || !out) return fail(CBA_ERR_INVALID, "cba_trial: null argument");
  if (!p->stepped) return fail(CBA_ERR_INVALID, "cba_trial: call cba_newton_step first");
  HIPCHK(hipSetDevice(p->device));
  const long tot = p->lay.total();
  const int vg = vec_grid(tot);
  if (cam_x_new) { int rcu = upload_cam(p, cam_x_new, p->cam_over1); if (rcu) return rcu; }
  {
    ScopedTimer t(p, T_VECTOR);
    hipLaunchKernelGGL(k_trial_update, dim3(vg), dim3(BLOCK), 0, p->stream, p->x, p->g, p->sinv, p->s, alpha, beta, tot, p->lay.ncp_pad,
                       p->rank == 0 ? 1 : 0, (const double*)p->cam_over1, cam_x_new ? p->ncp : 0, (const double*)nullptr, p->x_new, p->partial4);
    if (p->sharded()) hipLaunchKernelGGL(k_reduce_narrow<false>, dim3(1), dim3(BLOCK), 0, p->stream, p->partial4, vg, 1, p->scal + 28);
  }
  launch_cam_prep(p, p->x_new, p->tab_new);
  int rc;
  if (p->sharded()) {
    rc = launch_cost(p, p->x_new, p->tab_new, 24, nullptr);
    if (rc) return rc;
    rc = exchange(p, SLOT(24) | SLOT(28), false);
    if (rc) return rc;
    rc = sync_scalars(p, 32);
  } else {
    int cost_rows = 0;
    rc = launch_cost(p, p->x_new, p->tab_new, 24, nullptr, &cost_rows);
    if (rc) return rc;
    rc = sync_scalars(p, 32, p->partial1, cost_rows, 24, p->partial4, vg, 28);
  }
  if (rc) return rc;
  HIPCHK(hipGetLastError());
  const double c = 0.5 * p->h_scal[24];
  out->finite = (p->h_flags[0] == 0 && std::isfinite(c)) ? 1 : 0;
  out->cost = out->finite ? c : NAN;
  out->step_norm = std::sqrt(p->h_scal[28]);
  p->have_trial = true; p->trial_built = false; p->trial_cost = c;
  return CBA_OK;
}

int cba_accept(cba_problem* p) {
  if (!p) return fail(CBA_ERR_INVALID, "cba_accept: null argument");
  if (!p->have_trial) return fail(CBA_ERR_INVALID, "cba_accept: no trial point");
  std::swap(p->x, p->x_new);
  std::swap(p->tab, p->tab_new);
  p->spec_valid = false; p->spec_scale_ready = false; p->gnorm_mailed = false;
  if (p->trial_built) {
    std::swap(p->V, p->V2); std::swap(p->g, p->g2); std::swap(p->Upacked, p->U2);
    p->cost_x = p->trial_cost;
    if (p->spec_enqueued) {
      std::swap(p->sinv, p->sinv2);
      if (p->bounds_on) { std::swap(p->sinv_state_c, p->sinv_state_c2); std::swap(p->cam_diag, p->cam_diag2); }
      p->spec_valid = p->spec_jv_enqueued && !p->spec_jv_dropped;
      p->spec_scale_ready = true;
      p->gnorm_mailed = !p->spec_valid;
    }
  }
  p->spec_enqueued = false;
  p->have_build = p->trial_built;
  p->trial_built = false;
  p->have_trial = false; p->linearized = false; p->stepped = false;
  return CBA_OK;
}

int cba_set_tolerances(cba_problem* p, double ftol, double xtol) {
  if (!p) return fail(CBA_ERR_INVALID, "cba_set_tolerances: null argument");
  if (!(ftol >= 0.0) || !(xtol >= 0.0)) return fail(CBA_ERR_INVALID, "cba_set_tolerances: the tolerances must be >= 0");
  p->ftol = ftol; p->xtol = xtol; p->tol_set = true;
  return CBA_OK;
}

int cba_hint_last_trial(cba_problem* p) {
  if (!p) return fail(CBA_ERR_INVALID, "cba_hint_last_trial: null argument");
  p->last_trial_hint = true;
  return CBA_OK;
}

// ... 315 lines not shown
```

### caliscope_amd/csrc/trf_math.h

```cpp
#pragma once
#include <math.h>

#ifdef __HIPCC__
#define TRF_HD __host__ __device__
#else
#define TRF_HD
#endif

namespace trf {

TRF_HD inline double min_quadratic_on_segment(double a, double b, double hi) {
  double best = fmin(0.0, hi * (a * hi + b));
  if (a != 0.0) {
    const double t = -0.5 * b / a;
    if (t > 0.0 && t < hi) best = fmin(best, t * (a * t + b));
  }
  return best;
}

constexpr double DAMPING_FLOOR = 1e-13;
TRF_HD inline double damping(double H_gg, double gh_sq, double radius) {
  const double lam = -min_quadratic_on_segment(0.5 * H_gg, -gh_sq, radius / sqrt(gh_sq)) / (radius * radius);
  return lam > DAMPING_FLOOR ? lam : DAMPING_FLOOR;
}

TRF_HD inline double poly_eval(const double* c, int deg, double t) {
  double p = c[0];
  for (int i = 1; i <= deg; ++i) p = p * t + c[i];
  return p;
}

template <int DEG>
TRF_HD inline int real_roots_of_degree(const double* c, double* out) {
  static_assert(DEG >= 1 && DEG <= 4, "quartics at most");
  if constexpr (DEG == 1) {
    out[0] = -c[1] / c[0];
    return 1;
  } else if constexpr (DEG == 2) {
    const double disc = c[1] * c[1] - 4.0 * c[0] * c[2];
    if (disc < 0.0) return 0;
    const double q = -0.5 * (c[1] + copysign(sqrt(disc), c[1]));
    int n = 0;
    if (q != 0.0) { out[n++] = q / c[0]; out[n++] = c[2] / q; }
    else { out[n++] = 0.0; }
    return n;
  } else {
    double d[DEG], crit[DEG - 1];
    for (int i = 0; i < DEG; ++i) d[i] = c[i] * (DEG - i);
    int nc = real_roots_of_degree<DEG - 1>(d, crit);
    for (int i = 1; i < nc; ++i)
      for (int j = i; j > 0 && crit[j] < crit[j - 1]; --j) { const double t = crit[j]; crit[j] = crit[j - 1]; crit[j - 1] = t; }
    double bound = 0.0;
    for (int i = 1; i <= DEG; ++i) bound = fmax(bound, fabs(c[i] / c[0]));
    bound += 1.0;
    double knots[DEG + 1];
    int nk = 0;
    knots[nk++] = -bound;
    for (int i = 0; i < nc; ++i)
      if (crit[i] > -bound && crit[i] < bound) knots[nk++] = crit[i];
    knots[nk++] = bound;
    int n = 0;
    double scale = 0.0;
    for (int i = 0; i <= DEG; ++i) scale = fmax(scale, fabs(c[i]));
    for (int k = 0; k + 1 < nk; ++k) {
      double a = knots[k], b = knots[k + 1];
      double fa = poly_eval(c, DEG, a), fb = poly_eval(c, DEG, b);
      if (fa == 0.0) { out[n++] = a; continue; }
      if (k + 2 == nk && fb == 0.0) { out[n++] = b; continue; }
      if ((fa < 0.0) == (fb < 0.0)) {
        if (k > 0 && fabs(fa) <= 1e-14 * scale * fmax(1.0, pow(fabs(a), (double)DEG))) out[n++] = a;
        continue;
      }
      for (int it = 0; it < 200 && b - a > 0.0; ++it) {
        const double m = 0.5 * (a + b);
        if (m == a || m == b) break;
        const double fm = poly_eval(c, DEG, m);
        if (fm == 0.0) { a = b = m; break; }
        if ((fm < 0.0) == (fa < 0.0)) { a = m; fa = fm; } else { b = m; }
      }
      out[n++] = 0.5 * (a + b);
      if (n >= DEG) break;
    }
    return n;
  }
}

TRF_HD inline int real_roots(const double* c_in, int n_coef, double* out) {
  int lead = 0;
  while (lead < n_coef && c_in[lead] == 0.0) ++lead;
  switch (n_coef - 1 - lead) {
    case 4: return real_roots_of_degree<4>(c_in + lead, out);
    case 3: return real_roots_of_degree<3>(c_in + lead, out);
    case 2: return real_roots_of_degree<2>(c_in + lead, out);
    case 1: return real_roots_of_degree<1>(c_in + lead, out);
    default: return 0;
  }
}

TRF_HD inline void solve_subspace_2d(double b00, double b01, double b11, double g0, double g1, double radius, double* p) {
  if (b00 > 0.0) {
    const double schur = b11 - b01 * b01 / b00;
    if (schur > 0.0) {
      const double det = b00 * schur;
      const double p0 = -(b11 * g0 - b01 * g1) / det, p1 = -(b00 * g1 - b01 * g0) / det;
      if (p0 * p0 + p1 * p1 <= radius * radius) { p[0] = p0; p[1] = p1; return; }
    }
  }
  const double r2 = radius * radius;
  const double a = b00 * r2, b = b01 * r2, c = b11 * r2, d = g0 * radius, f = g1 * radius;
  const double coef[5] = {-b + d, 2.0 * (a - c + f), 6.0 * b, 2.0 * (-a + c + f), -b - d};
  double t[4];
  const int nt = real_roots(coef, 5, t);
  if (nt == 0) {
    const double n = hypot(g0, g1);
    p[0] = n > 0 ? -radius * g0 / n : 0.0;
    p[1] = n > 0 ? -radius * g1 / n : 0.0;
    return;
  }
  double best = INFINITY;
  for (int i = 0; i <= nt; ++i) {
    double c0, c1;
    if (i < nt) { const double q = 1.0 + t[i] * t[i]; c0 = radius * 2.0 * t[i] / q; c1 = radius * (1.0 - t[i] * t[i]) / q; }
    else { c0 = 0.0; c1 = -radius; }
    const double val = 0.5 * (c0 * (b00 * c0 + b01 * c1) + c1 * (b01 * c0 + b11 * c1)) + g0 * c0 + g1 * c1;
    if (val < best) { best = val; p[0] = c0; p[1] = c1; }
  }
}

TRF_HD inline void subspace_model(double H_gg, double gh_sq, double lam, double gh_dot_p, double p_sq, double w_sq, double* b00,
                                  double* b01, double* b11) {
  const double c = gh_dot_p / gh_sq, gh_norm = sqrt(gh_sq), w_norm = sqrt(w_sq);
  const double H_gp = -gh_sq - lam * gh_dot_p, H_pp = -gh_dot_p - lam * p_sq;
  *b00 = H_gg / gh_sq;
  *b01 = (H_gp - c * H_gg) / (gh_norm * w_norm);
  *b11 = (H_pp - 2.0 * c * H_gp + c * c * H_gg) / w_sq;
}

TRF_HD inline double reduction_ratio(double actual, double predicted) {
  if (predicted > 0.0) return actual / predicted;
  if (predicted == 0.0 && actual == 0.0) return 1.0;
  return 0.0;
}

constexpr int TERMINATION_NONE = -100;
TRF_HD inline int termination(double dF, double F, double dx_norm, double x_norm, double ratio, double ftol, double xtol) {
  const bool f_ok = dF < ftol * F && ratio > 0.25;
  const bool x_ok = dx_norm < xtol * (xtol + x_norm);
  if (f_ok && x_ok) return 4;
  if (f_ok) return 2;
  if (x_ok) return 3;
  return TERMINATION_NONE;
}

}
```

Before: 4.004 billion obs/s.

## Fold trial-step computation and subspace solve into the build kernel prologue

Moves the trial-step work (the step-norm reductions, the 2D trust-region subspace solve, the camera table preparation for the trial point, and the camera x_new update) into the prologue of the trial build kernel, in place of the separate k_step_cam launch. Every block redundantly reduces the partials and solves the subspace problem, and block 0 writes the shared outputs. The quartic root finding is split per interval across wave lanes. This is meant to remove a kernel launch and a serial dependency on the critical path. In exchange, each block repeats the small reductions and camera preparation. A verify mode compares the folded results against the reference path.

```diff
diff --git a/caliscope_amd/csrc/cba_kernels.h b/caliscope_amd/csrc/cba_kernels.h
--- a/caliscope_amd/csrc/cba_kernels.h
+++ b/caliscope_amd/csrc/cba_kernels.h
@@ -598,15 +598,26 @@
   double* x_new;
   double* step_partial;
 };
-template <int NC, bool CAMG = false, bool UGLOB = false, bool TRIAL = false>
+struct StepFold {
+  const double* partial; int rows;
+  int ncp_pad;
+  double* scal; const int* flags; double* fz;
+  double* step_cam;
+  double* tab_out;
+  const double* cam_const; const int* cam_model; const int* cam_np; const int* cam_off;
+};
+__device__ __forceinline__ bool step_fold_prologue(const StepFold& f, const TrialSrc& trial, double* sh_tab, int n_cams, double* alpha, double* beta);
+
+template <int NC, bool CAMG = false, bool UGLOB = false, bool TRIAL = false, bool FOLD = false>
 __global__ void __launch_bounds__(BLOCK)
 k_build_cs(CsPlan cs, const double* __restrict__ xvec, VecLayout lay, const double* __restrict__ tab, int n_cams, int loss, double f_scale,
            double* __restrict__ Vblk, double* __restrict__ gvec, double* __restrict__ partialU, double* __restrict__ partial_cost,
-           int* __restrict__ flags, const double* __restrict__ skip, TrialSrc trial = TrialSrc{}) {
+           int* __restrict__ flags, const double* __restrict__ skip, TrialSrc trial = TrialSrc{}, StepFold fold = StepFold{}) {
   CBA_STAMP(ST_BUILD);
   using UP = UPack<NC>;
   static_assert(!UGLOB || CAMG, "a camera count beyond the LDS copy of the blocks is beyond the LDS copy of the table as well");
-  if (skip && *skip != 0.0) return;
+  static_assert(!FOLD || (TRIAL && !CAMG), "the folded step prepares the trial point's camera table in LDS");
+  if (!FOLD && skip && *skip != 0.0) return;
   extern __shared__ __attribute__((aligned(16))) double sh[];
   double* sh_tab = sh;
   double* sh_U = sh_tab + (CAMG ? 0 : n_cams * CAMTAB_LDS);
@@ -614,13 +625,18 @@
   double* sh_vg = sh_U + (UGLOB ? 0 : n_cams * UP::STRIDE);
   double* sh_x = sh_vg + 9 * PM;
   double* sh_red = sh_x + 3 * PM;
-  if (!CAMG) stage_camtab(sh_tab, tab, n_cams);
+  double t_alpha = 0.0, t_beta = 0.0;
+  if constexpr (FOLD) {
+    if (!step_fold_prologue(fold, trial, sh_tab, n_cams, &t_alpha, &t_beta)) return;
+  } else {
+    if (!CAMG) stage_camtab(sh_tab, tab, n_cams);
+    if (TRIAL) { t_alpha = trial.ab[0]; t_beta = trial.ab[1]; }
+  }
   if (!UGLOB)
     for (int i = threadIdx.x; i < n_cams * UP::STRIDE; i += BLOCK) sh_U[i] = 0.0;
   const double* px = xvec + lay.ncp_pad;
   double* gp = gvec + lay.ncp_pad;
   double cost = 0.0, step_sq = 0.0;
-  const double t_alpha = TRIAL ? trial.ab[0] : 0.0, t_beta = TRIAL ? trial.ab[1] : 0.0;
   bool bad = false;
   for (int s = blockIdx.x; s < cs.n_sc; s += gridDim.x) {
     const int o0 = cs.obs_start[s], o1 = cs.obs_start[s + 1], p0 = cs.pt_first[s], npts = cs.pt_count[s];
@@ -726,7 +742,7 @@
   __syncthreads();
   if (!UGLOB) {
     for (int c = threadIdx.x; c < n_cams; c += BLOCK) {
-      const double* Jl = tab + (long)c * CAMTAB_DOUBLES + 12;
+      const double* Jl = FOLD ? cam_at(sh_tab, c).Jl : tab + (long)c * CAMTAB_DOUBLES + 12;
       double* Uc = sh_U + (long)c * UP::STRIDE;
       double M[3][3], T[3][3];
 #pragma unroll
@@ -3054,31 +3070,40 @@
 __device__ __forceinline__ SubspaceIn subspace_inputs(const double* __restrict__ scal, const int* __restrict__ flags, const double* __restrict__ fz) {
   return SubspaceIn{scal[0], scal[3], scal[12], fz[0], fz[1], flags[1], flags[2]};
 }
-__device__ __forceinline__ void fused_subspace(double* __restrict__ scal, const int* __restrict__ flags, double* __restrict__ fz, const SubspaceIn* pre) {
-  const SubspaceIn in = pre ? *pre : subspace_inputs(scal, flags, fz);
-  const double gh_sq = in.gh_sq, jg_sq = in.jg + in.c_gg, p_sq = scal[16], ghp = scal[17];
+struct SubspaceOut { double w_sq, need_host, pS[2], predicted, alpha, beta; };
+template <class Roots>
+__device__ __forceinline__ SubspaceOut subspace_step(const SubspaceIn& in, double p_sq, double ghp, const Roots& roots) {
+  const double gh_sq = in.gh_sq, jg_sq = in.jg + in.c_gg;
   const double lam = in.lam, radius = in.radius, gh_norm = sqrt(gh_sq);
   const double c = ghp / gh_sq;
-  const double w_sq = p_sq - ghp * ghp / gh_sq;
-  scal[20] = w_sq;
+  SubspaceOut o{p_sq - ghp * ghp / gh_sq, 0.0, {0.0, 0.0}, 0.0, 0.0, 0.0};
+  const double w_sq = o.w_sq;
   const bool two_d = true;
-  double need_host = 0.0, pS[2] = {0.0, 0.0}, alpha = 0.0, beta = 0.0, predicted = 0.0;
   const bool ok = in.f1 == 0 && in.f2 == 0 && isfinite(p_sq) && isfinite(ghp) && gh_sq > 0.0;
   if (!ok || !(w_sq > 1e-3 * p_sq)) {
-    need_host = 1.0;
+    o.need_host = 1.0;
   } else {
     double b00, b01 = 0.0, b11;
     const double w_norm = two_d ? sqrt(w_sq) : 1.0;
     if (two_d) trf::subspace_model(jg_sq, gh_sq, lam, ghp, p_sq, w_sq, &b00, &b01, &b11);
     else { b00 = jg_sq / gh_sq; b11 = 1.0; }
-    trf::solve_subspace_2d(b00, b01, b11, gh_norm, 0.0, radius, pS);
+    double* pS = o.pS;
+    trf::solve_subspace_2d(b00, b01, b11, gh_norm, 0.0, radius, pS, roots);
     if (!two_d) pS[1] = 0.0;
-    predicted = -(0.5 * (pS[0] * (b00 * pS[0] + b01 * pS[1]) + pS[1] * (b01 * pS[0] + b11 * pS[1])) + gh_norm * pS[0]);
-    beta = two_d ? pS[1] / w_norm : 0.0;
-    alpha = pS[0] / gh_norm - beta * c;
-  }
-  fz[2] = alpha; fz[3] = beta;
-  scal[42] = need_host; scal[43] = pS[0]; scal[44] = pS[1]; scal[45] = predicted; scal[46] = alpha; scal[47] = beta;
+    o.predicted = -(0.5 * (pS[0] * (b00 * pS[0] + b01 * pS[1]) + pS[1] * (b01 * pS[0] + b11 * pS[1])) + gh_norm * pS[0]);
+    o.beta = two_d ? pS[1] / w_norm : 0.0;
+    o.alpha = pS[0] / gh_norm - o.beta * c;
+  }
+  return o;
+}
+__device__ __forceinline__ void subspace_store(const SubspaceOut& o, double* __restrict__ scal, double* __restrict__ fz) {
+  scal[20] = o.w_sq;
+  fz[2] = o.alpha; fz[3] = o.beta;
+  scal[42] = o.need_host; scal[43] = o.pS[0]; scal[44] = o.pS[1]; scal[45] = o.predicted; scal[46] = o.alpha; scal[47] = o.beta;
+}
+__device__ __forceinline__ void fused_subspace(double* __restrict__ scal, const int* __restrict__ flags, double* __restrict__ fz, const SubspaceIn* pre) {
+  const SubspaceIn in = pre ? *pre : subspace_inputs(scal, flags, fz);
+  subspace_store(subspace_step(in, scal[16], scal[17], trf::SerialRoots{}), scal, fz);
 }
 
 
@@ -3369,6 +3394,15 @@
   }
 }
 
+__device__ __forceinline__ void cam_prepare_opaque(double* xc, double* cc, int model, int np, CamTab* t, int off) {
+#pragma unroll
+  for (int i = 0; i < MAX_NC; ++i) asm volatile("" : "+v"(xc[i]));
+#pragma unroll
+  for (int i = 0; i < CAM_CONST_STRIDE; ++i) asm volatile("" : "+v"(cc[i]));
+  asm volatile("" : "+v"(model), "+v"(np));
+  cam_prepare(xc, cc, model, np, t, off);
+}
+
 __global__ void __launch_bounds__(BLOCK)
 k_step_cam(const double* __restrict__ partial, int rows, const double* __restrict__ x, const double* __restrict__ g, const double* __restrict__ sinv,
            const double* __restrict__ s, int ncp_pad, double* __restrict__ scal, const int* __restrict__ flags, double* __restrict__ fz,
@@ -3466,11 +3500,166 @@
     const int np = mine ? my_np : cam_np[c], off = mine ? my_off : cam_off[c];
     for (int i = 0; i < MAX_NC; ++i) xc[i] = (i < np) ? sh_xc[off + i] : 0.0;
     CamTab t;
-    if (mine) cam_prepare(xc, my_const, my_model, np, &t, off);
-    else cam_prepare(xc, cam_const + c * CAM_CONST_STRIDE, cam_model[c], np, &t, off);
+    double cc[CAM_CONST_STRIDE];
+#pragma unroll
+    for (int i = 0; i < CAM_CONST_STRIDE; ++i) cc[i] = mine ? my_const[i] : cam_const[c * CAM_CONST_STRIDE + i];
+    cam_prepare_opaque(xc, cc, mine ? my_model : cam_model[c], np, &t, off);
     const double* src = reinterpret_cast<const double*>(&t);
     for (int i = 0; i < CAMTAB_DOUBLES; ++i) tab_out[c * CAMTAB_DOUBLES + i] = src[i];
   }
+}
+
+struct WaveLanes {
+  template <int DEG>
+  __device__ __forceinline__ void run(const double* c, const double* knots, int nk, double scale, int* kind, double* root) const {
+    const int lane = threadIdx.x & (WAVE - 1);
+    double kn[DEG + 1];
+#pragma unroll
+    for (int i = 0; i <= DEG; ++i) { kn[i] = knots[i]; asm volatile("" : "+v"(kn[i])); }
+    double a = kn[0], b = kn[1];
+#pragma unroll
+    for (int i = 1; i < DEG; ++i) { a = (lane == i) ? kn[i] : a; b = (lane == i) ? kn[i + 1] : b; }
+    int kd = trf::PIECE_NONE;
+    double r = 0.0;
+    if (lane + 1 < nk) kd = trf::piece_root<DEG>(c, a, b, nk, scale, lane, &r);
+#pragma unroll
+    for (int k = 0; k < DEG; ++k) { kind[k] = __shfl(kd, k); root[k] = __shfl(r, k); }
+  }
+};
+
+__device__ __forceinline__ double trial_entry(double alpha, double beta, double xi, double gi, double si, double stp, double* st) {
+  *st = alpha * gi / (si * si) + beta * stp;
+  return xi + *st;
+}
+
+__device__ __forceinline__ bool step_fold_prologue(const StepFold& f, const TrialSrc& trial, double* sh_tab, int n_cams, double* alpha_out, double* beta_out) {
+  __shared__ double sh_fold[3][BLOCK / WAVE];
+  __shared__ double sh_ab[3];
+  const double* __restrict__ x = trial.x;
+  const double* __restrict__ g = trial.g;
+  const double* __restrict__ sinv = trial.sinv;
+  const double* __restrict__ s = trial.s;
+  const int ncp_pad = f.ncp_pad, lane = threadIdx.x & (WAVE - 1), w = threadIdx.x / WAVE;
+  SubspaceIn pre{};
+  if (w == 0) pre = subspace_inputs(f.scal, f.flags, f.fz);
+  constexpr int KEEP = 2;
+  double kx[KEEP], kg[KEEP], ksi[KEEP], ks[KEEP];
+#pragma unroll
+  for (int q = 0; q < KEEP; ++q) {
+    const int i = threadIdx.x + q * BLOCK;
+    const bool in = i < ncp_pad;
+    kx[q] = in ? x[i] : 0.0; kg[q] = in ? g[i] : 0.0; ksi[q] = in ? sinv[i] : 1.0; ks[q] = in ? s[i] : 0.0;
+  }
+  const int my_cam = threadIdx.x < n_cams ? (int)threadIdx.x : -1;
+  int my_np = 0, my_off = 0, my_model = 0;
+  if (my_cam >= 0) { my_np = f.cam_np[my_cam]; my_off = f.cam_off[my_cam]; my_model = f.cam_model[my_cam]; }
+  double v[2] = {0.0, 0.0};
+  for (int b = threadIdx.x; b < f.rows; b += BLOCK) { v[0] += f.partial[(long)b * 4 + 0]; v[1] += f.partial[(long)b * 4 + 1]; }
+#pragma unroll
+  for (int q = 0; q < KEEP; ++q) {
+    const double ps = ks[q] * ksi[q];
+    v[0] = fma(ps, ps, v[0]);
+    v[1] = fma(kg[q], ks[q], v[1]);
+  }
+  for (int i = threadIdx.x + KEEP * BLOCK; i < ncp_pad; i += BLOCK) {
+    const double si = s[i], ps = si * sinv[i];
+    v[0] = fma(ps, ps, v[0]);
+    v[1] = fma(g[i], si, v[1]);
+  }
+#pragma unroll
+  for (int j = 0; j < 2; ++j) {
+    const double r = wave_sum(v[j]);
+    if (lane == 0) sh_fold[j][w] = r;
+  }
+  __syncthreads();
+  if (w == 0) {
+    double r[2];
+#pragma unroll
+    for (int j = 0; j < 2; ++j) {
+      r[j] = 0.0;
+      for (int i = 0; i < BLOCK / WAVE; ++i) r[j] += sh_fold[j][i];
+    }
+    const SubspaceOut o = subspace_step(pre, r[0], r[1], trf::PiecesRoots<WaveLanes>{});
+    if (lane == 0) {
+      sh_ab[0] = o.alpha; sh_ab[1] = o.beta; sh_ab[2] = o.need_host;
+      if (blockIdx.x == 0) {
+        f.scal[16] = r[0]; f.scal[17] = r[1]; f.scal[18] = 0.0; f.scal[19] = 0.0;
+        subspace_store(o, f.scal, f.fz);
+      }
+    }
+  }
+  __syncthreads();
+  const double alpha = sh_ab[0], beta = sh_ab[1];
+  *alpha_out = alpha; *beta_out = beta;
+  if (sh_ab[2] != 0.0) {
+    if (threadIdx.x == 0) { trial.step_partial[blockIdx.x] = 0.0; if (blockIdx.x == 0) f.step_cam[0] = 0.0; }
+    return false;
+  }
+  for (int c = threadIdx.x; c < n_cams; c += BLOCK) {
+    const bool mine = c == my_cam;
+    const int np = mine ? my_np : f.cam_np[c], off = mine ? my_off : f.cam_off[c], model = mine ? my_model : f.cam_model[c];
+    double xc[MAX_NC], cc[CAM_CONST_STRIDE];
+#pragma unroll
+    for (int i = 0; i < CAM_CONST_STRIDE; ++i) cc[i] = f.cam_const[c * CAM_CONST_STRIDE + i];
+#pragma unroll
+    for (int i = 0; i < MAX_NC; ++i) {
+      const int e = off + min(i, max(np - 1, 0));
+      double st;
+      const double xn = trial_entry(alpha, beta, x[e], g[e], sinv[e], s[e], &st);
+      xc[i] = (i < np) ? xn : 0.0;
+    }
+    CamTab t;
+    cam_prepare_opaque(xc, cc, model, np, &t, off);
+    const double* src = reinterpret_cast<const double*>(&t);
+#pragma unroll
+    for (int i = 0; i < CAMTAB_LIVE; ++i) sh_tab[c * CAMTAB_LDS + i] = src[i];
+    if (blockIdx.x == 0)
+      for (int i = 0; i < CAMTAB_DOUBLES; ++i) f.tab_out[c * CAMTAB_DOUBLES + i] = src[i];
+  }
+  if (blockIdx.x == 0) {
+    double s0 = 0.0;
+    auto entry = [&](int i, double xi, double gi, double si, double stp) {
+      double st;
+      trial.x_new[i] = trial_entry(alpha, beta, xi, gi, si, stp, &st);
+      s0 = fma(st, st, s0);
+    };
+#pragma unroll
+    for (int q = 0; q < KEEP; ++q)
+      if ((int)threadIdx.x + q * BLOCK < ncp_pad) entry(threadIdx.x + q * BLOCK, kx[q], kg[q], ksi[q], ks[q]);
+    for (int i = threadIdx.x + KEEP * BLOCK; i < ncp_pad; i += BLOCK) entry(i, x[i], g[i], sinv[i], s[i]);
+    const double r = wave_sum(s0);
+    if (lane == 0) sh_fold[2][w] = r;
+    __syncthreads();
+    if (threadIdx.x == 0) {
+      double tot = 0.0;
+      for (int i = 0; i < BLOCK / WAVE; ++i) tot += sh_fold[2][i];
+      f.step_cam[0] = tot;
+    }
+  }
+  return true;
+}
+
+__global__ void __launch_bounds__(BLOCK)
+k_step_fold_compare(const double* __restrict__ scal, const double* __restrict__ fz, const double* __restrict__ x_new, const double* __restrict__ tab,
+                    const double* __restrict__ step_cam, const double* __restrict__ scal_ref, const double* __restrict__ fz_ref,
+                    const double* __restrict__ x_ref, const double* __restrict__ tab_ref, const double* __restrict__ step_ref, int ncp_pad, int n_cams,
+                    unsigned long long* __restrict__ count) {
+  auto differ = [](double a, double b) { return __double_as_longlong(a) != __double_as_longlong(b); };
+  unsigned long long bad[5] = {0, 0, 0, 0, 0};
+  const int t = threadIdx.x;
+  if (t < 64 && ((t >= 16 && t <= 20) || (t >= 42 && t <= 47)) && differ(scal[t], scal_ref[t])) ++bad[0];
+  if ((t == 2 || t == 3) && differ(fz[t], fz_ref[t])) ++bad[1];
+  if (scal_ref[42] == 0.0) {
+    if (t == 0 && differ(step_cam[0], step_ref[0])) ++bad[2];
+    for (int i = t; i < ncp_pad; i += BLOCK) if (differ(x_new[i], x_ref[i])) ++bad[3];
+    for (int i = t; i < n_cams * CAMTAB_LIVE; i += BLOCK) {
+      const int e = (i / CAMTAB_LIVE) * CAMTAB_DOUBLES + i % CAMTAB_LIVE;
+      if (differ(tab[e], tab_ref[e])) ++bad[4];
+    }
+  }
+#pragma unroll
+  for (int q = 0; q < 5; ++q) if (bad[q]) atomicAdd(&count[1 + q], bad[q]);
+  if (t == 0) atomicAdd(&count[0], 1ull);
 }
 
 __global__ void __launch_bounds__(BLOCK)
diff --git a/caliscope_amd/csrc/cba_lib.hip b/caliscope_amd/csrc/cba_lib.hip
--- a/caliscope_amd/csrc/cba_lib.hip
+++ b/caliscope_amd/csrc/cba_lib.hip
@@ -112,6 +112,10 @@
   bool linear_pass = true;
   bool chol_pair = true;
   bool chol_early = true;
+  bool step_fold_verify = false;
+  double* fold_ref = nullptr;
+  unsigned long long* fold_count = nullptr;
+  bool step_fold = true;
   bool fuse_reg_finalize = true;
   double* scal = nullptr;
   double* xbuf = nullptr;
@@ -959,7 +963,8 @@
   if (use_cs) {
     if (build_cs_uglob<NC>(p)) { rc = allow_lds(k_build_cs<NC, true, true>, lds_build_cs<NC>(p, true, true)); if (!rc) rc = allow_lds(k_build_cs<NC, true, true, true>, lds_build_cs<NC>(p, true, true)); }
     else if (build_cs_camg<NC>(p)) { rc = allow_lds(k_build_cs<NC, true>, lds_build_cs<NC>(p, true)); if (!rc) rc = allow_lds(k_build_cs<NC, true, false, true>, lds_build_cs<NC>(p, true)); }
-    else { rc = allow_lds(k_build_cs<NC, false>, lds_build_cs<NC>(p, false)); if (!rc) rc = allow_lds(k_build_cs<NC, false, false, true>, lds_build_cs<NC>(p, false)); }
+    else { rc = allow_lds(k_build_cs<NC, false>, lds_build_cs<NC>(p, false)); if (!rc) rc = allow_lds(k_build_cs<NC, false, false, true>, lds_build_cs<NC>(p, false));
+           if (!rc) rc = allow_lds(k_build_cs<NC, false, false, true, true>, lds_build_cs<NC>(p, false)); }
     if (rc) return rc;
   }
   if (!use_cs || !build_cs_uglob<NC>(p)) {
@@ -1218,6 +1223,8 @@
   p->C = d->n_cams; p->P = d->n_points; p->N = d->n_obs;
   p->loss = d->loss; p->f_scale = d->f_scale;
   if (const char* e = std::getenv("CBA_REG_FINALIZE")) p->fuse_reg_finalize = e[0] != '0';
+  if (const char* e = std::getenv("CBA_STEP_FOLD")) p->step_fold = e[0] != '0';
+  if (const char* e = std::getenv("CBA_TEST_STEP_FOLD_VERIFY")) p->step_fold_verify = e[0] != '0';
   if (const char* e = std::getenv("CBA_CHOL_EARLY")) p->chol_early = e[0] != '0';
   if (const char* e = std::getenv("CBA_CHOL_ENDS")) p->chol_ends = e[0] != '0';
   if (const char* e = std::getenv("CBA_CHOL_PAIR")) p->chol_pair = e[0] != '0';
@@ -1434,9 +1441,35 @@
 }
 
 template <int NC>
+static bool step_folds(const cba_problem* p, bool compact) {
+  return p->step_fold && fused_trial(p, compact) && !p->bounds_on && !build_cs_uglob<NC>(p) && !build_cs_camg<NC>(p) &&
+         (size_t)4 * p->grid_backsub + p->grid + 1 <= (size_t)4 * PARTIAL4_ROWS;
+}
+
+static int enqueue_step_fold_verify(cba_problem* p, const StepFold& f, const TrialSrc& tr) {
+  const size_t n_ref = 72 + (size_t)p->lay.ncp_pad + (size_t)p->C * CAMTAB_DOUBLES;
+  if (!p->fold_ref) {
+    int rc = dev_alloc(p, &p->fold_ref, n_ref);
+    if (!rc) rc = dev_alloc(p, &p->fold_count, (size_t)6);
+    if (rc) return rc;
+    HIPCHK(hipMemsetAsync(p->fold_count, 0, 6 * sizeof(unsigned long long), p->stream));
+  }
+  double *scal_ref = p->fold_ref, *fz_ref = scal_ref + 64, *step_ref = fz_ref + 4, *x_ref = step_ref + 4, *tab_ref = x_ref + p->lay.ncp_pad;
+  HIPCHK(hipMemcpyAsync(scal_ref, f.scal, 64 * sizeof(double), hipMemcpyDeviceToDevice, p->stream));
+  HIPCHK(hipMemcpyAsync(fz_ref, f.fz, 4 * sizeof(double), hipMemcpyDeviceToDevice, p->stream));
+  hipLaunchKernelGGL(k_step_cam, dim3(1), dim3(BLOCK), (size_t)p->lay.ncp_pad * sizeof(double), p->stream, f.partial, f.rows, tr.x, tr.g, tr.sinv, tr.s,
+                     f.ncp_pad, scal_ref, f.flags, fz_ref, x_ref, step_ref, tab_ref, f.cam_const, f.cam_model, f.cam_np, f.cam_off, p->C,
+                     (const double*)nullptr, (const double*)nullptr, 0);
+  hipLaunchKernelGGL(k_step_fold_compare, dim3(1), dim3(BLOCK), 0, p->stream, (const double*)f.scal, (const double*)f.fz, (const double*)tr.x_new,
+                     (const double*)f.tab_out, (const double*)f.step_cam, (const double*)scal_ref, (const double*)fz_ref, (const double*)x_ref,
+                     (const double*)tab_ref, (const double*)step_ref, f.ncp_pad, p->C, p->fold_count);
+  return CBA_OK;
+}
+
+template <int NC>
 static int run_build_into(cba_problem* p, const double* xvec, const double* tab, double* V, double* g, double* Upacked, int cost_slot,
                           const double* skip = nullptr, bool defer_exchange = false, bool compact = false, int flag_slot = 0,
-                          const TrialSrc* trial = nullptr, const PubArgs* pub = nullptr, const ScaleArgs* scale = nullptr) {
+                          const TrialSrc* trial = nullptr, const PubArgs* pub = nullptr, const ScaleArgs* scale = nullptr, const StepFold* fold = nullptr) {
   RoctxRange range("cba:build");
   {
     ScopedTimer t(p, T_BUILD);
@@ -1452,7 +1485,7 @@
       const TrialSrc tsrc = trial ? *trial : TrialSrc{};
       auto launch_cs = [&](auto kernel, size_t lds) {
         hipLaunchKernelGGL(kernel, dim3(p->grid), dim3(BLOCK), lds, p->stream, p->cs, xvec, p->lay, tab, p->C, p->loss, p->f_scale,
-                           V, g, p->partial, p->partial1, p->flags + flag_slot, skip, tsrc);
+                           V, g, p->partial, p->partial1, p->flags + flag_slot, skip, tsrc, fold ? *fold : StepFold{});
       };
       if (build_cs_uglob<NC>(p)) {
         (void)hipMemsetAsync(p->partial, 0, (size_t)p->C * UPack<NC>::STRIDE * sizeof(double), p->stream);
@@ -1461,9 +1494,15 @@
       } else if (build_cs_camg<NC>(p)) {
         if (trial) launch_cs(k_build_cs<NC, true, false, true>, lds_build_cs<NC>(p, true));
         else launch_cs(k_build_cs<NC, true>, lds_build_cs<NC>(p, true));
+      } else if (fold) {
+        launch_cs(k_build_cs<NC, false, false, true, true>, lds_build_cs<NC>(p, false));
       } else {
         if (trial) launch_cs(k_build_cs<NC, false, false, true>, lds_build_cs<NC>(p, false));
         else launch_cs(k_build_cs<NC, false>, lds_build_cs<NC>(p, false));
+      }
+      if (fold && p->step_fold_verify) {
+        const int rcv = enqueue_step_fold_verify(p, *fold, tsrc);
+        if (rcv) return rcv;
       }
     } else
     switch (p->det_m) {
@@ -1946,6 +1985,7 @@
     }
   }
   if (fused_trial(p, compact)) {
+    if (step_folds<NC>(p, compact)) return CBA_OK;
     ScopedTimer t(p, T_VECTOR);
     hipLaunchKernelGGL(k_step_cam, dim3(1), dim3(BLOCK), (size_t)p->lay.ncp_pad * sizeof(double), p->stream, (const double*)p->partial4, p->grid_backsub,
                        (const double*)p->x, (const double*)p->g, (const double*)p->sinv, (const double*)p->s, p->lay.ncp_pad, p->scal, (const int*)p->flags, p->fz,
@@ -1993,19 +2033,22 @@
                        (const double*)p->cam_const, (const int*)p->cam_model, (const int*)p->cam_np, (const int*)p->cam_off, p->C);
     if (!compact) hipLaunchKernelGGL(k_reduce_narrow<false>, dim3(1), dim3(BLOCK), 0, p->stream, p->partial4, vg, 1, p->scal + 28);
   }
-  const TrialSrc tsrc{p->x, p->g, p->sinv, p->s, p->fz + 2, p->x_new, p->partial4};
+  const bool sfold = ft && step_folds<NC>(p, compact);
+  double* const step_rows = sfold ? p->partial4 + (size_t)4 * p->grid_backsub : p->partial4;
+  const TrialSrc tsrc{p->x, p->g, p->sinv, p->s, p->fz + 2, p->x_new, step_rows};
+  const StepFold sf_args{p->partial4, p->grid_backsub, p->lay.ncp_pad, p->scal, p->flags, p->fz, step_rows + p->grid, p->tab_new, p->cam_const, p->cam_model, p->cam_np, p->cam_off};
   const unsigned long long seq = compact ? ++p->publish_seq : 0;
   const bool bnd = compact && p->bounds_on;
   const bool last_trial = p->last_trial_hint;
   p->last_trial_hint = false;
   const bool spec_test = compact && p->spec_skip && p->tol_set && !p->bounds_on && !last_trial;
-  const PubArgs pub{p->scal, 49, p->flags, p->d_hscal, p->d_hflags, seq, p->partial1, p->grid, 24, p->partial4, ft ? p->grid + 1 : vg, 28,
+  const PubArgs pub{p->scal, 49, p->flags, p->d_hscal, p->d_hflags, seq, p->partial1, p->grid, 24, step_rows, ft ? p->grid + 1 : vg, 28,
                     {p->x, p->g, p->sinv_state_c, p->s}, bnd ? p->d_hbcam : (double*)nullptr, p->ncp,
                     spec_test ? p->spec_word : (int*)nullptr, p->ftol, p->xtol, p->cost_pending ? NAN : p->cost_x};
   const bool sf = scale_fusable<NC>(p, compact);
   const ScaleArgs sa{p->V2, p->lay, 0, p->sinv2, p->sinv, p->x_new, p->g2, p->v1, p->partial4b, p->partial_gmax};
   rc = run_build_into<NC>(p, p->x_new, p->tab_new, p->V2, p->g2, p->U2, 24, p->scal + 42, true, compact, 0, ft ? &tsrc : nullptr,
-                          compact ? &pub : nullptr, sf ? &sa : nullptr);
+                          compact ? &pub : nullptr, sf ? &sa : nullptr, sfold ? &sf_args : nullptr);
   if (rc) return rc;
   if (!compact) return CBA_OK;
   *seq_out = seq;
@@ -2351,6 +2394,18 @@
   if (rc) return rc;
   p->h_flags[1] = f1; p->h_flags[2] = f2;
   read_newton(p, out);
+  return CBA_OK;
+}
+
+int cba_test_step_fold_verified(cba_problem* p, int64_t* counts) {
+  if (!p || !counts) return fail(CBA_ERR_INVALID, "cba_test_step_fold_verified: null argument");
+  for (int i = 0; i < 6; ++i) counts[i] = 0;
+  if (!p->fold_count) return CBA_OK;
+  HIPCHK(hipSetDevice(p->device));
+  unsigned long long h[6] = {0, 0, 0, 0, 0, 0};
+  HIPCHK(hipMemcpyAsync(h, p->fold_count, sizeof h, hipMemcpyDeviceToHost, p->stream));
+  HIPCHK(hipStreamSynchronize(p->stream));
+  for (int i = 0; i < 6; ++i) counts[i] = (int64_t)h[i];
   return CBA_OK;
 }
 
diff --git a/caliscope_amd/csrc/trf_math.h b/caliscope_amd/csrc/trf_math.h
--- a/caliscope_amd/csrc/trf_math.h
+++ b/caliscope_amd/csrc/trf_math.h
@@ -97,7 +97,151 @@
   }
 }
 
+constexpr int PIECE_NONE = 0, PIECE_KNOT = 1, PIECE_BISECTED = 2;
+
+template <int N>
+TRF_HD inline double pick(const double* v, int k) {
+  double r = v[0];
+  for (int i = 1; i < N; ++i) r = (k == i) ? v[i] : r;
+  return r;
+}
+
+template <int N>
+TRF_HD inline void place(double* v, int k, double x) {
+  for (int i = 0; i < N; ++i)
+    if (k == i) v[i] = x;
+}
+
+template <int DEG>
+TRF_HD inline int pieces_knots(const double* c, double* crit, int nc, double* knots, double* scale) {
+  for (int i = 1; i < DEG - 1; ++i) {
+    bool go = i < nc;
+    for (int j = i; j > 0; --j) {
+      go = go && crit[j] < crit[j - 1];
+      if (go) { const double t = crit[j]; crit[j] = crit[j - 1]; crit[j - 1] = t; }
+    }
+  }
+  double bound = 0.0;
+  for (int i = 1; i <= DEG; ++i) bound = fmax(bound, fabs(c[i] / c[0]));
+  bound += 1.0;
+  for (int i = 0; i <= DEG; ++i) knots[i] = bound;
+  int nk = 0;
+  knots[nk++] = -bound;
+  for (int i = 0; i < DEG - 1; ++i)
+    if (i < nc && crit[i] > -bound && crit[i] < bound) place<DEG + 1>(knots, nk++, crit[i]);
+  place<DEG + 1>(knots, nk++, bound);
+  *scale = 0.0;
+  for (int i = 0; i <= DEG; ++i) *scale = fmax(*scale, fabs(c[i]));
+  return nk;
+}
+
+template <int DEG>
+TRF_HD inline int piece_root(const double* c, double a, double b, int nk, double scale, int k, double* root) {
+  double fa = poly_eval(c, DEG, a), fb = poly_eval(c, DEG, b);
+  if (fa == 0.0) { *root = a; return PIECE_KNOT; }
+  if (k + 2 == nk && fb == 0.0) { *root = b; return PIECE_KNOT; }
+  if ((fa < 0.0) == (fb < 0.0)) {
+    if (k > 0 && fabs(fa) <= 1e-14 * scale * fmax(1.0, pow(fabs(a), (double)DEG))) { *root = a; return PIECE_KNOT; }
+    return PIECE_NONE;
+  }
+  for (int it = 0; it < 200 && b - a > 0.0; ++it) {
+    const double m = 0.5 * (a + b);
+    if (m == a || m == b) break;
+    const double fm = poly_eval(c, DEG, m);
+    if (fm == 0.0) { a = b = m; break; }
+    if ((fm < 0.0) == (fa < 0.0)) { a = m; fa = fm; } else { b = m; }
+  }
+  *root = 0.5 * (a + b);
+  return PIECE_BISECTED;
+}
+
+template <int DEG>
+TRF_HD inline int pieces_collect(const int* kind, const double* root, int nk, double* out) {
+  int n = 0;
+  bool done = false;
+  for (int k = 0; k < DEG; ++k) {
+    if (done || k + 1 >= nk || kind[k] == PIECE_NONE) continue;
+    place<DEG>(out, n++, root[k]);
+    if (kind[k] == PIECE_BISECTED && n >= DEG) done = true;
+  }
+  return n;
+}
+
+struct SerialLanes {
+  template <int DEG>
+  TRF_HD void run(const double* c, const double* knots, int nk, double scale, int* kind, double* root) const {
+    for (int k = 0; k < DEG; ++k) {
+      kind[k] = PIECE_NONE; root[k] = 0.0;
+      if (k + 1 < nk) kind[k] = piece_root<DEG>(c, knots[k], knots[k + 1], nk, scale, k, &root[k]);
+    }
+  }
+};
+
+template <int DEG, class Lanes>
+TRF_HD inline int real_roots_pieces_of_degree(const double* c, double* out, const Lanes& lanes) {
+  if constexpr (DEG <= 2) {
+    return real_roots_of_degree<DEG>(c, out);
+  } else {
+    double d[DEG], crit[DEG - 1], knots[DEG + 1], scale;
+    for (int i = 0; i < DEG; ++i) d[i] = c[i] * (DEG - i);
+    const int nc = real_roots_pieces_of_degree<DEG - 1>(d, crit, lanes);
+    const int nk = pieces_knots<DEG>(c, crit, nc, knots, &scale);
+    int kind[DEG];
+    double root[DEG];
+    lanes.template run<DEG>(c, knots, nk, scale, kind, root);
+    return pieces_collect<DEG>(kind, root, nk, out);
+  }
+}
+
+template <int LEAD, class Lanes>
+TRF_HD inline int real_roots_pieces_behind(const double* c_in, int n_coef, double* out, const Lanes& lanes) {
+  switch (n_coef - 1 - LEAD) {
+    case 4: return real_roots_pieces_of_degree<4>(c_in + LEAD, out, lanes);
+    case 3: return real_roots_pieces_of_degree<3>(c_in + LEAD, out, lanes);
+    case 2: return real_roots_of_degree<2>(c_in + LEAD, out);
+    case 1: return real_roots_of_degree<1>(c_in + LEAD, out);
+    default: return 0;
+  }
+}
+template <class Lanes>
+TRF_HD inline int real_roots_pieces(const double* c_in, int n_coef, double* out, const Lanes& lanes) {
+  int lead = 0;
+  bool zeros = true;
+  for (int i = 0; i < 5; ++i) {
+    zeros = zeros && i < n_coef && c_in[i] == 0.0;
+    if (zeros) lead = i + 1;
+  }
+  switch (lead) {
+    case 0: return real_roots_pieces_behind<0>(c_in, n_coef, out, lanes);
+    case 1: return real_roots_pieces_behind<1>(c_in, n_coef, out, lanes);
+    case 2: return real_roots_pieces_behind<2>(c_in, n_coef, out, lanes);
+    case 3: return real_roots_pieces_behind<3>(c_in, n_coef, out, lanes);
+    default: return 0;
+  }
+}
+
+struct SerialRoots {
+  TRF_HD int operator()(const double* c, int n_coef, double* out) const { return real_roots(c, n_coef, out); }
+};
+template <class Lanes>
+struct PiecesRoots {
+  Lanes lanes;
+  TRF_HD int operator()(const double* c, int n_coef, double* out) const { return real_roots_pieces(c, n_coef, out, lanes); }
+};
+
+TRF_HD inline void subspace_quartic(double b00, double b01, double b11, double g0, double g1, double radius, double* coef) {
+  const double r2 = radius * radius;
+  const double a = b00 * r2, b = b01 * r2, c = b11 * r2, d = g0 * radius, f = g1 * radius;
+  coef[0] = -b + d; coef[1] = 2.0 * (a - c + f); coef[2] = 6.0 * b; coef[3] = 2.0 * (-a + c + f); coef[4] = -b - d;
+}
+
+template <class Roots>
+TRF_HD inline void solve_subspace_2d(double b00, double b01, double b11, double g0, double g1, double radius, double* p, const Roots& roots);
 TRF_HD inline void solve_subspace_2d(double b00, double b01, double b11, double g0, double g1, double radius, double* p) {
+  solve_subspace_2d(b00, b01, b11, g0, g1, radius, p, SerialRoots{});
+}
+template <class Roots>
+TRF_HD inline void solve_subspace_2d(double b00, double b01, double b11, double g0, double g1, double radius, double* p, const Roots& roots) {
   if (b00 > 0.0) {
     const double schur = b11 - b01 * b01 / b00;
     if (schur > 0.0) {
@@ -106,11 +250,9 @@
       if (p0 * p0 + p1 * p1 <= radius * radius) { p[0] = p0; p[1] = p1; return; }
     }
   }
-  const double r2 = radius * radius;
-  const double a = b00 * r2, b = b01 * r2, c = b11 * r2, d = g0 * radius, f = g1 * radius;
-  const double coef[5] = {-b + d, 2.0 * (a - c + f), 6.0 * b, 2.0 * (-a + c + f), -b - d};
-  double t[4];
-  const int nt = real_roots(coef, 5, t);
+  double coef[5], t[4];
+  subspace_quartic(b00, b01, b11, g0, g1, radius, coef);
+  const int nt = roots(coef, 5, t);
   if (nt == 0) {
     const double n = hypot(g0, g1);
     p[0] = n > 0 ? -radius * g0 / n : 0.0;
@@ -120,7 +262,7 @@
   double best = INFINITY;
   for (int i = 0; i <= nt; ++i) {
     double c0, c1;
-    if (i < nt) { const double q = 1.0 + t[i] * t[i]; c0 = radius * 2.0 * t[i] / q; c1 = radius * (1.0 - t[i] * t[i]) / q; }
+    if (i < nt) { const double ti = pick<4>(t, i), q = 1.0 + ti * ti; c0 = radius * 2.0 * ti / q; c1 = radius * (1.0 - ti * ti) / q; }
     else { c0 = 0.0; c1 = -radius; }
     const double val = 0.5 * (c0 * (b00 * c0 + b01 * c1) + c1 * (b01 * c0 + b11 * c1)) + g0 * c0 + g1 * c1;
     if (val < best) { best = val; p[0] = c0; p[1] = c1; }
```

Result: no change. 4.040 billion obs/s, median of 6 (+0.9%).
